# KhaoulaAguech/pl-fem-vectoriel

Hardware: AMD Instinct MI355X
Metric: eigenmodes/sec (assembly+solve), 7-core P2 mesh, 10 modes; |Δn_eff| vs ref (higher is better)
Workload: dtype f64

## Files before the change

include/plfem.h:

```cpp
#ifndef PLFEM_H
#define PLFEM_H

#include <stdint.h>

#ifdef __cplusplus
extern "C" {
#endif

#define PLFEM_OK 0
#define PLFEM_EINVAL (-1)
#define PLFEM_EMESH (-2)
#define PLFEM_EHIP (-3)
#define PLFEM_ENOCONV (-4)
#define PLFEM_ESTATE (-5)
#define PLFEM_ESINGULAR (-6)
#define PLFEM_ERESIDUAL (-7)
#define PLFEM_EHOST (-8)

typedef struct plfem_symbolic plfem_symbolic;
typedef struct plfem_ctx plfem_ctx;

int plfem_symbolic_create(int32_t nv, int32_t ne, const double* p_host, const int32_t* t_host,
                          int32_t leaf_elems, int32_t nthreads, plfem_symbolic** out,
                          char* err, int32_t errlen);
// ... 79 lines not shown
int plfem_modes_dev(plfem_ctx* ctx, const double** evecs_dev, int32_t* k);

int plfem_set_option(plfem_ctx* ctx, const char* name, double value);

int plfem_timings(plfem_ctx* ctx, double* out_host );

enum { PLFEM_PROF_KFWD = 0, PLFEM_PROF_FWD_SWEEP, PLFEM_PROF_BWD_SWEEP, PLFEM_PROF_SPMV_B, PLFEM_PROF_COUNT };
int plfem_profile_begin(plfem_ctx* ctx, int32_t max_ranges);
int plfem_profile_end(plfem_ctx* ctx, double* out_host );

#define PLFEM_LOC_TOL 1e-10
#define PLFEM_LOC_EPS4 8.881784197001252e-16
typedef struct plfem_locator plfem_locator;
int plfem_locator_bytes(const plfem_symbolic* sym, int64_t* bytes);
int plfem_locator_create(const plfem_symbolic* sym, int32_t device, void* hip_stream, void* mem_dev, int64_t mem_bytes,
                         plfem_locator** out, char* err, int32_t errlen);
void plfem_locator_destroy(plfem_locator* loc);
const char* plfem_locator_last_error(const plfem_locator* loc);
int plfem_stage_modes(plfem_locator* loc, int32_t ncomp, int32_t k, int32_t nrows, const double* src_dev, double* dst_dev);
int plfem_sample_fields(plfem_locator* loc, int32_t ncomp, int32_t k, const double* modes_dev, int32_t indexed,
                        const double* beta_dev, int32_t npts, const double* points_dev, double* out_dev, int32_t* elem_dev);
int plfem_overlap_work_bytes(int32_t ka, int32_t kb, int64_t* bytes);
int plfem_field_overlap(plfem_locator* loc_a, const double* modes_a_dev, int32_t ka, int32_t indexed_a,
                        plfem_locator* loc_b, const double* modes_b_dev, int32_t kb, int32_t indexed_b, int32_t ncomp,
                        const double* cores_host, int32_t ncore, double eps_core, double eps_clad,
                        void* work_dev, int64_t work_bytes, double* out_host);
int plfem_overlap_posed_work_bytes(const plfem_locator* loc_b, int32_t ka, int32_t kb, int32_t nposes, int64_t* bytes);
int plfem_field_overlap_posed(plfem_locator* loc_a, const double* modes_a_dev, int32_t ka, int32_t indexed_a,
                              plfem_locator* loc_b, const double* modes_b_dev, int32_t kb, int32_t indexed_b, int32_t ncomp,
                              const double* cores_host, int32_t ncore, double eps_core, double eps_clad,
                              int32_t nposes, const double* poses_host ,
                              void* work_dev, int64_t work_bytes, double* out_host );
int plfem_gram_work_bytes(int32_t ncomp, int32_t k, int64_t* bytes);
int plfem_mode_grams(plfem_locator* loc, int32_t ncomp, int32_t k, const double* modes_dev, int32_t indexed,
                     const double* cores_host, int32_t ncore, void* work_dev, int64_t work_bytes, double* out_host);

int plfem_profile_gram_work_bytes(int32_t ncomp, int32_t k, int64_t* bytes);
int plfem_profile_grams(plfem_locator* loc, int32_t ncomp, int32_t k, const double* modes_dev, int32_t indexed,
                        const double* layers_host, int32_t nlayer, double eps_bg, void* work_dev, int64_t work_bytes,
                        double* out_host);

int plfem_locator_set_index_map(plfem_locator* loc, const double* eps_host, int32_t nx, int32_t ny, double x0, double y0,
                                double dx, double dy);

int plfem_core_gram_work_bytes(const plfem_locator* loc, int32_t ncomp, int32_t k, int32_t ncore, int64_t* bytes);
int plfem_core_grams(plfem_locator* loc, int32_t ncomp, int32_t k, const double* modes_dev, int32_t indexed,
                     const double* cores_host, int32_t ncore, void* work_dev, int64_t work_bytes,
                     double* out_host   ,
                     int64_t* count_host );

int plfem_velocity_gram_work_bytes(const plfem_locator* loc, int32_t ncomp, int32_t k, int32_t nvel, int64_t* bytes);
int plfem_velocity_grams(plfem_locator* loc, int32_t ncomp, int32_t k, const double* modes_dev, int32_t indexed,
                         const double* cores_host, int32_t ncore, double eps_core, double eps_clad,
                         const double* layers_host, int32_t nlayer, double eps_bg, int32_t use_profile,
                         const double* velocities_host , int32_t nvel,
                         void* work_dev, int64_t work_bytes,
                         double* out_host    ,
                         int64_t* count_host );

int plfem_moment_gram_work_bytes(int32_t ncomp, int32_t k, int64_t* bytes);
int plfem_moment_grams(plfem_locator* loc, int32_t ncomp, int32_t k, const double* modes_dev, int32_t indexed,
                       const double* cores_host, int32_t ncore, const double origin_host[2], void* work_dev,
                       int64_t work_bytes, double* out_host);

int plfem_profile_tangent_gram_work_bytes(const plfem_locator* loc, int32_t ncomp, int32_t k, int32_t ntan, int32_t nmap,
                                          int32_t moments, int64_t* bytes);
int plfem_profile_tangent_grams(plfem_locator* loc, int32_t ncomp, int32_t k, const double* modes_dev, int32_t indexed,
                                const double* layers_host, int32_t nlayer, double eps_bg,
                                const double* tangents_host , int32_t ntan,
                                const double* tangent_maps_host , int32_t nmap,
                                const int32_t* tangent_map_host ,
                                int32_t moments, const double origin_host[2],
                                void* work_dev, int64_t work_bytes, double* out_host);

int plfem_index_map_gradient_work_bytes(const plfem_locator* loc, int32_t ncomp, int32_t k, int64_t* bytes);
int plfem_index_map_gradients(plfem_locator* loc, int32_t ncomp, int32_t k, const double* modes_dev, int32_t indexed,
                              const double* layers_host, int32_t nlayer, double eps_bg,
                              void* work_dev, int64_t work_bytes,
                              double* out_host ,
                              int32_t* support_host );

int plfem_quartic_work_bytes(int32_t ncomp, int32_t k, int64_t* bytes);
int plfem_mode_quartic(plfem_locator* loc, int32_t ncomp, int32_t k, const double* modes_dev, int32_t indexed,
                       const double* cores_host, int32_t ncore, double w_core, double w_clad,
                       void* work_dev, int64_t work_bytes, double* out_host);

int plfem_project_work_bytes(int32_t ncomp, int32_t k, int32_t la, int32_t lb, int64_t* bytes);
int plfem_mode_project(plfem_locator* loc, int32_t ncomp, int32_t k, const double* modes_dev, int32_t indexed,
                       int32_t la, const double* xfac_host ,
                       int32_t lb, const double* yfac_host ,
                       void* work_dev, int64_t work_bytes, double* out_host );

int plfem_project_sampled_work_bytes(int32_t ncomp, int32_t k, int32_t nf, int64_t* bytes);
int plfem_mode_project_sampled(plfem_locator* loc, int32_t ncomp, int32_t k, const double* modes_dev, int32_t indexed,
                               int32_t nx, int32_t ny, double x0, double y0, double dx, double dy,
                               int32_t nf, const double* frames_dev ,
                               void* work_dev, int64_t work_bytes, double* out_host );

int plfem_indicator_work_bytes(const plfem_locator* loc, int32_t ncomp, int32_t k, int64_t* bytes);
int plfem_mode_indicators(plfem_locator* loc, int32_t ncomp, int32_t k, const double* modes_dev, int32_t indexed,
                          const double* lambda_host , double k0, double alpha_p,
                          const double* cores_host, int32_t ncore, double eps_core, double eps_clad,
                          const double* layers_host, int32_t nlayer, double eps_bg,
                          void* work_dev, int64_t work_bytes, double* out_host );

int plfem_flux_gram_work_bytes(int32_t k, int64_t* bytes);
int plfem_flux_grams(plfem_locator* loc, int32_t ncomp, int32_t k, const double* modes_dev, int32_t indexed,
                     const double* cores_host, int32_t ncore, double eps_core, double eps_clad,
                     const double* layers_host, int32_t nlayer, double eps_bg, int32_t use_profile,
                     void* work_dev, int64_t work_bytes, double* out_host );
int plfem_sample_efields(plfem_locator* loc, int32_t ncomp, int32_t k, const double* modes_dev, int32_t indexed,
                         const double* beta_dev , double k0,
                         const double* cores_host, int32_t ncore, double eps_core, double eps_clad,
                         const double* layers_host, int32_t nlayer, double eps_bg, int32_t use_profile,
                         int32_t npts, const double* points_dev, double* out_dev ,
                         double* eps_dev , int32_t* elem_dev);
int plfem_flux_overlap_posed_work_bytes(const plfem_locator* loc_b, int32_t ka, int32_t kb, int32_t nposes, int64_t* bytes);
int plfem_flux_overlap_posed(plfem_locator* loc_a, const double* modes_a_dev, int32_t ka, int32_t indexed_a,
                             const double* cores_a_host, int32_t ncore_a, double eps_core_a, double eps_clad_a,
                             const double* layers_a_host, int32_t nlayer_a, double eps_bg_a, int32_t use_profile_a,
                             plfem_locator* loc_b, const double* modes_b_dev, int32_t kb, int32_t indexed_b,
                             const double* cores_b_host, int32_t ncore_b, double eps_core_b, double eps_clad_b,
                             const double* layers_b_host, int32_t nlayer_b, double eps_bg_b, int32_t use_profile_b,
                             int32_t nposes, const double* poses_host ,
                             void* work_dev, int64_t work_bytes, double* out_host );

#ifdef PLFEM_TEST_HOOKS
int plfem_debug_factor_until(plfem_ctx* ctx, double sigma, int32_t level, int32_t step, int32_t stage);
int plfem_debug_copy(plfem_ctx* ctx, const char* name, int64_t offset, int64_t count, double* out_host);
int plfem_debug_symeig(int32_t n, const double* a_host, int32_t last_rows, double* w_out, double* v_out);
int plfem_debug_symeig_band(int32_t n, int32_t b, const double* a_host, int32_t nsel, double* w_out, double* v_out);
int plfem_debug_set_perturb(plfem_ctx* ctx, double value);
int plfem_debug_set_elements(plfem_ctx* ctx, const double* elem_host );
#define PLFEM_DEBUG_PLAN_FIELDS 10
int plfem_debug_solve_block(plfem_ctx* ctx, const double* rhs_dev, int64_t ldx, double* x_dev, int32_t refine_steps);
int plfem_debug_level_plan(plfem_ctx* ctx, int64_t* out, int64_t cap);
enum { PLFEM_DEBUG_PANEL_DOT = 0, PLFEM_DEBUG_PANEL_AXPY, PLFEM_DEBUG_PANEL_DOT_BLOCK, PLFEM_DEBUG_PANEL_AXPY_BLOCK };
enum { PLFEM_DEBUG_SPMV_B_BLOCK = 0, PLFEM_DEBUG_SPMV_B_BLOCK_IL, PLFEM_DEBUG_SPMV_B_BLOCK_IL_GRAM, PLFEM_DEBUG_SPMV_A_BLOCK };
int plfem_debug_panel(plfem_ctx* ctx, int32_t form, int32_t ncols, const double* Pm, double* W, int64_t ldw, double* H,
                      int32_t ldh, double* hacc, int32_t ldacc, double* wil);
int plfem_debug_scale_store(plfem_ctx* ctx, const double* w, const double* bw, const double* beta2, double* v, double* bv,
                            double* beta_out);
int plfem_debug_first_pass(plfem_ctx* ctx, const double* xl_front, const double* BVm, const double* Vm, int32_t ncols,
                           double* W, int64_t ldw, double* Hout, int32_t ldh);
int plfem_debug_spmv_block(plfem_ctx* ctx, int32_t form, const double* x, double* y, int64_t ld, double* gram_out,
                           int32_t* nparts);
int plfem_debug_chol(plfem_ctx* ctx, const double* G, int32_t ldg, int32_t use_partials, int32_t nchunks, double* Tblk,
                     int32_t ldT, double* Rinv, int32_t* rank_flag);
int plfem_debug_block_scale(plfem_ctx* ctx, const double* W, const double* BW, int64_t ldw, const double* Rinv, double* Vn,
                            double* BVn, int64_t ldv, const double* exp_src, int32_t exp_n, double* exp_dst, int32_t* cnt_dst,
                            int32_t want_front);
int plfem_debug_rotate(plfem_ctx* ctx, const double* V, int32_t m, const double* S, int32_t ldS, int32_t p, double* out);
int plfem_debug_start_field(plfem_ctx* ctx, int32_t nvec, double* out);
#endif

#ifdef __cplusplus
}
#endif
#endif
```

pl_fem_vectoriel_amd/_native.py:

```python
from __future__ import annotations

import ctypes
import time
import os
from typing import Optional

import numpy as np

_HERE = os.path.dirname(os.path.abspath(__file__))
LIB_PATH = os.path.join(_HERE, "libplfem_hip.so")
HOOKS_PATH = os.path.join(_HERE, "libplfem_testhooks.so")

PLFEM_OK = 0
PLFEM_EINVAL, PLFEM_EMESH, PLFEM_EHIP, PLFEM_ENOCONV, PLFEM_ESTATE, PLFEM_ESINGULAR, PLFEM_ERESIDUAL = -1, -2, -3, -4, -5, -6, -7
PLFEM_EHOST = -8
BLOCKS = ("Axx", "Axy", "Ayx", "Ayy", "Minv", "Dxx", "Dxy", "Dyy")
INFO_NAMES = ("nv", "ne", "nedges", "N", "nsolve", "nnz", "levels", "nfronts", "front_doubles", "max_front",
              "solve_entries", "factor_flops", "t_numbering_us", "t_pattern_us", "t_tree_us", "t_fronts_us", "dofs_per_node",
              "arena_doubles")
POST_NAMES = ("norm", "div_energy", "core_x", "core_y", "all_x", "all_y")

EXPORTS = (
    "plfem_symbolic_create", "plfem_symbolic_destroy", "plfem_symbolic_info", "plfem_symbolic_array_bytes",
    "plfem_symbolic_get", "plfem_workspace_bytes", "plfem_create", "plfem_destroy", "plfem_last_error", "plfem_synchronize",
    "plfem_assemble_hfield", "plfem_block_values_dev", "plfem_block_values_host", "plfem_spmv", "plfem_factor",
    "plfem_solve", "plfem_lanczos_shift_invert", "plfem_postprocess", "plfem_timings",
    "plfem_profile_begin", "plfem_profile_end",
    "plfem_mesh_edge_count", "plfem_mesh_refine",
    "plfem_residuals", "plfem_set_option", "plfem_symbolic_create_ex", "plfem_assemble_scalar", "plfem_cmt_coupling",
    "plfem_solve_modes", "plfem_modes_dev",
    "plfem_locator_bytes", "plfem_locator_create", "plfem_locator_destroy", "plfem_locator_last_error", "plfem_stage_modes",
    "plfem_sample_fields", "plfem_overlap_work_bytes", "plfem_field_overlap", "plfem_gram_work_bytes", "plfem_mode_grams",
    "plfem_overlap_posed_work_bytes", "plfem_field_overlap_posed",
    "plfem_quartic_work_bytes", "plfem_mode_quartic", "plfem_project_work_bytes", "plfem_mode_project",
    "plfem_core_gram_work_bytes", "plfem_core_grams", "plfem_moment_gram_work_bytes", "plfem_moment_grams",
    "plfem_set_index_profile", "plfem_profile_gram_work_bytes", "plfem_profile_grams",
    "plfem_project_sampled_work_bytes", "plfem_mode_project_sampled",
    "plfem_indicator_work_bytes", "plfem_mode_indicators", "plfem_mesh_refine_marked_count", "plfem_mesh_refine_marked",
    "plfem_set_index_map", "plfem_locator_set_index_map",
    "plfem_flux_gram_work_bytes", "plfem_flux_grams", "plfem_sample_efields",
    "plfem_flux_overlap_posed_work_bytes", "plfem_flux_overlap_posed",
    "plfem_profile_tangent_gram_work_bytes", "plfem_profile_tangent_grams",
    "plfem_velocity_gram_work_bytes", "plfem_velocity_grams",
    "plfem_index_map_gradient_work_bytes", "plfem_index_map_gradients",
)
SOLVE_STATS = ("nconv", "n_opinv", "restarts", "max_rel_res", "n_block_solves", "true_residual_first", "true_residual", "refined",
               "pivot_perturbations", "assemble_us", "factor_us", "lanczos_us", "post_us", "upload_us", "residual_us", "call_us")
TEST_HOOK_EXPORTS = ("plfem_debug_factor_until", "plfem_debug_copy", "plfem_debug_symeig", "plfem_debug_symeig_band",
                     "plfem_debug_set_perturb", "plfem_debug_solve_block", "plfem_debug_level_plan", "plfem_debug_panel",
                     "plfem_debug_scale_store", "plfem_debug_first_pass", "plfem_debug_spmv_block", "plfem_debug_chol",
                     "plfem_debug_block_scale", "plfem_debug_rotate", "plfem_debug_start_field", "plfem_debug_set_elements")
PANEL_FORMS = ("dot", "axpy", "dot_block", "axpy_block")
SPMV_BLOCK_FORMS = ("b_block", "b_block_il", "b_block_il_gram", "a_block")
BLOCK_P = 4
PLAN_FIELDS = ("count", "fwd_rows", "bwd_rows", "fwd_mixed", "max_s2", "max_m", "fwd_n", "bwd_n", "steps", "max_block_p")
MAX_NCV = 320
PROF_SLOTS = ("k_fwd", "fwd_sweep", "bwd_sweep", "spmv_b")

_ARRAY_DTYPES = {
    "edof": np.int32, "tsorted": np.int32, "edges": np.int32, "doflocs": np.float64, "bmask": np.uint8,
    "interior": np.int32, "int_index": np.int32, "rowptr": np.int32, "colind": np.int32, "slot_row": np.int32,
    "nptr": np.int32, "nadj": np.int32, "nloc": np.uint8, "leaf_of_elem": np.int32, "leaf_elem_ptr": np.int32, "leaf_elems": np.int32, "epos": np.int32, "epos_leaf": np.int32,
    "owner": np.int32, "fs": np.int32, "fb": np.int32, "fs_true": np.int32, "fb_true": np.int32,
    "fnode_ptr": np.int64, "fnodes": np.int32, "cinv0": np.int32, "cinv1": np.int32, "foff": np.int64, "soff": np.int64, "prow": np.int32, "npos": np.int32,
    "loc_grid": np.float64, "loc_cell_ptr": np.int32, "loc_cell_elems": np.int32, "loc_stats": np.float64,
    "elem_nbr": np.int32,
}


from scipy.sparse.linalg import ArpackNoConvergence as _ArpackNoConvergence


def set_index_map_call(entry, handle, index_map):
    if index_map is None:
        return entry(handle, None, 0, 0, 0.0, 0.0, 0.0, 0.0)
    eps, x0, y0, dx, dy = index_map
    eps = np.ascontiguousarray(eps, dtype=np.float64)
    if eps.ndim != 2:
        raise ValueError("the index map must be a (ny, nx) array")
    return entry(handle, eps.ctypes.data_as(ctypes.c_void_p), eps.shape[1], eps.shape[0], float(x0), float(y0), float(dx),
                 float(dy))


class ArpackLikeNoConvergence(_ArpackNoConvergence, RuntimeError):

    def __init__(self, msg, eigenvalues=None, eigenvectors=None, stats=None):
        _ArpackNoConvergence.__init__(self, msg, eigenvalues, eigenvectors)
        self.stats = stats


_lib = None
_hooks = None

SCRATCH_FILL = None


def device_scratch(nbytes: int, tdev):
    import torch
    if SCRATCH_FILL is None:
        return torch.empty(int(nbytes), dtype=torch.uint8, device=tdev)
    buf = torch.empty((int(nbytes) + 7) & ~7, dtype=torch.uint8, device=tdev)
    buf.view(torch.float64).fill_(float(SCRATCH_FILL))
    torch.cuda.current_stream(tdev).synchronize()
    return buf


def device_output(shape, dtype, tdev):
    import torch
    if SCRATCH_FILL is None:
        return torch.empty(shape, dtype=dtype, device=tdev)
    shape = tuple(int(v) for v in (shape if isinstance(shape, (tuple, list)) else (shape,)))
    nbytes = int(np.prod(shape, dtype=np.int64)) * torch.empty((), dtype=dtype).element_size()
    return device_scratch(nbytes, tdev)[:nbytes].view(dtype).view(shape)


def _tune_host_allocator(_force: bool = False) -> None:
    if os.environ.get("PLFEM_MALLOC_TUNE", "0") != "1" and not _force:
        return
    try:
        libc = ctypes.CDLL("libc.so.6")
        libc.mallopt(-3, 32 << 20)
        libc.mallopt(-1, 512 << 20)
    except (OSError, AttributeError):
        pass


def load_library() -> ctypes.CDLL:
    global _lib
    if _lib is not None:
        return _lib
    if not os.path.exists(LIB_PATH):
        raise RuntimeError(
            f"libplfem_hip.so requis: {LIB_PATH} not found — build it with "
            "`python -c 'import __graft_entry__ as g; g.build()'` (hipcc --offload-arch=gfx950). "
            "There is no CPU fallback for the eigenmode path.")
    import torch
    lib = ctypes.CDLL(LIB_PATH)
    _tune_host_allocator()
    c_void_pp = ctypes.POINTER(ctypes.c_void_p)
    lib.plfem_symbolic_create.argtypes = [ctypes.c_int32, ctypes.c_int32, ctypes.c_void_p, ctypes.c_void_p,
                                          ctypes.c_int32, ctypes.c_int32, c_void_pp, ctypes.c_char_p, ctypes.c_int32]
    lib.plfem_symbolic_create_ex.argtypes = [ctypes.c_int32, ctypes.c_int32, ctypes.c_void_p, ctypes.c_void_p, ctypes.c_int32,
                                             ctypes.c_int32, ctypes.c_int32, ctypes.c_int32, c_void_pp, ctypes.c_char_p, ctypes.c_int32]
    lib.plfem_symbolic_destroy.argtypes = [ctypes.c_void_p]
    lib.plfem_symbolic_destroy.restype = None
    lib.plfem_symbolic_info.argtypes = [ctypes.c_void_p, ctypes.c_void_p]
    lib.plfem_symbolic_array_bytes.argtypes = [ctypes.c_void_p, ctypes.c_char_p]
    lib.plfem_symbolic_array_bytes.restype = ctypes.c_int64
    lib.plfem_symbolic_get.argtypes = [ctypes.c_void_p, ctypes.c_char_p, ctypes.c_void_p, ctypes.c_int64]
    lib.plfem_workspace_bytes.argtypes = [ctypes.c_void_p, ctypes.c_int32, ctypes.POINTER(ctypes.c_int64)]
    lib.plfem_create.argtypes = [ctypes.c_void_p, ctypes.c_int32, ctypes.c_void_p, ctypes.c_int32, ctypes.c_void_p,
                                 ctypes.c_int64, c_void_pp, ctypes.c_char_p, ctypes.c_int32]
    lib.plfem_destroy.argtypes = [ctypes.c_void_p]
    lib.plfem_destroy.restype = None
    lib.plfem_last_error.argtypes = [ctypes.c_void_p]
    lib.plfem_last_error.restype = ctypes.c_char_p
    lib.plfem_synchronize.argtypes = [ctypes.c_void_p]
    lib.plfem_assemble_hfield.argtypes = [ctypes.c_void_p, ctypes.c_void_p, ctypes.c_int32, ctypes.c_double,
                                          ctypes.c_double, ctypes.c_double, ctypes.c_double]
    lib.plfem_assemble_scalar.argtypes = [ctypes.c_void_p, ctypes.c_void_p, ctypes.c_int32, ctypes.c_double,
                                          ctypes.c_double, ctypes.c_double]
    lib.plfem_cmt_coupling.argtypes = [ctypes.c_void_p, ctypes.c_int32, ctypes.c_void_p, ctypes.c_void_p, ctypes.c_void_p,
                                       ctypes.c_int32, ctypes.c_double, ctypes.c_double, ctypes.c_void_p, ctypes.c_void_p,
                                       ctypes.c_void_p, ctypes.POINTER(ctypes.c_double)]
    lib.plfem_block_values_dev.argtypes = [ctypes.c_void_p, ctypes.c_int32, c_void_pp]
    lib.plfem_block_values_host.argtypes = [ctypes.c_void_p, ctypes.c_int32, ctypes.c_void_p]
    lib.plfem_spmv.argtypes = [ctypes.c_void_p, ctypes.c_int32, ctypes.c_void_p, ctypes.c_void_p]
    lib.plfem_factor.argtypes = [ctypes.c_void_p, ctypes.c_double]
    lib.plfem_solve.argtypes = [ctypes.c_void_p, ctypes.c_void_p, ctypes.c_void_p, ctypes.c_int32]
    lib.plfem_lanczos_shift_invert.argtypes = [ctypes.c_void_p, ctypes.c_int32, ctypes.c_int32, ctypes.c_double,
                                               ctypes.c_int32, ctypes.c_double, ctypes.c_void_p, ctypes.c_void_p,
                                               ctypes.c_void_p]
    lib.plfem_postprocess.argtypes = [ctypes.c_void_p, ctypes.c_int32, ctypes.c_void_p, ctypes.c_void_p,
                                      ctypes.c_int32, ctypes.c_void_p, ctypes.c_void_p, ctypes.c_void_p]
    lib.plfem_timings.argtypes = [ctypes.c_void_p, ctypes.c_void_p]
    lib.plfem_mesh_edge_count.argtypes = [ctypes.c_int32, ctypes.c_int32, ctypes.c_void_p, ctypes.c_void_p,
                                          ctypes.POINTER(ctypes.c_int32), ctypes.c_char_p, ctypes.c_int32]
    lib.plfem_mesh_refine.argtypes = [ctypes.c_int32, ctypes.c_int32, ctypes.c_void_p, ctypes.c_void_p,
                                      ctypes.c_void_p, ctypes.c_void_p, ctypes.c_char_p, ctypes.c_int32]
    lib.plfem_profile_begin.argtypes = [ctypes.c_void_p, ctypes.c_int32]
    lib.plfem_profile_end.argtypes = [ctypes.c_void_p, ctypes.c_void_p]
    lib.plfem_residuals.argtypes = [ctypes.c_void_p, ctypes.c_int32, ctypes.c_void_p, ctypes.c_void_p, ctypes.c_void_p]
    lib.plfem_set_option.argtypes = [ctypes.c_void_p, ctypes.c_char_p, ctypes.c_double]
    lib.plfem_solve_modes.argtypes = ([ctypes.c_void_p, ctypes.c_void_p, ctypes.c_int32] + [ctypes.c_double] * 5 +
                                      [ctypes.c_int32, ctypes.c_int32, ctypes.c_double, ctypes.c_int32, ctypes.c_double,
                                       ctypes.c_double] + [ctypes.c_void_p] * 6)
    lib.plfem_modes_dev.argtypes = [ctypes.c_void_p, c_void_pp, ctypes.POINTER(ctypes.c_int32)]
    lib.plfem_locator_bytes.argtypes = [ctypes.c_void_p, ctypes.POINTER(ctypes.c_int64)]
    lib.plfem_locator_create.argtypes = [ctypes.c_void_p, ctypes.c_int32, ctypes.c_void_p, ctypes.c_void_p, ctypes.c_int64,
                                         c_void_pp, ctypes.c_char_p, ctypes.c_int32]
    lib.plfem_locator_destroy.argtypes = [ctypes.c_void_p]
    lib.plfem_locator_destroy.restype = None
    lib.plfem_locator_last_error.argtypes = [ctypes.c_void_p]
    lib.plfem_locator_last_error.restype = ctypes.c_char_p
    vp, i32, i64, f64 = ctypes.c_void_p, ctypes.c_int32, ctypes.c_int64, ctypes.c_double
    head, tail, size = [vp, i32, i32, vp, i32], [vp, i64, vp], [ctypes.POINTER(i64)]
    pair = [vp, vp, i32, i32] * 2 + [i32, vp, i32, f64, f64]
    lib.plfem_stage_modes.argtypes = [vp, i32, i32, i32, vp, vp]
    lib.plfem_sample_fields.argtypes = head + [vp, i32, vp, vp, vp]
    lib.plfem_overlap_work_bytes.argtypes = [i32, i32] + size
    lib.plfem_field_overlap.argtypes = pair + tail
    lib.plfem_overlap_posed_work_bytes.argtypes = [vp, i32, i32, i32] + size
    lib.plfem_field_overlap_posed.argtypes = pair + [i32, vp] + tail
    lib.plfem_gram_work_bytes.argtypes = [i32, i32] + size
    lib.plfem_mode_grams.argtypes = head + [vp, i32] + tail
    lib.plfem_core_gram_work_bytes.argtypes = [vp, i32, i32, i32] + size
    lib.plfem_core_grams.argtypes = head + [vp, i32] + tail + [vp]
    lib.plfem_moment_gram_work_bytes.argtypes = [i32, i32] + size
    lib.plfem_moment_grams.argtypes = head + [vp, i32, vp] + tail
    lib.plfem_set_index_profile.argtypes = [vp, vp, i32, f64]
    lib.plfem_set_index_map.argtypes = [vp, vp, i32, i32] + [f64] * 4
    lib.plfem_locator_set_index_map.argtypes = lib.plfem_set_index_map.argtypes
    lib.plfem_profile_gram_work_bytes.argtypes = [i32, i32] + size
    lib.plfem_profile_grams.argtypes = head + [vp, i32, f64] + tail
    lib.plfem_profile_tangent_gram_work_bytes.argtypes = [vp, i32, i32, i32, i32, i32] + size
    lib.plfem_profile_tangent_grams.argtypes = head + [vp, i32, f64, vp, i32, vp, i32, vp, i32, vp] + tail
    lib.plfem_quartic_work_bytes.argtypes = [i32, i32] + size
    lib.plfem_mode_quartic.argtypes = head + [vp, i32, f64, f64] + tail
    lib.plfem_project_work_bytes.argtypes = [i32] * 4 + size
    lib.plfem_mode_project.argtypes = head + [i32, vp, i32, vp] + tail
    lib.plfem_project_sampled_work_bytes.argtypes = [i32] * 3 + size
    lib.plfem_mode_project_sampled.argtypes = head + [i32, i32, f64, f64, f64, f64, i32, vp] + tail
    lib.plfem_indicator_work_bytes.argtypes = [vp, i32, i32] + size
    lib.plfem_mode_indicators.argtypes = head + [vp, f64, f64, vp, i32, f64, f64, vp, i32, f64] + tail
    material = [vp, i32, f64, f64, vp, i32, f64, i32]
    lib.plfem_flux_gram_work_bytes.argtypes = [i32] + size
    lib.plfem_flux_grams.argtypes = head + material + tail
    lib.plfem_sample_efields.argtypes = head + [vp, f64] + material + [i32, vp, vp, vp, vp]
    lib.plfem_flux_overlap_posed_work_bytes.argtypes = [vp, i32, i32, i32] + size
    lib.plfem_flux_overlap_posed.argtypes = ([vp, vp, i32, i32] + material) * 2 + [i32, vp] + tail
    lib.plfem_velocity_gram_work_bytes.argtypes = [vp, i32, i32, i32] + size
    lib.plfem_velocity_grams.argtypes = head + material + [vp, i32] + tail + [vp]
    lib.plfem_index_map_gradient_work_bytes.argtypes = [vp, i32, i32] + size
    lib.plfem_index_map_gradients.argtypes = head + [vp, i32, f64] + tail + [vp]
    lib.plfem_mesh_refine_marked_count.argtypes = [ctypes.c_int32, ctypes.c_int32, ctypes.c_void_p, ctypes.c_void_p,
                                                   ctypes.c_void_p, ctypes.POINTER(ctypes.c_int32),
                                                   ctypes.POINTER(ctypes.c_int32), ctypes.c_char_p, ctypes.c_int32]
    lib.plfem_mesh_refine_marked.argtypes = [ctypes.c_int32, ctypes.c_int32, ctypes.c_void_p, ctypes.c_void_p, ctypes.c_void_p,
                                             ctypes.c_void_p, ctypes.c_void_p, ctypes.c_void_p, ctypes.c_char_p, ctypes.c_int32]
    _lib = lib
    return lib


def _ptr(a: np.ndarray):
    return a.ctypes.data_as(ctypes.c_void_p)


def mesh_refine(p, t):
    lib = load_library()
    p = np.ascontiguousarray(np.asarray(p, dtype=np.float64))
    t = np.ascontiguousarray(np.asarray(t, dtype=np.int32))
    if p.ndim != 2 or p.shape[0] != 2 or t.ndim != 2 or t.shape[0] != 3:
        raise ValueError("mesh.p must be (2, nv) and mesh.t (3, ne)")
    err = ctypes.create_string_buffer(512)
    nedges = ctypes.c_int32(0)
    rc = lib.plfem_mesh_edge_count(p.shape[1], t.shape[1], _ptr(p), _ptr(t), ctypes.byref(nedges), err, 512)
    if rc != PLFEM_OK:
        raise ValueError(f"plfem_mesh_edge_count failed ({rc}): {err.value.decode()}")
    p2 = np.empty((2, p.shape[1] + nedges.value), dtype=np.float64)
    t2 = np.empty((3, 4 * t.shape[1]), dtype=np.int32)
    rc = lib.plfem_mesh_refine(p.shape[1], t.shape[1], _ptr(p), _ptr(t), _ptr(p2), _ptr(t2), err, 512)
    if rc != PLFEM_OK:
        raise ValueError(f"plfem_mesh_refine failed ({rc}): {err.value.decode()}")
    return p2, t2


def mesh_refine_marked(p, t, marked):
    lib = load_library()
    p = np.ascontiguousarray(np.asarray(p, dtype=np.float64))
    t = np.ascontiguousarray(np.asarray(t, dtype=np.int32))
    if p.ndim != 2 or p.shape[0] != 2 or t.ndim != 2 or t.shape[0] != 3:
        raise ValueError("mesh.p must be (2, nv) and mesh.t (3, ne)")
    try:
        mk = np.asarray(marked)
        if mk.dtype.kind not in "biu":
            raise TypeError
    except (TypeError, ValueError):
        raise ValueError("marked must be an array of one flag (bool or integer) per element") from None
    if mk.shape != (t.shape[1],):
        raise ValueError(f"marked must have one flag per element ({t.shape[1]}), got shape {mk.shape}")
    mk = np.ascontiguousarray(mk != 0, dtype=np.uint8)
    err = ctypes.create_string_buffer(512)
    nv2, ne2 = ctypes.c_int32(0), ctypes.c_int32(0)
    rc = lib.plfem_mesh_refine_marked_count(p.shape[1], t.shape[1], _ptr(p), _ptr(t), _ptr(mk), ctypes.byref(nv2),
                                            ctypes.byref(ne2), err, 512)
    if rc != PLFEM_OK:
        raise ValueError(f"plfem_mesh_refine_marked_count failed ({rc}): {err.value.decode()}")
    p2 = np.empty((2, nv2.value), dtype=np.float64)
    t2 = np.empty((3, ne2.value), dtype=np.int32)
    parent = np.empty(ne2.value, dtype=np.int32)
    rc = lib.plfem_mesh_refine_marked(p.shape[1], t.shape[1], _ptr(p), _ptr(t), _ptr(mk), _ptr(p2), _ptr(t2), _ptr(parent),
                                      err, 512)
    if rc != PLFEM_OK:
        raise ValueError(f"plfem_mesh_refine_marked failed ({rc}): {err.value.decode()}")
    return p2, t2, parent


def load_test_hooks() -> ctypes.CDLL:
    global _hooks
    if _hooks is not None:
        return _hooks
    load_library()
    if not os.path.exists(HOOKS_PATH):
        raise RuntimeError(f"{HOOKS_PATH} not found -- build it with `python -c 'import __graft_entry__ as g; g.build()'`")
    h = ctypes.CDLL(HOOKS_PATH)
    h.plfem_debug_factor_until.argtypes = [ctypes.c_void_p, ctypes.c_double, ctypes.c_int32, ctypes.c_int32, ctypes.c_int32]
    h.plfem_debug_copy.argtypes = [ctypes.c_void_p, ctypes.c_char_p, ctypes.c_int64, ctypes.c_int64, ctypes.c_void_p]
    h.plfem_debug_set_perturb.argtypes = [ctypes.c_void_p, ctypes.c_double]
    h.plfem_debug_set_elements.argtypes = [ctypes.c_void_p, ctypes.c_void_p]
    h.plfem_debug_solve_block.argtypes = [ctypes.c_void_p, ctypes.c_void_p, ctypes.c_int64, ctypes.c_void_p, ctypes.c_int32]
    h.plfem_debug_level_plan.argtypes = [ctypes.c_void_p, ctypes.c_void_p, ctypes.c_int64]
    h.plfem_debug_symeig.argtypes = [ctypes.c_int32, ctypes.c_void_p, ctypes.c_int32, ctypes.c_void_p, ctypes.c_void_p]
    h.plfem_debug_symeig_band.argtypes = [ctypes.c_int32, ctypes.c_int32, ctypes.c_void_p, ctypes.c_int32,
                                          ctypes.c_void_p, ctypes.c_void_p]
    vp, i32, i64 = ctypes.c_void_p, ctypes.c_int32, ctypes.c_int64
    h.plfem_debug_panel.argtypes = [vp, i32, i32, vp, vp, i64, vp, i32, vp, i32, vp]
    h.plfem_debug_scale_store.argtypes = [vp, vp, vp, vp, vp, vp, vp]
    h.plfem_debug_first_pass.argtypes = [vp, vp, vp, vp, i32, vp, i64, vp, i32]
    h.plfem_debug_spmv_block.argtypes = [vp, i32, vp, vp, i64, vp, vp]
    h.plfem_debug_chol.argtypes = [vp, vp, i32, i32, i32, vp, i32, vp, vp]
    h.plfem_debug_block_scale.argtypes = [vp, vp, vp, i64, vp, vp, vp, i64, vp, i32, vp, vp, i32]
    h.plfem_debug_rotate.argtypes = [vp, vp, i32, vp, i32, i32, vp]
    h.plfem_debug_start_field.argtypes = [vp, i32, vp]
    _hooks = h
    return h


def debug_symeig(a, last_rows: int = -1):
    lib = load_test_hooks()
    a = np.ascontiguousarray(np.asarray(a, dtype=np.float64))
    n = a.shape[0]
    if a.shape != (n, n):
        raise ValueError("square matrix expected")
    w = np.empty(n, dtype=np.float64)
    v = np.empty((n, n if last_rows < 0 else last_rows), dtype=np.float64)
    rc = lib.plfem_debug_symeig(n, _ptr(a), int(last_rows), _ptr(w), _ptr(v))
    if rc != PLFEM_OK:
        raise ValueError(f"plfem_debug_symeig failed ({rc})")
    return w, v


def debug_symeig_band(a, b: int, nsel: int):
    lib = load_test_hooks()
    a = np.ascontiguousarray(np.asarray(a, dtype=np.float64))
    n = a.shape[0]
    if a.shape != (n, n):
        raise ValueError("square matrix expected")
    w = np.empty(n, dtype=np.float64)
    v = np.empty((n, n), dtype=np.float64)
    rc = lib.plfem_debug_symeig_band(n, int(b), _ptr(a), int(nsel), _ptr(w), _ptr(v))
    if rc != PLFEM_OK:
        raise ValueError(f"plfem_debug_symeig_band failed ({rc})")
    return w, v


def default_host_threads() -> int:
    ncpu = os.cpu_count() or 1
    if ncpu < 64:
        return max(1, min(ncpu, 8))
    try:
        local_world = max(1, int(os.environ.get("LOCAL_WORLD_SIZE", "1")))
    except ValueError:
        local_world = 1
    return max(2, min(24, (ncpu // 2) // local_world))


class Symbolic:

    def __init__(self, p, t, leaf_elems: int = 0, nthreads: int = 0, dofs_per_node: int = 2, dirichlet: bool = True):
        lib = load_library()
        p = np.ascontiguousarray(np.asarray(p, dtype=np.float64))
        t = np.ascontiguousarray(np.asarray(t, dtype=np.int32))
        if p.ndim != 2 or p.shape[0] != 2 or t.ndim != 2 or t.shape[0] != 3:
            raise ValueError("mesh.p must be (2, nv) and mesh.t (3, ne)")
        h = ctypes.c_void_p()
        err = ctypes.create_string_buffer(512)
        if nthreads <= 0:
            nthreads = int(os.environ.get("PLFEM_HOST_THREADS", default_host_threads()))
        if leaf_elems <= 0:
            leaf_elems = int(os.environ.get("PLFEM_LEAF_ELEMS", 0))
        rc = lib.plfem_symbolic_create_ex(p.shape[1], t.shape[1], _ptr(p), _ptr(t), int(leaf_elems), int(nthreads),
                                          int(dofs_per_node), 1 if dirichlet else 0, ctypes.byref(h), err, 512)
        if rc != PLFEM_OK:
            raise ValueError(f"plfem_symbolic_create failed ({rc}): {err.value.decode()}")
        self._h = h
        self._lib = lib
        info = np.zeros(32, dtype=np.int64)
        lib.plfem_symbolic_info(h, _ptr(info))
        self.info = {k: int(info[i]) for i, k in enumerate(INFO_NAMES)}
        for k in ("nv", "ne", "nedges", "N", "nsolve", "nnz"):
            setattr(self, k, self.info[k])
        self.dofs_per_node = self.info["dofs_per_node"]

    def array(self, name: str) -> np.ndarray:
        nb = self._lib.plfem_symbolic_array_bytes(self._h, name.encode())
        if nb < 0:
            raise KeyError(name)
        out = np.empty(nb // np.dtype(_ARRAY_DTYPES[name]).itemsize, dtype=_ARRAY_DTYPES[name])
        rc = self._lib.plfem_symbolic_get(self._h, name.encode(), _ptr(out), ctypes.c_int64(nb))
        if rc != PLFEM_OK:
            raise RuntimeError(f"plfem_symbolic_get({name}) failed: {rc}")
        return out

    def close(self):
        if getattr(self, "_h", None):
            self._lib.plfem_symbolic_destroy(self._h)
            self._h = None

    def __del__(self):
        try:
            self.close()
        except Exception:
            pass


class Context:

    def __init__(self, sym: Symbolic, device: Optional[int] = None, max_ncv: int = 65, use_torch_stream: bool = True):
        import torch

        lib = load_library()
        if not torch.cuda.is_available():
            raise RuntimeError("no HIP device visible: the eigenmode path has no CPU fallback")
        if device is None:
            device = torch.cuda.current_device()
        self.torch = torch
        self.device = int(device)
        self.tdev = torch.device("cuda", self.device)
        self.sym = sym
        self._lib = lib
        stream = torch.cuda.current_stream(self.tdev).cuda_stream if use_torch_stream else 0
        h = ctypes.c_void_p()
        err = ctypes.create_string_buffer(512)
        need = ctypes.c_int64(0)
        rc = lib.plfem_workspace_bytes(sym._h, int(max_ncv), ctypes.byref(need))
        if rc != PLFEM_OK:
            raise ValueError(f"plfem_workspace_bytes failed ({rc})")
        t0 = time.perf_counter()
        self.workspace = device_scratch(int(need.value) + 256, self.tdev)
        self.t_workspace = time.perf_counter() - t0
        base = self.workspace.data_ptr()
        aligned = (base + 255) & ~255
        rc = lib.plfem_create(sym._h, self.device, ctypes.c_void_p(stream), int(max_ncv), ctypes.c_void_p(aligned),
                              ctypes.c_int64(int(need.value)), ctypes.byref(h), err, 512)
        if rc in (PLFEM_EINVAL, PLFEM_EMESH):
            raise ValueError(f"plfem_create: {err.value.decode()}")
        if rc != PLFEM_OK:
            raise RuntimeError(f"plfem_create failed ({rc}): {err.value.decode()}")
        self._h = h
        self.max_ncv = int(max_ncv)
        self.N = sym.N
        self.dpn = sym.dofs_per_node
        self.n2 = self.dpn * sym.N

    def _check(self, rc, what):
        if rc == PLFEM_OK:
            return
        msg = self._lib.plfem_last_error(self._h).decode()
        if rc in (PLFEM_EINVAL, PLFEM_EMESH):
            raise ValueError(f"{what}: {msg}")
        raise RuntimeError(f"{what} failed ({rc}): {msg}")

    def _cores(self, cores):
        c = np.ascontiguousarray(np.asarray(cores, dtype=np.float64).reshape(-1, 3))
        return c, c.shape[0]

    def empty(self, *shape):
        return device_output(shape, self.torch.float64, self.tdev)

    def set_index_profile(self, profile=None):
        if profile is None:
            self._check(self._lib.plfem_set_index_profile(self._h, None, 0, 0.0), "plfem_set_index_profile")
            self.set_index_map(None)
            return
        t = np.ascontiguousarray(np.asarray(profile.table(), dtype=np.float64).reshape(-1, 8))
        index_map = getattr(profile, "index_map", None)
# ... 36 lines not shown

    def spmv(self, which: str, x):
        y = self.empty(self.n2)
        self._check(self._lib.plfem_spmv(self._h, 0 if which == "A" else 1, ctypes.c_void_p(x.data_ptr()),
                                         ctypes.c_void_p(y.data_ptr())), "plfem_spmv")
        return y

    def factor(self, sigma: float):
        self._check(self._lib.plfem_factor(self._h, float(sigma)), "plfem_factor")

    def solve(self, rhs, refine_steps: int = 0):
        x = self.empty(self.n2)
        self._check(self._lib.plfem_solve(self._h, ctypes.c_void_p(rhs.data_ptr()), ctypes.c_void_p(x.data_ptr()),
                                          int(refine_steps)), "plfem_solve")
        return x

    def lanczos(self, k, ncv, tol, maxiter, sigma):
        evals = np.empty(k, dtype=np.float64)
        evecs = self.empty(k, self.n2)
        stats = np.zeros(8, dtype=np.float64)
        rc = self._lib.plfem_lanczos_shift_invert(self._h, int(k), int(ncv), float(tol), int(maxiter), float(sigma),
                                                  _ptr(evals), ctypes.c_void_p(evecs.data_ptr()), _ptr(stats))
        st = {"nconv": int(stats[0]), "n_opinv": int(stats[1]), "restarts": int(stats[2]), "max_rel_res": float(stats[3]),
              "n_block_solves": int(stats[4])}
        if rc == PLFEM_ENOCONV:
            raise ArpackLikeNoConvergence(self._lib.plfem_last_error(self._h).decode(), evals, evecs, st)
        self._check(rc, "plfem_lanczos_shift_invert")
        return evals, evecs, st

    def solve_modes(self, cores, eps_core, eps_clad, k0, alpha_p, sigma, k, ncv, tol, maxiter, residual_tol, tol_refined,
                    modes_host=None):
        c, n = self._cores(cores)
        evals = np.empty(k, dtype=np.float64)
        post = np.zeros((k, len(POST_NAMES)), dtype=np.float64)
        resid = np.zeros(k, dtype=np.float64)
        stats = np.zeros(len(SOLVE_STATS), dtype=np.float64)
        frac = ctypes.c_double(0.0)
        if modes_host is not None and (tuple(modes_host.shape) != (k, self.dpn * self.sym.nsolve) or not modes_host.is_contiguous()
                                       or modes_host.dtype != self.torch.float64 or modes_host.device.type != "cpu"):
            raise ValueError("modes_host must be a contiguous float64 CPU tensor of shape (k, dofs_per_node * nsolve)")
        rc = self._lib.plfem_solve_modes(self._h, _ptr(c), n, float(eps_core), float(eps_clad), float(k0), float(alpha_p),
                                         float(sigma), int(k), int(ncv), float(tol), int(maxiter), float(residual_tol),
                                         float(tol_refined), _ptr(evals), _ptr(post), ctypes.cast(ctypes.byref(frac), ctypes.c_void_p),
                                         _ptr(resid), ctypes.c_void_p(modes_host.data_ptr()) if modes_host is not None else None,
                                         _ptr(stats))
        st = {name: (float(stats[i]) if name.endswith("_us") or "res" in name else int(stats[i])) for i, name in enumerate(SOLVE_STATS)}
        st["refined"] = bool(st["refined"])
        if rc == PLFEM_ENOCONV:
            raise ArpackLikeNoConvergence(self._lib.plfem_last_error(self._h).decode(), evals, self.modes_dev(), st)
        self._check(rc, "plfem_solve_modes")
        return evals, post, float(frac.value), resid, st

    def modes_dev(self):
        ptr = ctypes.c_void_p()
        k = ctypes.c_int32(0)
        self._check(self._lib.plfem_modes_dev(self._h, ctypes.byref(ptr), ctypes.byref(k)), "plfem_modes_dev")

        class _View:
            __cuda_array_interface__ = {"shape": (int(k.value), int(self.n2)), "typestr": "<f8", "data": (int(ptr.value), False),
                                        "version": 2, "strides": None}
        return self.torch.as_tensor(_View(), device=self.tdev).clone()

    def postprocess(self, evecs, cores, want_interior: bool = True):
        k = evecs.shape[0]
        c, n = self._cores(cores)
        out = np.zeros((k, len(POST_NAMES)), dtype=np.float64)
        frac = ctypes.c_double(0.0)
        modes_int = self.empty(k, self.dpn * self.sym.nsolve) if want_interior else None
        self._check(self._lib.plfem_postprocess(self._h, int(k), ctypes.c_void_p(evecs.data_ptr()), _ptr(c), n,
                                                _ptr(out), ctypes.byref(frac),
                                                ctypes.c_void_p(modes_int.data_ptr()) if want_interior else None),
                    "plfem_postprocess")
        return out, float(frac.value), modes_int

    def timings(self):
        t = np.zeros(8, dtype=np.float64)
        self._check(self._lib.plfem_timings(self._h, _ptr(t)), "plfem_timings")
        return {"assemble_us": t[0], "factor_us": t[1], "lanczos_us": t[2], "post_us": t[3], "upload_us": t[4],
                "pivot_perturbations": int(t[5])}

    def debug_factor_until(self, sigma, level, step, stage):
        self._check(load_test_hooks().plfem_debug_factor_until(self._h, float(sigma), int(level), int(step), int(stage)),
                    "plfem_debug_factor_until")

    def debug_copy(self, name: str, offset: int, count: int) -> np.ndarray:
        out = np.empty(int(count), dtype=np.float64)
        self._check(load_test_hooks().plfem_debug_copy(self._h, name.encode(), ctypes.c_int64(int(offset)),
                                                       ctypes.c_int64(int(count)), _ptr(out)), "plfem_debug_copy")
        return out

    def debug_set_perturb(self, value: float):
        self._check(load_test_hooks().plfem_debug_set_perturb(self._h, float(value)), "plfem_debug_set_perturb")

    def debug_set_elements(self, elem: np.ndarray):
        elem = np.ascontiguousarray(elem, dtype=np.float64)
        if elem.size != self.sym.ne * 8 * 36:
            raise ValueError("debug_set_elements: need ne x 8 x 36 doubles")
        self._check(load_test_hooks().plfem_debug_set_elements(self._h, _ptr(elem)), "plfem_debug_set_elements")

    def debug_solve_block(self, rhs, x, ldx: int, refine_steps: int = 0):
        self._check(load_test_hooks().plfem_debug_solve_block(self._h, ctypes.c_void_p(rhs.data_ptr()), ctypes.c_int64(int(ldx)),
                                                              ctypes.c_void_p(x.data_ptr()), int(refine_steps)),
                    "plfem_debug_solve_block")

    @staticmethod
    def _dev(t, offset: int = 0):
        return None if t is None else ctypes.c_void_p(t.data_ptr() + 8 * int(offset))

    def debug_panel(self, form: str, ncols: int, Pm, W, ldw: int, H, ldh: int, hacc=None, ldacc: int = 0, wil=None):
        d = self._dev
        self._check(load_test_hooks().plfem_debug_panel(self._h, PANEL_FORMS.index(form), int(ncols), d(Pm), d(W), int(ldw), d(H),
                                                        int(ldh), d(hacc), int(ldacc), d(wil)), "plfem_debug_panel")

    def debug_scale_store(self, w, bw, beta2, v, bv, beta_out=None):
        d = self._dev
        self._check(load_test_hooks().plfem_debug_scale_store(self._h, d(w), d(bw), d(beta2), d(v), d(bv), d(beta_out)),
                    "plfem_debug_scale_store")

    def debug_first_pass(self, xl_front, BVm, Vm, ncols: int, W, ldw: int, Hout, ldh: int):
        d = self._dev
        self._check(load_test_hooks().plfem_debug_first_pass(self._h, d(xl_front), d(BVm), d(Vm), int(ncols), d(W), int(ldw),
                                                             d(Hout), int(ldh)), "plfem_debug_first_pass")

    def debug_spmv_block(self, form: str, x, y, ld: int, gram_out=None) -> int:
        nparts = ctypes.c_int32(0)
        d = self._dev
        self._check(load_test_hooks().plfem_debug_spmv_block(self._h, SPMV_BLOCK_FORMS.index(form), d(x), d(y), int(ld),
                                                             d(gram_out), ctypes.byref(nparts)), "plfem_debug_spmv_block")
        return int(nparts.value)

    def debug_chol(self, G, ldg: int, use_partials: bool, nchunks: int, Tblk, ldT: int, Rinv, Tblk_offset: int = 0) -> int:
        flag = ctypes.c_int32(0)
        d = self._dev
        self._check(load_test_hooks().plfem_debug_chol(self._h, d(G), int(ldg), 1 if use_partials else 0, int(nchunks),
                                                       d(Tblk, Tblk_offset), int(ldT), d(Rinv), ctypes.byref(flag)),
                    "plfem_debug_chol")
        return int(flag.value)

    def debug_block_scale(self, W, BW, ldw: int, Rinv, Vn, BVn, ldv: int, exp_src=None, exp_n: int = 0, exp_dst=None,
                          cnt_dst=None, want_front: bool = False):
        d = self._dev
        self._check(load_test_hooks().plfem_debug_block_scale(self._h, d(W), d(BW), int(ldw), d(Rinv), d(Vn), d(BVn), int(ldv),
                                                              d(exp_src), int(exp_n), d(exp_dst), d(cnt_dst),
                                                              1 if want_front else 0), "plfem_debug_block_scale")

    def debug_rotate(self, V, m: int, S, ldS: int, p: int, out):
        d = self._dev
        self._check(load_test_hooks().plfem_debug_rotate(self._h, d(V), int(m), d(S), int(ldS), int(p), d(out)),
                    "plfem_debug_rotate")

    def debug_start_field(self, nvec: int, out):
        self._check(load_test_hooks().plfem_debug_start_field(self._h, int(nvec), self._dev(out)), "plfem_debug_start_field")

    def debug_level_plan(self):
        nl = self.sym.info["levels"] + 1
        out = np.zeros(len(PLAN_FIELDS) * nl, dtype=np.int64)
        self._check(load_test_hooks().plfem_debug_level_plan(self._h, _ptr(out), ctypes.c_int64(out.size)),
                    "plfem_debug_level_plan")
        return [dict(zip(PLAN_FIELDS, (int(v) for v in row))) for row in out.reshape(nl, len(PLAN_FIELDS))]

    def profile_begin(self, max_launches: int = 4096):
        self._check(self._lib.plfem_profile_begin(self._h, int(max_launches)), "plfem_profile_begin")

    def profile_end(self):
        out = np.zeros((len(PROF_SLOTS), 3), dtype=np.float64)
        self._check(self._lib.plfem_profile_end(self._h, _ptr(out)), "plfem_profile_end")
        res = {"launches": int(out[0, 0]), "total_us": float(out[0, 1]), "bytes": float(out[0, 2])}
        res["slots"] = {name: {"ranges": int(out[i, 0]), "total_us": float(out[i, 1]), "bytes": float(out[i, 2])}
                        for i, name in enumerate(PROF_SLOTS)}
        return res

    def residuals(self, evals, evecs) -> np.ndarray:
        lam = np.ascontiguousarray(np.asarray(evals, dtype=np.float64))
        out = np.zeros(len(lam), dtype=np.float64)
        self._check(self._lib.plfem_residuals(self._h, len(lam), _ptr(lam), ctypes.c_void_p(evecs.data_ptr()), _ptr(out)),
                    "plfem_residuals")
        return out

    def set_option(self, name: str, value: float):
        self._check(self._lib.plfem_set_option(self._h, name.encode(), float(value)), "plfem_set_option")

    def synchronize(self):
        self._check(self._lib.plfem_synchronize(self._h), "plfem_synchronize")

    def close(self):
        if getattr(self, "_h", None):
            self._lib.plfem_destroy(self._h)
            self._h = None
            self.workspace = None

    def __del__(self):
        try:
            self.close()
        except Exception:
            pass
```

pl_fem_vectoriel_amd/csrc/api_debug.hip:

```cpp
#include <algorithm>
#include <cmath>
#include <cstring>
#include <numeric>
#include <string>
#include <vector>

#ifndef PLFEM_TEST_HOOKS
#define PLFEM_TEST_HOOKS 1
#endif
#include "device.h"

namespace {
void perturb_root_pivots(plfem_ctx* c) {
  if (c->test_perturb != 0.0)
    plfem::launch_axpby(c, (int64_t)2 * c->dpn * c->S->fs[0], 1.0 + c->test_perturb, c->d_delta, 0.0, c->d_delta,
                        c->d_delta);
}
}

extern "C" int plfem_debug_set_perturb(plfem_ctx* c, double value) try {
  if (!c) return PLFEM_EINVAL;
  c->test_perturb = value;
  c->test_post_factor = value != 0.0 ? perturb_root_pivots : nullptr;
  c->factored = false;
  return PLFEM_OK;
} catch (...) { return host_failure(c); }

extern "C" int plfem_debug_factor_until(plfem_ctx* c, double sigma, int32_t level, int32_t step, int32_t stage) try {
  if (!c) return PLFEM_EINVAL;
  if (!c->assembled) { c->err = "debug factor before assemble"; return PLFEM_ESTATE; }
  TRY(wait_for_upload(c));
  plfem::launch_factor(c, sigma, level, step, stage);
  HIP_TRY(c, hipStreamSynchronize(c->stream));
  return check_launch(c, "debug factor");
} catch (...) { return host_failure(c); }

extern "C" int plfem_debug_copy(plfem_ctx* c, const char* name, int64_t offset, int64_t count, double* out_host) try {
  if (!c || !name || !out_host || offset < 0 || count < 0) return PLFEM_EINVAL;
  std::string n(name);
  const double* src = nullptr;
  if (n == "front") src = c->d_front;
  else if (n == "schur") src = c->d_schur;
  else if (n == "fvec") src = c->d_fvec;
  else if (n == "wbuf") src = c->d_wbuf;
  else if (n == "rbuf") src = c->d_rbuf;
  else if (n == "dinv") src = c->d_dinv;
  else if (n == "delta") src = c->d_delta;
  else if (n == "fvec2") src = c->d_fvec2;
  else if (n == "xl") src = c->d_xl;
  else if (n == "elem") src = c->d_elem;
  else if (n == "V") src = c->d_V;
  else if (n == "BV") src = c->d_BV;
  else if (n == "Hcols") src = c->d_Hcols;
  else if (n == "counters") {
    if (offset + count > 4) return PLFEM_EINVAL;
    int32_t tmp[4];
    HIP_TRY(c, hipStreamSynchronize(c->stream));
    HIP_TRY(c, hipMemcpy(tmp, c->d_counters, sizeof(tmp), hipMemcpyDeviceToHost));
    for (int64_t q = 0; q < count; ++q) out_host[q] = (double)tmp[offset + q];
    return PLFEM_OK;
  }
  else if (n == "colind" || n == "slot_row") {
    if (offset + count > c->nnz) return PLFEM_EINVAL;
    std::vector<int32_t> tmp((size_t)count);
    HIP_TRY(c, hipStreamSynchronize(c->stream));
    HIP_TRY(c, hipMemcpy(tmp.data(), (n == "colind" ? c->d_colind : c->d_slot_row) + offset, sizeof(int32_t) * count, hipMemcpyDeviceToHost));
    for (int64_t q = 0; q < count; ++q) out_host[q] = (double)tmp[q];
    return PLFEM_OK;
  }
  else return PLFEM_EINVAL;
  HIP_TRY(c, hipStreamSynchronize(c->stream));
  HIP_TRY(c, hipMemcpy(out_host, src + offset, sizeof(double) * count, hipMemcpyDeviceToHost));
  return PLFEM_OK;
} catch (...) { return host_failure(c); }

extern "C" int plfem_debug_set_elements(plfem_ctx* c, const double* elem_host) try {
  if (!c || !elem_host) return PLFEM_EINVAL;
  HIP_TRY(c, hipSetDevice(c->device));
  TRY(wait_for_upload(c));
  HIP_TRY(c, hipStreamSynchronize(c->stream));
  HIP_TRY(c, hipMemcpy(c->d_elem, elem_host, sizeof(double) * (size_t)c->ne * plfem::ELEM_STRIDE, hipMemcpyHostToDevice));
  plfem::launch_csr_gather(c);
  HIP_TRY(c, hipStreamSynchronize(c->stream));
  TRY(check_launch(c, "debug set elements"));
  c->assembled = true;
  c->factored = false;
  return PLFEM_OK;
} catch (...) { return host_failure(c); }

extern "C" int plfem_debug_solve_block(plfem_ctx* c, const double* rhs_dev, int64_t ldx, double* x_dev, int32_t refine_steps) try {
  constexpr int P = plfem::BLOCK_P;
  if (!c || !rhs_dev || !x_dev || refine_steps < 0) return PLFEM_EINVAL;
  if (!c->factored) { c->err = "debug block solve before plfem_factor"; return PLFEM_ESTATE; }
  if (c->max_block_p < P) { c->err = "debug block solve: the LDS budget of this tree allows one right-hand side per sweep"; return PLFEM_EINVAL; }
  if (ldx < c->n2) { c->err = "debug block solve: ldx < n2"; return PLFEM_EINVAL; }
  const int64_t scratch = (int64_t)c->n2 * plfem::basis_cols(c->max_ncv);
  if (refine_steps > 0 && 3 * P * ldx > scratch) { c->err = "debug block solve: ldx too large for the refinement scratch"; return PLFEM_EINVAL; }
  HIP_TRY(c, hipSetDevice(c->device));
  plfem::solve_refined(c, P, rhs_dev, x_dev, ldx, false, refine_steps, c->d_V2, c->d_V2 + (size_t)P * ldx,
                       c->d_V2 + (size_t)2 * P * ldx);
  HIP_TRY(c, hipStreamSynchronize(c->stream));
  return check_launch(c, "debug block solve");
} catch (...) { return host_failure(c); }

extern "C" int plfem_debug_level_plan(plfem_ctx* c, int64_t* out, int64_t cap) try {
  if (!c || !out) return PLFEM_EINVAL;
  const plfem::LaunchPlan& plan = *c->plan;
  const int nl = (int)plan.levels.size();
  if (cap < (int64_t)PLFEM_DEBUG_PLAN_FIELDS * nl) { c->err = "debug level plan: cap too small"; return PLFEM_EINVAL; }
  for (int l = 0; l < nl; ++l) {
    const plfem::LevelInfo& li = plan.levels[l];
    const int next = l + 1 < nl ? plan.levels[l + 1].step0 : (int)plan.upd_n.size();
    const int64_t rec[PLFEM_DEBUG_PLAN_FIELDS] = {li.count, li.fwd_rows, li.bwd_rows, li.fwd_mixed ? 1 : 0, li.max_s2, li.max_m,
                                                  li.fwd_n, li.bwd_n, next - li.step0, c->max_block_p};
    std::copy(rec, rec + PLFEM_DEBUG_PLAN_FIELDS, out + (int64_t)PLFEM_DEBUG_PLAN_FIELDS * l);
  }
  return PLFEM_OK;
} catch (...) { return host_failure(c); }

namespace {
int lanczos_hook_done(plfem_ctx* c, const char* what) {
  HIP_TRY(c, hipStreamSynchronize(c->stream));
  return check_launch(c, what);
}
}

extern "C" int plfem_debug_panel(plfem_ctx* c, int32_t form, int32_t ncols, const double* Pm, double* W, int64_t ldw, double* H,
                                 int32_t ldh, double* hacc, int32_t ldacc, double* wil) try {
  constexpr int P = plfem::BLOCK_P;
  if (!c || !H || !Pm || !W || form < PLFEM_DEBUG_PANEL_DOT || form > PLFEM_DEBUG_PANEL_AXPY_BLOCK) return PLFEM_EINVAL;
  if (ncols < 1 || ncols > c->max_ncv + P) { c->err = "debug panel: need 1 <= ncols <= max_ncv + BLOCK_P"; return PLFEM_EINVAL; }
  const bool block = form == PLFEM_DEBUG_PANEL_DOT_BLOCK || form == PLFEM_DEBUG_PANEL_AXPY_BLOCK;
  if (block && (ldw < c->n2 || ldh < ncols || (hacc && ldacc < ncols))) { c->err = "debug panel: leading dimension too small"; return PLFEM_EINVAL; }
  HIP_TRY(c, hipSetDevice(c->device));
  switch (form) {
    case PLFEM_DEBUG_PANEL_DOT: plfem::launch_panel_dot(c, 1, Pm, ncols, W, ldw, H, ldh, hacc, ldacc); break;
    case PLFEM_DEBUG_PANEL_AXPY: plfem::launch_panel_axpy(c, 1, Pm, ncols, H, ldh, W, ldw); break;
    case PLFEM_DEBUG_PANEL_DOT_BLOCK: plfem::launch_panel_dot(c, P, Pm, ncols, W, ldw, H, ldh, hacc, ldacc); break;
    default: plfem::launch_panel_axpy(c, P, Pm, ncols, H, ldh, W, ldw, wil); break;
  }
  return lanczos_hook_done(c, "debug panel");
} catch (...) { return host_failure(c); }

extern "C" int plfem_debug_scale_store(plfem_ctx* c, const double* w, const double* bw, const double* beta2, double* v, double* bv,
                                       double* beta_out) try {
  if (!c || !w || !bw || !beta2 || !v || !bv) return PLFEM_EINVAL;
  HIP_TRY(c, hipSetDevice(c->device));
  plfem::launch_scale_store(c, w, bw, beta2, v, bv, beta_out);
  return lanczos_hook_done(c, "debug scale store");
} catch (...) { return host_failure(c); }

extern "C" int plfem_debug_first_pass(plfem_ctx* c, const double* xl_front, const double* BVm, const double* Vm, int32_t ncols,
                                      double* W, int64_t ldw, double* Hout, int32_t ldh) try {
  if (!c || !xl_front || !BVm || !Vm || !W || !Hout) return PLFEM_EINVAL;
  if (ncols < 1 || ncols > plfem::FIRST_COLS || ldw < c->n2 || ldh < ncols) { c->err = "debug first pass: need 1 <= ncols <= FIRST_COLS, ldw >= n2, ldh >= ncols"; return PLFEM_EINVAL; }
  HIP_TRY(c, hipSetDevice(c->device));
  HIP_TRY(c, hipMemcpyAsync(c->d_xl, xl_front, sizeof(double) * 2 * c->fnodes_total * plfem::BLOCK_P, hipMemcpyDeviceToDevice, c->stream));
  plfem::launch_first_pass_block(c, BVm, Vm, ncols, W, ldw, Hout, ldh);
  return lanczos_hook_done(c, "debug first pass");
} catch (...) { return host_failure(c); }

extern "C" int plfem_debug_spmv_block(plfem_ctx* c, int32_t form, const double* x, double* y, int64_t ld, double* gram_out,
                                      int32_t* nparts) try {
  constexpr int P = plfem::BLOCK_P;
  if (!c || !x || !y || form < PLFEM_DEBUG_SPMV_B_BLOCK || form > PLFEM_DEBUG_SPMV_A_BLOCK) return PLFEM_EINVAL;
  if (!c->assembled) { c->err = "debug block spmv before assemble"; return PLFEM_ESTATE; }
  if (ld < c->n2) { c->err = "debug block spmv: ld < n2"; return PLFEM_EINVAL; }
  HIP_TRY(c, hipSetDevice(c->device));
  int np = 0;
  switch (form) {
    case PLFEM_DEBUG_SPMV_B_BLOCK: plfem::launch_spmv(c, 1, P, x, y, ld); break;
    case PLFEM_DEBUG_SPMV_B_BLOCK_IL: plfem::launch_spmv_b_block_il(c, x, y, ld); break;
    case PLFEM_DEBUG_SPMV_B_BLOCK_IL_GRAM:
      np = plfem::launch_spmv_b_block_il(c, x, y, ld, c->d_partial);
      if (gram_out) HIP_TRY(c, hipMemcpyAsync(gram_out, c->d_partial, sizeof(double) * P * P * np, hipMemcpyDeviceToDevice, c->stream));
      break;
    default: plfem::launch_spmv(c, 0, P, x, y, ld); break;
  }
  if (nparts) *nparts = np;
  return lanczos_hook_done(c, "debug block spmv");
} catch (...) { return host_failure(c); }

extern "C" int plfem_debug_chol(plfem_ctx* c, const double* G, int32_t ldg, int32_t use_partials, int32_t nchunks, double* Tblk,
                                int32_t ldT, double* Rinv, int32_t* rank_flag) try {
  constexpr int P = plfem::BLOCK_P;
  if (!c || !Tblk || !Rinv || ldT < P) return PLFEM_EINVAL;
  HIP_TRY(c, hipSetDevice(c->device));
  if (use_partials) {
    if (nchunks < 1 || (size_t)P * P * nchunks > c->partial_doubles) { c->err = "debug chol: nchunks out of range"; return PLFEM_EINVAL; }
    if (G) HIP_TRY(c, hipMemcpyAsync(c->d_partial, G, sizeof(double) * P * P * nchunks, hipMemcpyDeviceToDevice, c->stream));
  } else if (!G || ldg < P) {
    return PLFEM_EINVAL;
  }
  HIP_TRY(c, hipMemsetAsync(c->d_counters + 2, 0, sizeof(int32_t), c->stream));
  if (use_partials) plfem::launch_chol_from_partials(c, nchunks, Tblk, ldT, Rinv);
  else plfem::launch_chol_block(c, G, ldg, Tblk, ldT, Rinv);
  int32_t flag = 0;
  HIP_TRY(c, hipMemcpyAsync(&flag, c->d_counters + 2, sizeof(int32_t), hipMemcpyDeviceToHost, c->stream));
  HIP_TRY(c, hipMemsetAsync(c->d_counters + 2, 0, sizeof(int32_t), c->stream));
  TRY(lanczos_hook_done(c, "debug chol"));
  if (rank_flag) *rank_flag = flag;
  return PLFEM_OK;
} catch (...) { return host_failure(c); }

extern "C" int plfem_debug_block_scale(plfem_ctx* c, const double* W, const double* BW, int64_t ldw, const double* Rinv, double* Vn,
                                       double* BVn, int64_t ldv, const double* exp_src, int32_t exp_n, double* exp_dst,
                                       int32_t* cnt_dst, int32_t want_front) try {
  if (!c || !W || !BW || !Rinv || !Vn || !BVn || exp_n < 0) return PLFEM_EINVAL;
  if (ldw < c->n2 || ldv < c->n2) { c->err = "debug block scale: leading dimension < n2"; return PLFEM_EINVAL; }
  if (exp_dst && (!exp_src || !cnt_dst)) { c->err = "debug block scale: an export needs exp_src and cnt_dst"; return PLFEM_EINVAL; }
  HIP_TRY(c, hipSetDevice(c->device));
  plfem::launch_block_scale(c, W, BW, ldw, Rinv, Vn, BVn, ldv, exp_src, exp_dst ? exp_n : 0, exp_dst, cnt_dst,
                            want_front ? c->d_fvec : nullptr);
  return lanczos_hook_done(c, "debug block scale");
} catch (...) { return host_failure(c); }

extern "C" int plfem_debug_rotate(plfem_ctx* c, const double* V, int32_t m, const double* S, int32_t ldS, int32_t p, double* out) try {
  if (!c || !V || !S || !out) return PLFEM_EINVAL;
  if (m < 1 || m > PLFEM_MAX_NCV + plfem::BLOCK_P || p < 1 || ldS < m) { c->err = "debug rotate: need 1 <= m <= PLFEM_MAX_NCV + BLOCK_P, p >= 1, ldS >= m"; return PLFEM_EINVAL; }
  HIP_TRY(c, hipSetDevice(c->device));
  plfem::launch_rotate(c, V, m, S, ldS, p, out);
  return lanczos_hook_done(c, "debug rotate");
} catch (...) { return host_failure(c); }

extern "C" int plfem_debug_start_field(plfem_ctx* c, int32_t nvec, double* out) try {
  if (!c || !out || nvec < 1 || nvec > plfem::BLOCK_P) return PLFEM_EINVAL;
  HIP_TRY(c, hipSetDevice(c->device));
  plfem::launch_start_field(c, nvec, out);
  return lanczos_hook_done(c, "debug start field");
} catch (...) { return host_failure(c); }
```

pl_fem_vectoriel_amd/csrc/device.h:

```cpp
#pragma once
#include <hip/hip_runtime.h>

#include <cmath>
#include <cstdint>
#include <functional>
#include <string>
#include <type_traits>
#include <vector>

#include "../../include/plfem.h"
#include "internal.h"
#include "plan.h"

namespace plfem {

constexpr size_t PIN_POST = 0;
constexpr size_t PIN_RESID = 2048;
constexpr size_t PIN_CORE_QP = 4000;
constexpr size_t PIN_COUNTERS = 4096;
constexpr int PIN_COUNTERS_N = 2 * 4;
constexpr size_t PIN_CORES = 6144;
constexpr size_t PIN_LAYERS = 6400;
constexpr size_t PIN_PROJ = 8192;
static_assert(PIN_POST + 5 * PLFEM_MAX_NCV <= PIN_RESID, "pinned layout: post-processing sums");
// ... 28 lines not shown
  double* d = nullptr;
  size_t cap = 0;
  int nx = 0, ny = 0;
  double x0 = 0, y0 = 0, inv_dx = 0, inv_dy = 0;
  bool set() const { return nx > 0; }
};
struct IndexMapHeader {
  double x0, y0, inv_dx, inv_dy;
  int nx, ny;
};
static_assert(sizeof(IndexMapHeader) <= MAP_HEADER * sizeof(double), "the grid fits the map buffer's header");
}

struct plfem_ctx {
  const plfem::Symbolic* S = nullptr;
  const plfem::LaunchPlan* plan = nullptr;
  int device = 0;
  hipStream_t stream = nullptr;
  std::string err;
  int nv = 0, ne = 0, N = 0, nnz = 0, nsolve = 0, L = 0, nfronts = 0, max_ncv = 0;
  int dpn = 2, sh = 1;
  int64_t fnodes_total = 0;
  int64_t n2 = 0;
  int32_t* d_forder = nullptr;
  plfem::FrontRec* d_frec = nullptr;
  int2* d_tiles = nullptr;
  plfem::SweepJob* d_blk = nullptr;
  int32_t *d_tsorted = nullptr, *d_edof = nullptr, *d_rowptr = nullptr, *d_colind = nullptr;
  int32_t *d_slot_row = nullptr, *d_nptr = nullptr, *d_nadj = nullptr, *d_interior = nullptr;
  uint8_t* d_nloc = nullptr;
  uint8_t* d_bmask = nullptr;
  double* d_doflocs = nullptr;
  int32_t *d_fs2 = nullptr, *d_fm = nullptr;
  int64_t *d_fnode_ptr = nullptr, *d_foff = nullptr;
  int32_t *d_fnodes = nullptr, *d_cinv0 = nullptr, *d_cinv1 = nullptr;
  int32_t *d_epos = nullptr, *d_leaf_elem_ptr = nullptr, *d_leaf_elems = nullptr;
  double* d_cores = nullptr;
  double* d_layers = nullptr;
  int nlayer = 0;
  double eps_bg = 0.0;
  plfem::IndexMap map;
  double* d_elem = nullptr;
  double* d_vals[PLFEM_BLK_COUNT] = {nullptr};
  double* d_front = nullptr;
  double* d_schur = nullptr;
  int64_t arena_doubles = 0;
  int64_t* d_soff = nullptr;
  double* d_fvec = nullptr;
  double *d_u0 = nullptr, *d_u1 = nullptr;
  double* d_xl = nullptr;
  int32_t* d_npos = nullptr;
  int32_t* d_prow = nullptr;
  double *d_wbuf = nullptr, *d_rbuf = nullptr;
  double* d_dinv = nullptr;
  double* d_delta = nullptr;
  double* d_fvec2 = nullptr;
  int32_t* d_counters = nullptr;
  double *d_V = nullptr, *d_BV = nullptr, *d_V2 = nullptr, *d_BV2 = nullptr;
  double *d_w = nullptr, *d_bw = nullptr, *d_t1 = nullptr, *d_t2 = nullptr;
  double *d_hblk = nullptr, *d_G = nullptr, *d_Rinv = nullptr;
  double *d_h = nullptr, *d_hacc = nullptr, *d_partial = nullptr, *d_scal = nullptr, *d_S = nullptr;
  double* d_Hcols = nullptr;
  uint8_t* d_coremask = nullptr;
  double* d_post = nullptr;
  size_t post_doubles = 0;
  size_t partial_doubles = 0;
  double* h_pinned = nullptr;
  size_t h_pinned_bytes = 0;
  double* h_staging = nullptr;
  size_t h_staging_bytes = 0;
  double* h_slots = nullptr;
  char* slab = nullptr;
  size_t slab_off = 0, slab_bytes = 0;
  bool own_slab = false;
  int64_t workspace_need = 0;
  bool assembled = false, factored = false;
  hipEvent_t ev_step[2] = {nullptr, nullptr};
  bool defer_sync = false;
  hipStream_t copy_stream = nullptr;
  hipEvent_t ev_copy = nullptr;
  hipEvent_t ev_upload = nullptr;
  bool upload_pending = false;
  bool prof_on = false;
  unsigned prof_toggle = 0;
  int prof_n = 0, prof_max = 0;
  std::vector<hipEvent_t> prof_ev;
  std::vector<int> prof_slot;
  std::vector<double> prof_rbytes;
  int refine_steps = 0;
  void (*test_post_factor)(plfem_ctx*) = nullptr;
  double test_perturb = 0.0;
  int max_block_p = plfem::BLOCK_P;
  double sigma = 0.0;
  hipEvent_t ev[plfem::PH_COUNT][2] = {};
  bool ev_used[plfem::PH_COUNT] = {};
  double* modes_dev = nullptr;
  int modes_k = 0;
};

namespace {
template <class Owner>
int check_launch(Owner* owner, const char* what) {
  const hipError_t e = hipGetLastError();
  if (e == hipSuccess) return PLFEM_OK;
  owner->err = std::string(what) + ": " + hipGetErrorString(e);
  return PLFEM_EHIP;
}

int wait_for_upload(plfem_ctx* c) {
  if (!c->upload_pending) return PLFEM_OK;
  HIP_TRY(c, hipStreamWaitEvent(c->stream, c->ev_upload, 0));
  c->upload_pending = false;
  return PLFEM_OK;
}

hipError_t phase_begin(plfem_ctx* c, plfem::Phase ph) { return hipEventRecord(c->ev[ph][0], c->stream); }
hipError_t phase_end(plfem_ctx* c, plfem::Phase ph) {
  const hipError_t e = hipEventRecord(c->ev[ph][1], c->stream);
  if (e == hipSuccess) c->ev_used[ph] = true;
  return e;
}
double phase_us(const plfem_ctx* c, plfem::Phase ph) {
  float ms = 0;
  return (c->ev_used[ph] && hipEventElapsedTime(&ms, c->ev[ph][0], c->ev[ph][1]) == hipSuccess) ? ms * 1e3 : 0.0;
}
}

namespace plfem {

inline int prof_open(plfem_ctx* c, int slot, double bytes) {
  if (!c->prof_on || c->prof_n >= c->prof_max) return -1;
  while ((int)c->prof_ev.size() < 2 * (c->prof_n + 1)) {
    hipEvent_t e;
    if (hipEventCreate(&e) != hipSuccess) return -1;
    c->prof_ev.push_back(e);
  }
  const int id = c->prof_n++;
  c->prof_slot.push_back(slot);
  c->prof_rbytes.push_back(bytes);
  (void)hipEventRecord(c->prof_ev[2 * id], c->stream);
  return id;
}
inline void prof_close(plfem_ctx* c, int id) {
  if (id >= 0) (void)hipEventRecord(c->prof_ev[2 * id + 1], c->stream);
}

template <int V, int... Rest, class F>
inline void with_constant(int v, F&& f) {
  if constexpr (sizeof...(Rest) == 0) f(std::integral_constant<int, V>());
  else if (v == V) f(std::integral_constant<int, V>());
  else with_constant<Rest...>(v, f);
}

template <int V, bool DESC = false>
__device__ __forceinline__ int multi_reduce_index(int lane) {
  int idx = 0;
#pragma unroll
  for (int h = V / 2, s = 0; h >= 1; h >>= 1, ++s) idx += ((DESC ? lane >> (5 - s) : lane >> s) & 1) ? h : 0;
  return idx;
}

template <int H, int BIT, bool DESC, int V>
__device__ __forceinline__ void multi_reduce_step(double (&a)[V], int lane) {
  if constexpr (H >= 1) {
    const bool up = (lane & BIT) != 0;
#pragma unroll
    for (int k = 0; k < H; ++k) {
      const double send = up ? a[k] : a[k + H];
      const double keep = up ? a[k + H] : a[k];
      a[k] = keep + __shfl_xor(send, BIT);
    }
    multi_reduce_step<H / 2, DESC ? BIT / 2 : 2 * BIT, DESC>(a, lane);
  }
}

template <int V, bool DESC = false>
__device__ __forceinline__ void multi_reduce(double (&a)[V], int lane) {
  multi_reduce_step<V / 2, DESC ? 32 : 1, DESC>(a, lane);
  if constexpr (DESC) {
#pragma unroll
    for (int off = 32 / V; off >= 1; off >>= 1) a[0] += __shfl_xor(a[0], off);
  } else {
#pragma unroll
    for (int off = V; off < 64; off <<= 1) a[0] += __shfl_xor(a[0], off);
  }
}

inline int ceil_div(int64_t a, int64_t b) { return (int)((a + b - 1) / b); }
inline int basis_cols(int max_ncv) { return max_ncv + 1 + BLOCK_P; }
inline int proj_cols(int max_ncv) { return basis_cols(max_ncv) + 8; }

inline const char* profile_table_error(const double* layers, int nlayer, double eps_bg) {
  if (nlayer < 0 || nlayer > MAX_LAYERS) return "nlayer must be in [0, 64]";
  if (nlayer > 0 && !layers) return "null layer table";
  if (!std::isfinite(eps_bg) || !(eps_bg > 0.0)) return "the background permittivity must be finite and positive";
  for (int l = 0; l < nlayer; ++l) {
    const double* p = layers + LAYER_DOUBLES * l;
    for (int j = 0; j < LAYER_DOUBLES; ++j)
      if (!std::isfinite(p[j])) return "every layer entry must be finite";
    if (p[2] < 0.0) return "r_in must be >= 0";
    if (!(p[3] > p[2])) return "r_out must be > r_in";
    if (!(p[4] > 0.0) || !(p[5] > 0.0)) return "permittivities must be positive";
    if (p[6] < 0.0) return "g must be >= 0";
  }
  return nullptr;
}

inline const char* index_map_error(const double* eps, int nx, int ny, double x0, double y0, double dx, double dy) {
  if (nx < 2 || ny < 2 || nx > MAP_NMAX || ny > MAP_NMAX || (int64_t)nx * ny > MAP_SAMPLES)
    return "nx and ny must be in [2, 8192] with nx ny <= 2^24 (a null map with nx = ny = 0 clears)";
  if (!eps) return "null map";
  if (!std::isfinite(x0) || !std::isfinite(y0)) return "the origin must be finite";
  if (!std::isfinite(dx) || !std::isfinite(dy) || !(dx > 0.0) || !(dy > 0.0) || !std::isfinite(1.0 / dx) ||
      !std::isfinite(1.0 / dy))
    return "the steps must be finite and positive, with finite inverses";
  for (int64_t i = 0, n = (int64_t)nx * ny; i < n; ++i)
    if (!std::isfinite(eps[i]) || !(eps[i] > 0.0)) return "every permittivity must be finite and positive";
  return nullptr;
}

template <class Owner>
int set_index_map(Owner* o, const char* entry, const double* eps, int nx, int ny, double x0, double y0, double dx, double dy) {
  IndexMap& m = o->map;
  const bool clear = !eps && nx == 0 && ny == 0;
  if (!clear) {
    if (const char* bad = index_map_error(eps, nx, ny, x0, y0, dx, dy)) {
      o->err = std::string(entry) + ": " + bad;
      return PLFEM_EINVAL;
    }
  }
  if (clear && !m.d) return PLFEM_OK;
  HIP_TRY(o, hipSetDevice(o->device));
  const size_t n = clear ? 0 : (size_t)nx * ny;
  if (clear || m.cap < n) {
    HIP_TRY(o, hipStreamSynchronize(o->stream));
    double* old = m.d;
    m = IndexMap();
    if (old) HIP_TRY(o, hipFree(old));
    if (clear) return PLFEM_OK;
    HIP_TRY(o, hipMalloc((void**)&m.d, sizeof(double) * (MAP_HEADER + n)));
    m.cap = n;
  }
  m.nx = 0;
  const IndexMapHeader head{x0, y0, 1.0 / dx, 1.0 / dy, nx, ny};
  HIP_TRY(o, hipMemcpyAsync(m.d, &head, sizeof(head), hipMemcpyHostToDevice, o->stream));
  HIP_TRY(o, hipMemcpyAsync(m.d + MAP_HEADER, eps, sizeof(double) * n, hipMemcpyHostToDevice, o->stream));
  HIP_TRY(o, hipStreamSynchronize(o->stream));
  m.x0 = head.x0; m.y0 = head.y0; m.inv_dx = head.inv_dx; m.inv_dy = head.inv_dy;
  m.nx = nx; m.ny = ny;
  return PLFEM_OK;
}
inline void free_index_map(IndexMap& m) {
  if (m.d) (void)hipFree(m.d);
  m = IndexMap();
}

void launch_element_matrices(plfem_ctx* c, int ncore, double eps_core, double eps_clad, double k0, double alpha_p);
void launch_element_matrices_scalar(plfem_ctx* c, int ncore, double eps_core, double eps_clad, double k0);
double launch_delta_eps_mass(plfem_ctx* c, int ncore, double eps_core, double eps_clad);
void launch_csr_gather(plfem_ctx* c);
void launch_pattern_fill(plfem_ctx* c);
void launch_spmv(plfem_ctx* c, int which, int P, const double* x, double* y, int64_t ld);
int launch_spmv_b_block_il(plfem_ctx* c, const double* x_interleaved, double* y, int64_t ld, double* gram = nullptr);
inline int spmv_workgroups(int N) { return ceil_div(N, SPMV_WG_ROWS); }
inline size_t gram_partial_doubles(int N) { return (size_t)BLOCK_P * BLOCK_P * spmv_workgroups(N); }
void launch_residuals(plfem_ctx* c, int k, const double* lam_host, const double* evecs, double* out_host);
void launch_factor(plfem_ctx* c, double sigma, int stop_level = -1, int stop_step = 0, int stop_stage = 0);
void launch_solve(plfem_ctx* c, int P, const double* rhs, double* x, int64_t ldx, bool rhs_in_front_order = false);
inline int sweep_ldv(int m) { return (m + 2) & ~1; }
inline size_t sweep_dynamic_lds(int P, int m) { return sizeof(double) * P * sweep_ldv(m); }
inline size_t sweep_lds(int P, int m) { return sweep_dynamic_lds(P, m) + sizeof(double) * 8 * P * 64; }
void solve_refined(plfem_ctx* c, int P, const double* b, double* y, int64_t ld, bool b_in_front_order, int steps, double* ta,
                   double* tb, double* dy);
void launch_panel_dot(plfem_ctx* c, int P, const double* Pm, int ncols, const double* W, int64_t ldw, double* h, int ldh,
                      double* hacc = nullptr, int ldacc = 0);
inline int panel_chunks(int64_t n2) { return ceil_div(n2, PANEL_CHUNK); }
inline size_t panel_dot_partial_doubles(int64_t n2, int ncols) { return (size_t)panel_chunks(n2) * ncols * BLOCK_P; }
void launch_panel_axpy(plfem_ctx* c, int P, const double* Pm, int ncols, const double* H, int ldh, double* W, int64_t ldw,
                       double* w_interleaved = nullptr);
void launch_dot(plfem_ctx* c, const double* a, const double* b, double* out);
void launch_scale_store(plfem_ctx* c, const double* w, const double* bw, const double* beta2, double* v, double* bv,
                        double* beta_out);
void launch_axpby(plfem_ctx* c, int64_t n, double a, const double* x, double b, const double* y, double* z);
void launch_rotate(plfem_ctx* c, const double* V, int m, const double* Smat, int ldS, int p, double* out);
void launch_first_pass_block(plfem_ctx* c, const double* BVm, const double* Vm, int ncols, double* W, int64_t ldw, double* Hout, int ldh);
inline int first_pass_segments(int64_t n2) { return ceil_div(n2, FIRST_ROWS); }
inline size_t first_pass_partial_doubles(int64_t n2) { return (size_t)FIRST_COLS * BLOCK_P * first_pass_segments(n2); }
void launch_chol_from_partials(plfem_ctx* c, int nchunks, double* Tblk, int ldT, double* Rinv);
void launch_chol_block(plfem_ctx* c, const double* G, int ldg, double* Tblk, int ldT, double* Rinv);
void launch_block_scale(plfem_ctx* c, const double* W, const double* BW, int64_t ldw, const double* Rinv, double* Vn,
                        double* BVn, int64_t ldv, const double* exp_src = nullptr, int exp_n = 0, double* exp_dst = nullptr,
                        int32_t* cnt_dst = nullptr, double* bv_front = nullptr);
void launch_start_field(plfem_ctx* c, int nvec, double* out);
void launch_post(plfem_ctx* c, int k, double* evecs, int ncore, double* out_host, double* frac_core, double* modes_int);
void post_enqueue(plfem_ctx* c, int k, double* evecs, int ncore, double* modes_int, const std::function<void(int, int)>* group_done);
void post_finish(plfem_ctx* c, int k, double* out_host, double* frac_core);
void resid_enqueue(plfem_ctx* c, int k, const double* lam_host, const double* evecs);
void resid_finish(plfem_ctx* c, int k, double* out_host);
inline int post_blocks(int N) { return ceil_div(N, POST_ROWS); }
inline size_t post_sum_doubles(int N, int modes) { return (size_t)POST_SUMS * modes * (post_blocks(N) + 1); }
inline size_t resid_sum_doubles(int N, int modes) { return (size_t)RESID_SUMS * modes * (post_blocks(N) + 1); }

}
```

pl_fem_vectoriel_amd/csrc/kernels_assembly.hip:

```cpp
#include "device.h"
#include "p2_element.h"

namespace plfem {
namespace {

constexpr int EPB = 7;

template <bool PROFILE, typename... Map>
__global__ __launch_bounds__(256) void k_element_matrices(
    int ne, int N, const int32_t* __restrict__ tsorted, const double* __restrict__ doflocs,
    const double* __restrict__ cores, int ncore, double inv_eps_core, double inv_eps_clad, double k0sq,
    double alpha_p, int scalar, double* __restrict__ elem, Map... map) {
  static_assert(PROFILE || sizeof...(Map) == 0, "a map belongs to the profile instance");
  __shared__ double s_phi[6][6];
  __shared__ double s_gx[EPB][6][6];
  __shared__ double s_gy[EPB][6][6];
  __shared__ double s_w1[EPB][6];
  __shared__ double s_we[EPB][6];
  const int tid = threadIdx.x;
  const int e0 = blockIdx.x * EPB;
  if (tid < 36) {
    int i = tid / 6, q = tid % 6;
    s_phi[i][q] = p2_phi(i, c_qx[q], c_qy[q]);
  }
// ... 76 lines not shown
    double X, Y;
    P2Map(tsorted, (size_t)ne, doflocs, doflocs + N, e).point(c_qx[q], c_qy[q], X, Y);
    in_core = in_any_core(X, Y, cores, ncore);
  }
  const unsigned long long b = __ballot(in_core);
  if ((threadIdx.x & 63) == 0 && b) atomicAdd(count, (unsigned long long)__popcll(b));
}

constexpr int PATTERN_CAP = 64, PATTERN_OUT = 4096, PATTERN_BIG = 1536;
__global__ __launch_bounds__(128) void k_pattern_fill(int N, int ne, const int32_t* __restrict__ nptr,
                                                      const int32_t* __restrict__ nadj, const int32_t* __restrict__ edof,
                                                      const int32_t* __restrict__ rowptr, int32_t* __restrict__ colind,
                                                      int32_t* __restrict__ slot_row) {
  __shared__ int32_t cand[128][PATTERN_CAP + 1];
  __shared__ int32_t outbuf[PATTERN_OUT];
  __shared__ uint8_t outrow[PATTERN_OUT];
  __shared__ int32_t big[PATTERN_BIG];
  __shared__ uint8_t bigfirst[PATTERN_BIG];
  __shared__ int32_t biglist[128];
  __shared__ int nbig;
  const int i0 = blockIdx.x * 128;
  const int i = i0 + threadIdx.x;
  const int base = rowptr[i0], end = rowptr[min(i0 + 128, N)];
  const bool buffered = end - base <= PATTERN_OUT;
  if (threadIdx.x == 0) nbig = 0;
  __syncthreads();
  auto put = [&](int k, int col, int local_row) {
    if (buffered) { outbuf[k - base] = col; outrow[k - base] = (uint8_t)local_row; }
    else { colind[k] = col; slot_row[k] = i0 + local_row; }
  };
  if (i < N) {
    const int q0 = nptr[i], q1 = nptr[i + 1];
    const int nc = 6 * (q1 - q0);
    int32_t* mine = cand[threadIdx.x];
    if (nc > PATTERN_CAP && nc <= PATTERN_BIG) {
      biglist[atomicAdd(&nbig, 1)] = threadIdx.x;
    } else {
      const bool staged = nc <= PATTERN_CAP;
      if (staged) {
        for (int q = q0; q < q1; ++q) {
          const int e = nadj[q];
#pragma unroll
          for (int a = 0; a < 6; ++a) mine[6 * (q - q0) + a] = edof[(size_t)a * ne + e];
        }
      }
      int prev = -1;
      for (int k = rowptr[i]; k < rowptr[i + 1]; ++k) {
        int best = 0x7fffffff;
        if (staged) {
          for (int j = 0; j < nc; ++j) {
            const int v = mine[j];
            best = (v > prev && v < best) ? v : best;
          }
        } else {
          for (int q = q0; q < q1; ++q) {
            const int e = nadj[q];
#pragma unroll
            for (int a = 0; a < 6; ++a) {
              const int v = edof[(size_t)a * ne + e];
              best = (v > prev && v < best) ? v : best;
            }
          }
        }
        put(k, best, threadIdx.x);
        prev = best;
      }
    }
  }
  __syncthreads();
  const int nb = nbig;
  for (int b = 0; b < nb; ++b) {
    const int lr = biglist[b], r = i0 + lr;
    const int q0 = nptr[r], nc = 6 * (nptr[r + 1] - q0);
    for (int j = threadIdx.x; j < nc; j += 128) big[j] = edof[(size_t)(j % 6) * ne + nadj[q0 + j / 6]];
    __syncthreads();
    for (int j = threadIdx.x; j < nc; j += 128) {
      const int v = big[j];
      bool first = true;
      for (int m = 0; m < j; ++m) first = first && big[m] != v;
      bigfirst[j] = first;
    }
    __syncthreads();
    for (int j = threadIdx.x; j < nc; j += 128) {
      if (!bigfirst[j]) continue;
      const int v = big[j];
      int rank = 0;
      for (int m = 0; m < nc; ++m) rank += (bigfirst[m] && big[m] < v) ? 1 : 0;
      const int k = rowptr[r] + rank;
      if (k < rowptr[r + 1]) put(k, v, lr);
    }
    __syncthreads();
  }
  if (buffered) {
    for (int k = base + threadIdx.x; k < end; k += 128) {
      colind[k] = outbuf[k - base];
      slot_row[k] = i0 + outrow[k - base];
    }
  }
}

__global__ __launch_bounds__(256) void k_csr_gather(int nnz, int ne, const int32_t* __restrict__ slot_row,
                                                    const int32_t* __restrict__ colind, const int32_t* __restrict__ nptr,
                                                    const int32_t* __restrict__ nadj, const uint8_t* __restrict__ nloc,
                                                    const int32_t* __restrict__ edof, const double* __restrict__ elem,
                                                    double* __restrict__ v0, double* __restrict__ v1,
                                                    double* __restrict__ v2, double* __restrict__ v3,
                                                    double* __restrict__ v4, double* __restrict__ v5,
                                                    double* __restrict__ v6, double* __restrict__ v7) {
  int k = blockIdx.x * blockDim.x + threadIdx.x;
  if (k >= nnz) return;
  const int i = slot_row[k], col = colind[k];
  double acc[ELEM_FORMS] = {0, 0, 0, 0, 0, 0, 0, 0};
  const int q1 = nptr[i + 1];
  for (int q = nptr[i]; q < q1; ++q) {
    const int e = nadj[q];
    int b = -1;
#pragma unroll
    for (int bb = 0; bb < 6; ++bb)
      if (edof[(size_t)bb * ne + e] == col) b = bb;
    if (b < 0) continue;
    const double* p = elem + (size_t)e * ELEM_STRIDE + (int)nloc[q] * 6 + b;
#pragma unroll
    for (int f = 0; f < ELEM_FORMS; ++f) acc[f] += p[f * 36];
  }
  v0[k] = acc[0]; v1[k] = acc[1]; v2[k] = acc[2]; v3[k] = acc[3];
  v4[k] = acc[4]; v5[k] = acc[5]; v6[k] = acc[6]; v7[k] = acc[7];
}


template <int P, int DPN>
__global__ __launch_bounds__(256) void k_spmv_b_block(int N, int64_t ld, const int32_t* __restrict__ rowptr,
                                                      const int32_t* __restrict__ colind,
                                                      const uint8_t* __restrict__ bmask, const double* __restrict__ vm,
                                                      const double* __restrict__ x, double* __restrict__ y) {
  int gt = blockIdx.x * blockDim.x + threadIdx.x;
  int row = gt >> 3, sub = gt & 7;
  double sx[P], sy[P];
#pragma unroll
  for (int q = 0; q < P; ++q) { sx[q] = 0.0; sy[q] = 0.0; }
  if (row < N && !bmask[row]) {
    int q0 = rowptr[row], q1 = rowptr[row + 1];
    for (int k = q0 + sub; k < q1; k += 8) {
      const int c = colind[k];
      const double mv = vm[k];
#pragma unroll
      for (int q = 0; q < P; ++q) {
        sx[q] += mv * x[(int64_t)q * ld + c];
        if (DPN == 2) sy[q] += mv * x[(int64_t)q * ld + N + c];
      }
    }
  }
#pragma unroll
  for (int q = 0; q < P; ++q) {
#pragma unroll
    for (int off = 4; off >= 1; off >>= 1) {
      sx[q] += __shfl_xor(sx[q], off, 8);
      sy[q] += __shfl_xor(sy[q], off, 8);
    }
  }
  if (row < N && sub == 0) {
#pragma unroll
    for (int q = 0; q < P; ++q) {
      y[(int64_t)q * ld + row] = sx[q];
      if (DPN == 2) y[(int64_t)q * ld + N + row] = sy[q];
    }
  }
}

template <int P, int DPN, bool GRAM>
__global__ __launch_bounds__(256) void k_spmv_b_block_il(int N, int64_t ld, const int32_t* __restrict__ rowptr,
                                                         const int32_t* __restrict__ colind,
                                                         const uint8_t* __restrict__ bmask, const double* __restrict__ vm,
                                                         const double* __restrict__ xi, double* __restrict__ y,
                                                         double* __restrict__ gram) {
  int gt = blockIdx.x * blockDim.x + threadIdx.x;
  int row = gt >> 3, sub = gt & 7;
  double s[DPN * P];
#pragma unroll
  for (int q = 0; q < DPN * P; ++q) s[q] = 0.0;
  if (row < N && !bmask[row]) {
    int q0 = rowptr[row], q1 = rowptr[row + 1];
    for (int k = q0 + sub; k < q1; k += 8) {
      const int c = colind[k];
      const double mv = vm[k];
      const double* xc = xi + (int64_t)c * (DPN * P);
#pragma unroll
      for (int q = 0; q < DPN * P; ++q) s[q] += mv * xc[q];
    }
  }
#pragma unroll
  for (int q = 0; q < DPN * P; ++q) {
#pragma unroll
    for (int off = 4; off >= 1; off >>= 1) s[q] += __shfl_xor(s[q], off, 8);
  }
  if (row < N && sub == 0) {
#pragma unroll
    for (int comp = 0; comp < DPN; ++comp)
#pragma unroll
      for (int q = 0; q < P; ++q) y[(int64_t)q * ld + (int64_t)comp * N + row] = s[comp * P + q];
  }
  if (GRAM) {
    constexpr int GE = P * P / 8;
    static_assert(!GRAM || GE * 8 == P * P, "the 8 lanes of a row share the P x P entries");
    __shared__ double red[4][P * P];
    double g[GE];
#pragma unroll
    for (int t = 0; t < GE; ++t) g[t] = 0.0;
    if (row < N) {
      const double* xr = xi + (int64_t)row * (DPN * P);
#pragma unroll
      for (int t = 0; t < GE; ++t) {
        const int idx = GE * sub + t, p = idx / P, q = idx % P;
#pragma unroll
        for (int comp = 0; comp < DPN; ++comp) {
          double sq = s[comp * P];
#pragma unroll
          for (int qq = 1; qq < P; ++qq) sq = (q == qq) ? s[comp * P + qq] : sq;
          g[t] = fma(xr[comp * P + p], sq, g[t]);
        }
      }
    }
#pragma unroll
    for (int t = 0; t < GE; ++t) {
      g[t] += __shfl_xor(g[t], 8);
      g[t] += __shfl_xor(g[t], 16);
      g[t] += __shfl_xor(g[t], 32);
    }
    const int wave = threadIdx.x >> 6, lane = threadIdx.x & 63;
    if (lane < 8) {
#pragma unroll
      for (int t = 0; t < GE; ++t) red[wave][GE * lane + t] = g[t];
    }
    __syncthreads();
    if ((int)threadIdx.x < P * P)
      gram[(int64_t)threadIdx.x * gridDim.x + blockIdx.x] = (red[0][threadIdx.x] + red[1][threadIdx.x]) + (red[2][threadIdx.x] + red[3][threadIdx.x]);
  }
}

template <int P>
__global__ __launch_bounds__(256) void k_spmv_a_block(int N, int64_t ld, const int32_t* __restrict__ rowptr,
                                                      const int32_t* __restrict__ colind, const uint8_t* __restrict__ bmask,
                                                      const double* __restrict__ vxx, const double* __restrict__ vxy,
                                                      const double* __restrict__ vyx, const double* __restrict__ vyy,
                                                      const double* __restrict__ x, double* __restrict__ y) {
  int gt = blockIdx.x * blockDim.x + threadIdx.x;
  int row = gt >> 3, sub = gt & 7;
  double sx[P], sy[P];
#pragma unroll
  for (int q = 0; q < P; ++q) { sx[q] = 0.0; sy[q] = 0.0; }
  if (row < N && !bmask[row]) {
    int q0 = rowptr[row], q1 = rowptr[row + 1];
    for (int k = q0 + sub; k < q1; k += 8) {
      const int c = colind[k];
      const double axx = vxx[k], axy = vxy[k], ayx = vyx[k], ayy = vyy[k];
#pragma unroll
      for (int q = 0; q < P; ++q) {
        const double xx = x[(int64_t)q * ld + c], xy = x[(int64_t)q * ld + N + c];
        sx[q] += axx * xx + axy * xy;
        sy[q] += ayx * xx + ayy * xy;
      }
    }
  }
#pragma unroll
  for (int q = 0; q < P; ++q) {
#pragma unroll
    for (int off = 4; off >= 1; off >>= 1) {
      sx[q] += __shfl_xor(sx[q], off, 8);
      sy[q] += __shfl_xor(sy[q], off, 8);
    }
  }
  if (row < N && sub == 0) {
#pragma unroll
    for (int q = 0; q < P; ++q) {
      y[(int64_t)q * ld + row] = sx[q];
      y[(int64_t)q * ld + N + row] = sy[q];
    }
  }
}

}

namespace {
EpsMap eps_map(const IndexMap& m) { return {m.d}; }
}

void launch_element_matrices(plfem_ctx* c, int ncore, double eps_core, double eps_clad, double k0, double alpha_p) {
  int grid = (c->ne + EPB - 1) / EPB;
  if (c->map.set()) {
    hipLaunchKernelGGL((k_element_matrices<true, EpsMap>), dim3(grid), dim3(256), 0, c->stream, c->ne, c->N, c->d_tsorted,
                       c->d_doflocs, c->d_layers, c->nlayer, 0.0, c->eps_bg, k0 * k0, alpha_p, 0, c->d_elem, eps_map(c->map));
    return;
  }
  if (c->nlayer > 0) {
    hipLaunchKernelGGL(k_element_matrices<true>, dim3(grid), dim3(256), 0, c->stream, c->ne, c->N, c->d_tsorted,
                       c->d_doflocs, c->d_layers, c->nlayer, 0.0, c->eps_bg, k0 * k0, alpha_p, 0, c->d_elem);
    return;
  }
  hipLaunchKernelGGL(k_element_matrices<false>, dim3(grid), dim3(256), 0, c->stream, c->ne, c->N, c->d_tsorted,
                     c->d_doflocs, c->d_cores, ncore, 1.0 / eps_core, 1.0 / eps_clad, k0 * k0, alpha_p, 0, c->d_elem);
}

void launch_element_matrices_scalar(plfem_ctx* c, int ncore, double eps_core, double eps_clad, double k0) {
  int grid = (c->ne + EPB - 1) / EPB;
  if (c->map.set()) {
    hipLaunchKernelGGL((k_element_matrices<true, EpsMap>), dim3(grid), dim3(256), 0, c->stream, c->ne, c->N, c->d_tsorted,
                       c->d_doflocs, c->d_layers, c->nlayer, 0.0, c->eps_bg, k0 * k0, 0.0, 1, c->d_elem, eps_map(c->map));
    return;
  }
  if (c->nlayer > 0) {
    hipLaunchKernelGGL(k_element_matrices<true>, dim3(grid), dim3(256), 0, c->stream, c->ne, c->N, c->d_tsorted,
                       c->d_doflocs, c->d_layers, c->nlayer, 0.0, c->eps_bg, k0 * k0, 0.0, 1, c->d_elem);
    return;
  }
  hipLaunchKernelGGL(k_element_matrices<false>, dim3(grid), dim3(256), 0, c->stream, c->ne, c->N, c->d_tsorted,
                     c->d_doflocs, c->d_cores, ncore, eps_core, eps_clad, k0 * k0, 0.0, 1, c->d_elem);
}

double launch_delta_eps_mass(plfem_ctx* c, int ncore, double eps_core, double eps_clad) {
  unsigned long long* cnt = reinterpret_cast<unsigned long long*>(c->d_counters + 2);
  (void)hipMemsetAsync(cnt, 0, sizeof(unsigned long long), c->stream);
  const int64_t nq = (int64_t)c->ne * 6;
  hipLaunchKernelGGL(k_count_core_qp, dim3((unsigned)((nq + 255) / 256)), dim3(256), 0, c->stream, c->ne, c->N, c->d_tsorted,
                     c->d_doflocs, c->d_cores, ncore, cnt);
  unsigned long long* h = reinterpret_cast<unsigned long long*>(c->h_pinned + PIN_CORE_QP);
  (void)hipMemcpyAsync(h, cnt, sizeof(unsigned long long), hipMemcpyDeviceToHost, c->stream);
  (void)hipStreamSynchronize(c->stream);
  const double frac = (double)*h / (double)nq;
  const double mean = eps_clad + (eps_core - eps_clad) * frac;
  int grid = (c->ne + EPB - 1) / EPB;
  hipLaunchKernelGGL(k_element_matrices<false>, dim3(grid), dim3(256), 0, c->stream, c->ne, c->N, c->d_tsorted,
                     c->d_doflocs, c->d_cores, ncore, eps_core - mean, eps_clad - mean, 0.0, 0.0, 2, c->d_elem);
  launch_csr_gather(c);
  (void)hipMemsetAsync(cnt, 0, sizeof(unsigned long long), c->stream);
  return mean;
}

void launch_pattern_fill(plfem_ctx* c) {
  hipLaunchKernelGGL(k_pattern_fill, dim3((c->N + 127) / 128), dim3(128), 0, c->stream, c->N, c->ne, c->d_nptr, c->d_nadj,
                     c->d_edof, c->d_rowptr, c->d_colind, c->d_slot_row);
}

void launch_csr_gather(plfem_ctx* c) {
  int grid = (c->nnz + 255) / 256;
  hipLaunchKernelGGL(k_csr_gather, dim3(grid), dim3(256), 0, c->stream, c->nnz, c->ne, c->d_slot_row, c->d_colind,
                     c->d_nptr, c->d_nadj, c->d_nloc, c->d_edof, c->d_elem,
                     c->d_vals[0], c->d_vals[1], c->d_vals[2], c->d_vals[3], c->d_vals[4], c->d_vals[5],
                     c->d_vals[6], c->d_vals[7]);
}

void launch_spmv(plfem_ctx* c, int which, int P, const double* x, double* y, int64_t ld) {
  const int grid = spmv_workgroups(c->N);
  if (c->dpn == 2 && which == 0) {
    with_constant<1, BLOCK_P>(P, [&](auto p) {
      hipLaunchKernelGGL(k_spmv_a_block<decltype(p)::value>, dim3(grid), dim3(256), 0, c->stream, c->N, ld, c->d_rowptr,
                         c->d_colind, c->d_bmask, c->d_vals[PLFEM_BLK_AXX], c->d_vals[PLFEM_BLK_AXY], c->d_vals[PLFEM_BLK_AYX],
                         c->d_vals[PLFEM_BLK_AYY], x, y);
    });
    return;
  }
  const double* v = c->d_vals[which == 0 ? PLFEM_BLK_AXX : PLFEM_BLK_MINV];
  with_constant<1, BLOCK_P>(P, [&](auto p) {
    with_constant<1, 2>(c->dpn, [&](auto dpn) {
      hipLaunchKernelGGL((k_spmv_b_block<decltype(p)::value, decltype(dpn)::value>), dim3(grid), dim3(256), 0, c->stream, c->N, ld,
                         c->d_rowptr, c->d_colind, c->d_bmask, v, x, y);
    });
  });
}

int launch_spmv_b_block_il(plfem_ctx* c, const double* xi, double* y, int64_t ld, double* gram) {
  const int grid = spmv_workgroups(c->N);
  with_constant<1, 2>(c->dpn, [&](auto dpn) {
    with_constant<1, 0>(gram != nullptr, [&](auto with_gram) {
      hipLaunchKernelGGL((k_spmv_b_block_il<BLOCK_P, decltype(dpn)::value, decltype(with_gram)::value != 0>), dim3(grid), dim3(256), 0,
                         c->stream, c->N, ld, c->d_rowptr, c->d_colind, c->d_bmask, c->d_vals[PLFEM_BLK_MINV], xi, y, gram);
    });
  });
  return grid;
}

}
```

pl_fem_vectoriel_amd/csrc/kernels_front.hip:

```cpp
#include <algorithm>

#include <type_traits>

#include "device.h"

namespace plfem {
namespace {

typedef double v4d __attribute__((ext_vector_type(4)));

__device__ __forceinline__ double* schur_of(int f, const int64_t* __restrict__ soff, double* __restrict__ schur, int64_t arena) {
  const int level = 31 - __clz(f + 1);
  return schur + (level & 1) * arena + soff[f];
}

template <int sh>
__global__ __launch_bounds__(256) void k_leaf_assemble(
    int first_front, int ne, double sigma, const int32_t* __restrict__ fs2, const int32_t* __restrict__ fm,
    const int64_t* __restrict__ foff, const int64_t* __restrict__ soff,
    const int64_t* __restrict__ fnode_ptr, const int32_t* __restrict__ fnodes,
    const int32_t* __restrict__ leaf_elem_ptr, const int32_t* __restrict__ leaf_elems,
    const int32_t* __restrict__ epos, const double* __restrict__ elem, double* __restrict__ front,
    double* __restrict__ schur, int64_t arena) {
  const int lf = blockIdx.x;
  const int f = first_front + lf;
  const int m = fm[f], s2 = fs2[f], b2 = m - s2;
  constexpr int dpn = sh + 1;
  double* F = front + foff[f];
  double* S = schur_of(f, soff, schur, arena);
  auto at = [&](int i, int j) -> int64_t { return j < s2 ? (int64_t)j * m + i : (i >= s2 ? -2 - ((int64_t)(j - s2) * b2 + (i - s2)) : -1); };
  const int tid = threadIdx.x;
  const int32_t* fn = fnodes + fnode_ptr[f];
  for (int q = tid; q < (m >> sh); q += 256)
    if (fn[q] < 0) {
      for (int cc = 0; cc < dpn; ++cc) {
        const int d = dpn * q + cc;
        if (d < s2) F[(int64_t)d * m + d] = 1.0;
        else S[(int64_t)(d - s2) * b2 + (d - s2)] = 1.0;
      }
    }
  __syncthreads();
  constexpr int nd = 6 * dpn;
  const int adof = tid / nd, bdof = tid % nd;
  const int a = adof >> sh, ca = adof & sh, b = bdof >> sh, cb = bdof & sh;
  const bool worker = tid < nd * nd;
  const int blk_a = (ca == 0 && cb == 0) ? PLFEM_BLK_AXX : (ca == 0) ? PLFEM_BLK_AXY : (cb == 0) ? PLFEM_BLK_AYX : PLFEM_BLK_AYY;
  const bool diag_blk = ca == cb;
  constexpr int EB = 8;
  for (int q0 = leaf_elem_ptr[lf]; q0 < leaf_elem_ptr[lf + 1]; q0 += EB) {
    const int nb = min(EB, leaf_elem_ptr[lf + 1] - q0);
    int64_t dst[EB];
    double val[EB];
#pragma unroll
    for (int t = 0; t < EB; ++t) {
      dst[t] = -1;
      val[t] = 0.0;
      if (worker && t < nb) {
        const int e = leaf_elems[q0 + t];
        const int pa = epos[(size_t)(q0 + t) * 6 + a], pb = epos[(size_t)(q0 + t) * 6 + b];
        const double* em = elem + (size_t)e * ELEM_STRIDE + a * 6 + b;
        double v = em[blk_a * 36];
        if (diag_blk) v -= sigma * em[PLFEM_BLK_MINV * 36];
        if (pa >= 0 && pb >= 0) { dst[t] = at(dpn * pa + ca, dpn * pb + cb); val[t] = v; }
      }
    }
#pragma unroll
    for (int t = 0; t < EB; ++t) {
      if (t < nb) {
        if (dst[t] >= 0) F[dst[t]] += val[t];
        else if (dst[t] <= -2) S[-2 - dst[t]] += val[t];
        __syncthreads();
      }
    }
  }
}

template <int sh>
__global__ __launch_bounds__(256) void k_front_gather(
    const int2* __restrict__ tiles, const int32_t* __restrict__ fs2, const int32_t* __restrict__ fm,
    const int64_t* __restrict__ foff, const int64_t* __restrict__ soff, const int64_t* __restrict__ fnode_ptr,
    const int32_t* __restrict__ fnodes, const int32_t* __restrict__ cinv0, const int32_t* __restrict__ cinv1,
    double* __restrict__ front, double* __restrict__ schur, int64_t arena) {
  const int2 job = tiles[blockIdx.x];
  const int f = job.x;
  const int m = fm[f], s2 = fs2[f], b2 = m - s2;
  constexpr int dpn = sh + 1;
  const int i = (job.y & 0xffff) * 64 + (threadIdx.x & 63);
  const int j0 = ((job.y >> 16) * 4 + (threadIdx.x >> 6)) * 16;
  if (i >= m || j0 >= m) return;
  if (j0 >= s2 && i < s2) return;
  const int64_t np = fnode_ptr[f];
  const int qi = i >> sh, ci = i & sh;
  const int c0i = cinv0[np + qi], c1i = cinv1[np + qi];
  const bool dummy_i = fnodes[np + qi] < 0;
  const int ch0 = 2 * f + 1, ch1 = 2 * f + 2;
  const int b0 = fm[ch0] - fs2[ch0], b1 = fm[ch1] - fs2[ch1];
  const double* S0 = schur_of(ch0, soff, schur, arena);
  const double* S1 = schur_of(ch1, soff, schur, arena);
  double* F = front + foff[f];
  double* S = schur_of(f, soff, schur, arena);
  int c0j[16 >> sh], c1j[16 >> sh];
#pragma unroll
  for (int q = 0; q < (16 >> sh); ++q) {
    c0j[q] = cinv0[np + (j0 >> sh) + q];
    c1j[q] = cinv1[np + (j0 >> sh) + q];
  }
  double v[16];
#pragma unroll
  for (int jj = 0; jj < 16; ++jj) {
    const int cj = jj & sh, q = jj >> sh;
    double a = 0.0, b = 0.0;
    if (c0i >= 0 && c0j[q] >= 0) {
      const int bi = dpn * c0i + ci, bj = dpn * c0j[q] + cj;
      a = S0[(int64_t)min(bi, bj) * b0 + max(bi, bj)];
    }
    if (c1i >= 0 && c1j[q] >= 0) {
      const int bi = dpn * c1i + ci, bj = dpn * c1j[q] + cj;
      b = S1[(int64_t)min(bi, bj) * b1 + max(bi, bj)];
    }
    v[jj] = a + b;
  }
#pragma unroll
  for (int jj = 0; jj < 16; ++jj) {
    const int j = j0 + jj;
    const double val = (dummy_i && i == j) ? 1.0 : v[jj];
    if (j0 < s2) F[(int64_t)j * m + i] = val;
    else S[(int64_t)(j - s2) * b2 + (i - s2)] = val;
  }
}

__device__ __forceinline__ double fast_rcp(double d) {
  double r = __builtin_amdgcn_rcp(d);
  r = fma(fma(-d, r, 1.0), r, r);
  return fma(fma(-d, r, 1.0), r, r);
}

__device__ __forceinline__ double lane_xor16(double v, bool odd_row) {
  const int lo = __double2loint(v), hi = __double2hiint(v);
  const auto a = __builtin_amdgcn_permlane16_swap(lo, lo, false, false);
  const auto b = __builtin_amdgcn_permlane16_swap(hi, hi, false, false);
  return __hiloint2double(odd_row ? b[0] : b[1], odd_row ? a[0] : a[1]);
}

__device__ __forceinline__ void pair_step(double a, double b, double c, double thr, double rep, bool past_first, bool past_second,
                                          double y0, double y1, const double (&ra)[4], const double (&rb)[4],
                                          double (&v)[4], double& d0, double& d1, double& od, int& nper) {
  const double p = b * b;
  const double det = fma(a, c, -p) - fma(b, b, -p);
  const double s = fmax(fmax(fabs(a), fabs(c)), fabs(b));
  if (p * fabs(det) <= (a * a) * (s * s)) {
    if (__builtin_expect(!(fabs(a) >= thr), 0)) {
      a = (a < 0.0) ? -rep : rep;
      nper += 1;
    }
    const double r1 = fast_rcp(a);
    const double g = b * r1;
    double d2 = fma(-g, b, c);
    if (__builtin_expect(!(fabs(d2) >= thr), 0)) {
      d2 = (d2 < 0.0) ? -rep : rep;
      nper += 1;
    }
    const double r2 = fast_rcp(d2);
    const double l0 = past_first ? y0 * r1 : 0.0;
    const double l1 = past_second ? fma(-l0, b, y1) * r2 : 0.0;
#pragma unroll
    for (int cc = 0; cc < 4; ++cc) v[cc] = fma(-l1, fma(-g, ra[cc], rb[cc]), fma(-l0, ra[cc], v[cc]));
    d0 = r1;
    d1 = r2;
    od = 0.0;
    asm volatile("" ::: "memory");
  } else {
    double dt = det;
    if (__builtin_expect(!(fabs(dt) >= thr * s), 0)) {
      dt = (dt < 0.0) ? -rep * s : rep * s;
      nper += 1;
    }
    const double rd = fast_rcp(dt);
    const double x11 = c * rd, x12 = -b * rd, x22 = a * rd;
    const double l0 = past_second ? fma(y0, x11, y1 * x12) : 0.0;
    const double l1 = past_second ? fma(y0, x12, y1 * x22) : 0.0;
#pragma unroll
    for (int cc = 0; cc < 4; ++cc) v[cc] = fma(-l1, rb[cc], fma(-l0, ra[cc], v[cc]));
    d0 = x11;
    d1 = x22;
    od = x12;
    asm volatile("" ::: "memory");
  }
}

struct PivotLds {
  double row[2][2][NB];
  double col[2][2][NB];
  double rmax[NB];
};

__device__ __forceinline__ void ldl_pivot_block(const double* src, int64_t ld, int nbk, int tid,
                                                double (*tile)[NB + 1], double* __restrict__ sDd, double* __restrict__ sDo,
                                                PivotLds& S, int32_t* __restrict__ counters) {
  static_assert(NB == 32, "thread map of ldl_pivot_block");
  const int i = tid & 31, cg = tid >> 5;
  double v[4];
  double rmax = 0.0;
#pragma unroll
  for (int cc = 0; cc < 4; ++cc) {
    const int c = 4 * cg + cc;
    v[cc] = (i < nbk && c < nbk) ? src[(int64_t)c * ld + i] : (i == c ? 1.0 : 0.0);
    rmax = fmax(rmax, fabs(v[cc]));
  }
  __syncthreads();
  tile[cg][i] = rmax;
  __syncthreads();
  if (tid < NB) {
    double r = 0.0;
#pragma unroll
    for (int g = 0; g < 8; ++g) r = fmax(r, fmax(tile[g][tid], tile[g][tid ^ 1]));
    S.rmax[tid] = r;
  }
  double dd = 1.0, od = 0.0;
  int nper = 0;
#pragma unroll
  for (int q = 0; q < NB / 2; ++q) {
    const int k = 2 * q, cgk = k >> 2, pc = k & 3, buf = q & 1;
    if (k >= nbk) break;
    if (cg == cgk) {
      S.col[buf][0][i] = v[pc];
      S.col[buf][1][i] = v[pc + 1];
      v[pc] = (i == k) ? 1.0 : 0.0;
      v[pc + 1] = (i == k + 1) ? 1.0 : 0.0;
    }
    if ((i | 1) == k + 1) {
#pragma unroll
      for (int cc = 0; cc < 4; ++cc) S.row[buf][i & 1][4 * cg + cc] = v[cc];
    }
    __syncthreads();
    const double a = S.col[buf][0][k], b = S.col[buf][0][k + 1], c = S.col[buf][1][k + 1];
    const double thr = fmax(1e-13 * S.rmax[k], 1e-300), rep = fmax(1e-8 * S.rmax[k], 1e-300);
    const double y0 = (i > k) ? S.col[buf][0][i] : 0.0, y1 = (i > k + 1) ? S.col[buf][1][i] : 0.0;
    double ra[4], rb[4];
#pragma unroll
    for (int cc = 0; cc < 4; ++cc) {
      const int cidx = 4 * cg + cc;
      const bool behind = cidx > k + 1;
      ra[cc] = behind ? S.col[buf][0][cidx] : S.row[buf][0][cidx];
      rb[cc] = behind ? S.col[buf][1][cidx] : S.row[buf][1][cidx];
    }
    double d0, d1, o01;
    pair_step(a, b, c, thr, rep, i > k, i > k + 1, y0, y1, ra, rb, v, d0, d1, o01, nper);
    if ((i | 1) == k + 1) {
      dd = (i == k) ? d0 : d1;
      od = o01;
    }
  }
  __syncthreads();
#pragma unroll
  for (int cc = 0; cc < 4; ++cc) {
    const int c = 4 * cg + cc;
    tile[i][c] = (c <= i) ? v[cc] : 0.0;
  }
  if (tid < NB) {
    sDd[i] = dd;
    sDo[i] = od;
  }
  if (tid == 0 && nper > 0 && counters) atomicAdd(&counters[0], nper);
}

__device__ __forceinline__ void store_pivot_results(int f, int k0, int nbk, int64_t np,
                                                    double* __restrict__ dinv, double* __restrict__ delta,
                                                    double (*tile)[NB + 1], const double* __restrict__ sDd,
                                                    const double* __restrict__ sDo) {
  double* D = dinv + (int64_t)f * NB * NB;
  for (int e = threadIdx.x; e < NB * NB; e += 256) D[e] = tile[e & (NB - 1)][e >> 5];
  if ((int)threadIdx.x < nbk)
    reinterpret_cast<double2*>(delta)[2 * np + k0 + threadIdx.x] = make_double2(sDd[threadIdx.x], sDo[threadIdx.x]);
}

struct PanelOperands {
  double xa0[NB / 4], xa1[NB / 4], rdd[2][4], rdo[2][4];
  __device__ __forceinline__ void load(const double (*tile)[NB + 1], const double* sDd, const double* sDo, int nbk, int lr, int lk) {
#pragma unroll
    for (int kk = 0; kk < NB / 4; ++kk) {
      xa0[kk] = tile[lr][4 * kk + lk];
      xa1[kk] = tile[16 + lr][4 * kk + lk];
    }
#pragma unroll
    for (int tc = 0; tc < 2; ++tc)
#pragma unroll
      for (int r = 0; r < 4; ++r) {
        const int c = 16 * tc + lk + 4 * r;
        rdd[tc][r] = (c < nbk) ? sDd[c] : 0.0;
        rdo[tc][r] = (c < nbk) ? sDo[c] : 0.0;
      }
  }
  __device__ __forceinline__ void rows(const double (&b)[NB / 4], int nbk, int kcol, int64_t m, int i, int lk,
                                       double* __restrict__ W, double* __restrict__ Y, double* __restrict__ F) const {
    v4d y0 = (v4d){0.0, 0.0, 0.0, 0.0}, y1 = (v4d){0.0, 0.0, 0.0, 0.0};
#pragma unroll
    for (int kk = 0; kk < NB / 4; ++kk) {
      y0 = __builtin_amdgcn_mfma_f64_16x16x4f64(xa0[kk], b[kk], y0, 0, 0, 0);
      y1 = __builtin_amdgcn_mfma_f64_16x16x4f64(xa1[kk], b[kk], y1, 0, 0, 0);
    }
#pragma unroll
    for (int tc = 0; tc < 2; ++tc)
#pragma unroll
      for (int r = 0; r < 4; ++r) {
        const int c = 16 * tc + lk + 4 * r;
        const double y = tc == 0 ? y0[r] : y1[r];
        const double w = fma(y, rdd[tc][r], lane_xor16(y, lk & 1) * rdo[tc][r]);
        W[(int64_t)c * m + i] = w;
        Y[(int64_t)c * m + i] = y;
        if (c < nbk) F[(int64_t)(kcol + c) * m + i] = w;
      }
  }
};

__global__ __launch_bounds__(256) void k_ldl_first_panel(const FrontRec* __restrict__ frec, double* __restrict__ front,
                                                         double* __restrict__ dinv, double* __restrict__ delta,
                                                         double* __restrict__ wbuf, double* __restrict__ rbuf,
                                                         int32_t* __restrict__ counters) {
  const FrontRec R = frec[blockIdx.x];
  const int f = R.f;
  const int s2 = R.s2;
  const int nbk = min(NB, s2);
  const int m = R.m;
  double* F = front + R.foff;
  const int wave = threadIdx.x >> 6, lane = threadIdx.x & 63;
  const int bx = blockIdx.y;
  const int n_pan = gridDim.y;
  const int t0 = nbk;
  if (bx > 0 && t0 + bx * 64 >= m) return;
  __shared__ __attribute__((aligned(16))) PivotLds piv;
  __shared__ double tile[NB][NB + 1];
  __shared__ double sDd[NB], sDo[NB];
  const int lr = lane & 15, lk = lane >> 4;
  double b[NB / 4];
  {
    const int ibase = t0 + bx * 64 + 16 * wave;
#pragma unroll
    for (int kk = 0; kk < NB / 4; ++kk) {
      const int jx = 4 * kk + lk;
      b[kk] = (ibase < m && jx < nbk) ? F[(int64_t)jx * m + ibase + lr] : 0.0;
    }
  }
  ldl_pivot_block(F, m, nbk, threadIdx.x, tile, sDd, sDo, piv, bx == 0 ? counters : nullptr);
  __syncthreads();
  if (bx == 0) store_pivot_results(f, 0, nbk, R.np, dinv, delta, tile, sDd, sDo);
  double* W = wbuf + 2 * R.np * NB;
  double* Y = rbuf + 2 * R.np * NB;
  PanelOperands po;
  po.load(tile, sDd, sDo, nbk, lr, lk);
  for (int ch = bx; t0 + ch * 64 < m; ch += n_pan) {
    const int ibase = t0 + ch * 64 + 16 * wave;
    if (ibase >= m) break;
    const int i = ibase + lr;
    if (ch != bx) {
#pragma unroll
      for (int kk = 0; kk < NB / 4; ++kk) {
        const int jx = 4 * kk + lk;
        b[kk] = (jx < nbk) ? F[(int64_t)jx * m + i] : 0.0;
      }
    }
    po.rows(b, nbk, 0, m, i, lk, W, Y, F);
  }
}

__device__ __forceinline__ void ldl_invrow_block(int f, int bx, int kb, const int32_t* __restrict__ fs2,
                                                 const int32_t* __restrict__ fm, const int64_t* __restrict__ foff,
                                                 double* __restrict__ front, const double* __restrict__ dinv,
                                                 double* __restrict__ part ) {
  const int s2 = fs2[f];
  const int k0 = kb * NB;
  if (k0 >= s2 || k0 == 0) return;
  const int wave = threadIdx.x >> 6, lane = threadIdx.x & 63;
  const int c0 = bx * 16;
  if (c0 >= k0) return;
  const int nbk = min(NB, s2 - k0);
  const int m = fm[f];
  double* F = front + foff[f];
  const double* D = dinv + (int64_t)f * NB * NB;
  const int lr = lane & 15, lk = lane >> 4;
  const int c = c0 + lr;
  v4d t0 = (v4d){0.0, 0.0, 0.0, 0.0}, t1 = (v4d){0.0, 0.0, 0.0, 0.0};
  auto groups = [&](int j0, auto G_) {
    constexpr int G = decltype(G_)::value;
    double a0[4 * G], a1[4 * G], b[4 * G];
#pragma unroll
    for (int t = 0; t < 4 * G; ++t) {
      const int j = j0 + 4 * t + lk;
      a0[t] = F[(int64_t)j * m + k0 + lr];
      a1[t] = (nbk > 16) ? F[(int64_t)j * m + k0 + 16 + lr] : 0.0;
      b[t] = (j >= c) ? F[(int64_t)j * m + c] : 0.0;
    }
#pragma unroll
    for (int t = 0; t < 4 * G; ++t) {
      t0 = __builtin_amdgcn_mfma_f64_16x16x4f64(a0[t], b[t], t0, 0, 0, 0);
      t1 = __builtin_amdgcn_mfma_f64_16x16x4f64(a1[t], b[t], t1, 0, 0, 0);
    }
  };
  const int ngroups = (k0 - c0) / 16;
  int j0 = c0 + 16 * (wave * ngroups / 4);
  const int j_end = c0 + 16 * ((wave + 1) * ngroups / 4);
  for (; j0 + 16 < j_end; j0 += 32) groups(j0, std::integral_constant<int, 2>());
  if (j0 < j_end) groups(j0, std::integral_constant<int, 1>());
  if (wave > 0) {
#pragma unroll
    for (int r = 0; r < 4; ++r) {
      part[((wave - 1) * 8 + r) * 64 + lane] = t0[r];
      part[((wave - 1) * 8 + 4 + r) * 64 + lane] = t1[r];
    }
  }
  __syncthreads();
  if (wave > 0) return;
#pragma unroll
  for (int w = 0; w < 3; ++w)
#pragma unroll
    for (int r = 0; r < 4; ++r) {
      t0[r] += part[(w * 8 + r) * 64 + lane];
      t1[r] += part[(w * 8 + 4 + r) * 64 + lane];
    }
  v4d x0 = (v4d){0.0, 0.0, 0.0, 0.0}, x1 = (v4d){0.0, 0.0, 0.0, 0.0};
#pragma unroll
  for (int kk = 0; kk < 8; ++kk) {
    const int q = 4 * kk + lk;
    const double a0 = -D[(int64_t)q * NB + lr];
    const double a1 = -D[(int64_t)q * NB + 16 + lr];
    const double b = kk < 4 ? t0[kk & 3] : t1[kk & 3];
    x0 = __builtin_amdgcn_mfma_f64_16x16x4f64(a0, b, x0, 0, 0, 0);
    x1 = __builtin_amdgcn_mfma_f64_16x16x4f64(a1, b, x1, 0, 0, 0);
  }
#pragma unroll
  for (int r = 0; r < 4; ++r) {
    const int r0 = lk + 4 * r, r1 = 16 + lk + 4 * r;
    if (r0 < nbk) F[(int64_t)(k0 + r0) * m + c] = x0[r];
    if (r1 < nbk) F[(int64_t)(k0 + r1) * m + c] = x1[r];
  }
}

template <int MODE>
__device__ __forceinline__ void ldl_update_tile(const int2 job, int kb, const int32_t* __restrict__ fs2,
                                                const int32_t* __restrict__ fm, const int64_t* __restrict__ foff,
                                                const int64_t* __restrict__ soff, const int64_t* __restrict__ fnode_ptr,
                                                double* __restrict__ front, double* __restrict__ schur, int64_t arena,
                                                const double* __restrict__ wbuf, const double* __restrict__ rbuf,
                                                const double* __restrict__ wbuf_prev, const double* __restrict__ rbuf_prev) {
  const int f = job.x;
  const int s2 = fs2[f];
  const int k0 = kb * NB;
  if (k0 >= s2) return;
  const int m = fm[f];
  const int nbk = min(NB, s2 - k0);
  const int t0 = k0 + nbk;
  const int wave = threadIdx.x >> 6, lane = threadIdx.x & 63;
  const int i0 = t0 + ((job.y & 0xffff) * 2 + (wave & 1)) * 32;
  const int j0 = t0 + ((job.y >> 16) * 2 + (wave >> 1)) * 32;
  if (i0 >= m || j0 >= m) return;
  if (i0 < j0) return;
  const int ncol = (t0 < s2 && j0 == t0) ? min(NB, s2 - t0) : 0;
  if ((MODE == 0 && t0 < s2) || ncol == NB) return;
  double* F = front + foff[f];
  double* S = schur_of(f, soff, schur, arena);
  const int b2 = m - s2;
// ... 374 lines not shown
```

pl_fem_vectoriel_amd/csrc/kernels_lanczos.hip:

```cpp
#include <algorithm>
#include <cmath>
#include <functional>

#include "device.h"
#include "p2_element.h"

namespace plfem {
namespace {

typedef double v4d __attribute__((ext_vector_type(4)));
constexpr int CHUNK = PANEL_CHUNK;

__global__ __launch_bounds__(256) void k_scale_store(int64_t n, const double* __restrict__ w,
                                                     const double* __restrict__ bw, const double* __restrict__ beta2,
                                                     double* __restrict__ v, double* __restrict__ bv,
                                                     double* __restrict__ beta_out) {
  const double b2 = *beta2;
  const double beta = sqrt(fmax(b2, 0.0));
  const double inv = beta > 0.0 ? 1.0 / beta : 0.0;
  const int64_t i = (int64_t)blockIdx.x * 256 + threadIdx.x;
  if (i == 0 && beta_out) *beta_out = beta;
  if (i >= n) return;
  v[i] = w[i] * inv;
  bv[i] = bw[i] * inv;
}

__global__ __launch_bounds__(256) void k_axpby(int64_t n, double a, const double* __restrict__ x, double b,
                                               const double* __restrict__ y, double* __restrict__ z) {
  const int64_t i = (int64_t)blockIdx.x * 256 + threadIdx.x;
  if (i < n) z[i] = a * x[i] + b * y[i];
}

template <int P, int CW>
__global__ __launch_bounds__(256) void k_panel_dot_p(int64_t n, int ncols, int nchunks, const double* __restrict__ Pm,
                                                     const double* __restrict__ W, int64_t ldw,
                                                     double* __restrict__ partial) {
  const int c0 = (blockIdx.y * 4 + (threadIdx.x >> 6)) * CW;
  if (c0 >= ncols) return;
  const int lane = threadIdx.x & 63;
  const int64_t i0 = (int64_t)blockIdx.x * CHUNK;
  const int64_t i1 = min(n, i0 + CHUNK);
  const double* col[CW];
#pragma unroll
  for (int t = 0; t < CW; ++t) col[t] = Pm + (int64_t)min(c0 + t, ncols - 1) * n;
  double acc[CW][P];
#pragma unroll
  for (int t = 0; t < CW; ++t)
#pragma unroll
    for (int q = 0; q < P; ++q) acc[t][q] = 0.0;
  int64_t i = i0 + lane;
  for (; i + 64 < i1; i += 128) {
    double a[2][CW], w[2][P];
#pragma unroll
    for (int h = 0; h < 2; ++h) {
#pragma unroll
      for (int t = 0; t < CW; ++t) a[h][t] = col[t][i + 64 * h];
#pragma unroll
      for (int q = 0; q < P; ++q) w[h][q] = W[(int64_t)q * ldw + i + 64 * h];
    }
#pragma unroll
    for (int h = 0; h < 2; ++h)
#pragma unroll
      for (int t = 0; t < CW; ++t)
#pragma unroll
        for (int q = 0; q < P; ++q) acc[t][q] += a[h][t] * w[h][q];
  }
  for (; i < i1; i += 64) {
    double w[P];
#pragma unroll
    for (int q = 0; q < P; ++q) w[q] = W[(int64_t)q * ldw + i];
#pragma unroll
    for (int t = 0; t < CW; ++t) {
      const double a = col[t][i];
#pragma unroll
      for (int q = 0; q < P; ++q) acc[t][q] += a * w[q];
    }
  }
#pragma unroll
  for (int t = 0; t < CW; ++t) {
#pragma unroll
    for (int q = 0; q < P; ++q) {
      double v = acc[t][q];
      for (int off = 32; off >= 1; off >>= 1) v += __shfl_xor(v, off);
      if (lane == 0 && c0 + t < ncols) partial[((int64_t)(c0 + t) * P + q) * nchunks + blockIdx.x] = v;
    }
  }
}

__global__ __launch_bounds__(64) void k_panel_dot_finish_p(int P, int nchunks, const double* __restrict__ partial,
                                                           double* __restrict__ h, int ldh, double* __restrict__ hacc,
                                                           int ldacc) {
  const int cq = blockIdx.x;
  const int c = cq / P, q = cq % P;
  double acc = 0.0;
  for (int t = threadIdx.x; t < nchunks; t += 64) acc += partial[(int64_t)cq * nchunks + t];
  for (int off = 32; off >= 1; off >>= 1) acc += __shfl_xor(acc, off);
  if (threadIdx.x == 0) {
    h[c + (int64_t)q * ldh] = acc;
    if (hacc) hacc[c + (int64_t)q * ldacc] += acc;
  }
}

template <int P>
__global__ __launch_bounds__(256) void k_panel_axpy_p(int64_t n, int ncols, const double* __restrict__ Pm,
                                                      const double* __restrict__ H, int ldh, double* __restrict__ W,
                                                      int64_t ldw, double* __restrict__ wil, int N, int dpn) {
  extern __shared__ double sh[];
  for (int k = threadIdx.x; k < ncols * P; k += 256) sh[k] = H[(k / P) + (int64_t)(k % P) * ldh];
  __syncthreads();
  const int64_t i = (int64_t)blockIdx.x * 256 + threadIdx.x;
  if (i >= n) return;
  double acc[P];
#pragma unroll
  for (int q = 0; q < P; ++q) acc[q] = 0.0;
  for (int c = 0; c < ncols; ++c) {
    const double a = Pm[(int64_t)c * n + i];
#pragma unroll
    for (int q = 0; q < P; ++q) acc[q] += a * sh[c * P + q];
  }
  double w[P];
#pragma unroll
  for (int q = 0; q < P; ++q) {
    w[q] = W[(int64_t)q * ldw + i] - acc[q];
    W[(int64_t)q * ldw + i] = w[q];
  }
  if (wil) {
    const int comp = (int)(i / N), node = (int)(i - (int64_t)comp * N);
    double* d = wil + ((int64_t)node * dpn + comp) * P;
#pragma unroll
    for (int q = 0; q < P; ++q) d[q] = w[q];
  }
}


template <int P>
__global__ __launch_bounds__(FIRST_THREADS) void k_permute_dot_first(int64_t n2, int N, int nseg, int ncols, const int32_t* __restrict__ npos,
                                                          const double* __restrict__ xl, double* __restrict__ W, int64_t ldw,
                                                          const double* __restrict__ Pm, double* __restrict__ partial) {
  constexpr int CW = FIRST_COLS, V = CW * P, NT = FIRST_THREADS, NW = NT / 64;
  static_assert(V <= 64 && (V & (V - 1)) == 0 && FIRST_ROWS % NT == 0 && NW == 4, "multi_reduce<V>; whole rows per thread; four waves meet");
  __shared__ double red[NW][V];
  const int seg = blockIdx.x, wave = threadIdx.x >> 6, lane = threadIdx.x & 63;
  double acc[V];
#pragma unroll
  for (int v = 0; v < V; ++v) acc[v] = 0.0;
  const double* col[CW];
#pragma unroll
  for (int t = 0; t < CW; ++t) col[t] = Pm + (int64_t)min(t, ncols - 1) * n2;
  constexpr int RPT = FIRST_ROWS / NT;
  int64_t g[RPT];
  int pos[RPT];
  double a[RPT][CW], w[RPT][P];
#pragma unroll
  for (int j = 0; j < RPT; ++j) {
    g[j] = (int64_t)seg * FIRST_ROWS + j * NT + threadIdx.x;
    const bool on = g[j] < n2;
    const int c = on && g[j] >= N;
    pos[j] = on ? npos[(int)(g[j] - (int64_t)c * N)] : -1;
#pragma unroll
    for (int t = 0; t < CW; ++t) a[j][t] = on ? col[t][g[j]] : 0.0;
  }
#pragma unroll
  for (int j = 0; j < RPT; ++j) {
    const int c = g[j] >= N;
#pragma unroll
    for (int q = 0; q < P; ++q) w[j][q] = pos[j] >= 0 ? xl[((int64_t)pos[j] + c) * P + q] : 0.0;
  }
#pragma unroll
  for (int j = 0; j < RPT; ++j) {
    if (g[j] < n2) {
#pragma unroll
      for (int q = 0; q < P; ++q) W[(int64_t)q * ldw + g[j]] = w[j][q];
    }
#pragma unroll
    for (int t = 0; t < CW; ++t)
#pragma unroll
      for (int q = 0; q < P; ++q) acc[t * P + q] = fma(a[j][t], w[j][q], acc[t * P + q]);
  }
  multi_reduce<V, true>(acc, lane);
  if ((lane & (64 / V - 1)) == 0) red[wave][multi_reduce_index<V, true>(lane)] = acc[0];
  __syncthreads();
  if ((int)threadIdx.x < V) {
    const int v = threadIdx.x, t = v / P;
    if (t < ncols) partial[(int64_t)v * nseg + seg] = (red[0][v] + red[1][v]) + (red[2][v] + red[3][v]);
  }
}

template <int P>
__global__ __launch_bounds__(256) void k_axpy_first(int64_t n, int ncols, int nseg, const double* __restrict__ Pm,
                                                    const double* __restrict__ partial, double* __restrict__ Hout, int ldh,
                                                    double* __restrict__ W, int64_t ldw) {
  constexpr int CW = 8;
  __shared__ double sh[CW * P];
  {
    const int v = threadIdx.x >> 3, part = threadIdx.x & 7;
    double x = 0.0;
    if (v / P < ncols) {
      const double* pp = partial + (int64_t)v * nseg;
      int k = part;
      for (; k + 7 * 8 < nseg; k += 8 * 8) {
        double t[8];
#pragma unroll
        for (int u = 0; u < 8; ++u) t[u] = pp[k + 8 * u];
#pragma unroll
        for (int u = 0; u < 8; ++u) x += t[u];
      }
      for (; k < nseg; k += 8) x += pp[k];
    }
    x += __shfl_xor(x, 1, 8);
    x += __shfl_xor(x, 2, 8);
    x += __shfl_xor(x, 4, 8);
    if (part == 0) {
      sh[v] = x;
      if (blockIdx.x == 0 && v / P < ncols) Hout[(v / P) + (int64_t)(v % P) * ldh] = x;
    }
  }
  __syncthreads();
  const int64_t i = (int64_t)blockIdx.x * 256 + threadIdx.x;
  if (i >= n) return;
  double a[CW];
#pragma unroll
  for (int t = 0; t < CW; ++t) a[t] = Pm[(int64_t)min(t, ncols - 1) * n + i];
  double acc[P];
#pragma unroll
  for (int q = 0; q < P; ++q) acc[q] = 0.0;
#pragma unroll
  for (int t = 0; t < CW; ++t)
    if (t < ncols) {
#pragma unroll
      for (int q = 0; q < P; ++q) acc[q] = fma(a[t], sh[t * P + q], acc[q]);
    }
#pragma unroll
  for (int q = 0; q < P; ++q) W[(int64_t)q * ldw + i] -= acc[q];
}

template <int P>
__global__ __launch_bounds__(64 * P * P > 1024 ? 1024 : 64 * P * P) void k_chol_small(const double* __restrict__ G, int ldg, const double* __restrict__ partial,
                                                           int nchunks, double* __restrict__ Tblk, int ldT,
                                                           double* __restrict__ Rinv, int32_t* __restrict__ counters) {
  __shared__ double sG[P * P];
  if (G) {
    if (threadIdx.x < P * P) sG[threadIdx.x] = G[(threadIdx.x % P) + (int64_t)(threadIdx.x / P) * ldg];
  } else {
    const int lane = threadIdx.x & 63;
    for (int cq = threadIdx.x >> 6; cq < P * P; cq += blockDim.x >> 6) {
      const double* pp = partial + (int64_t)cq * nchunks;
      double acc = 0.0;
      int t = lane;
      for (; t + 7 * 64 < nchunks; t += 8 * 64) {
        double v[8];
#pragma unroll
        for (int u = 0; u < 8; ++u) v[u] = pp[t + 64 * u];
#pragma unroll
        for (int u = 0; u < 8; ++u) acc += v[u];
      }
      for (; t < nchunks; t += 64) acc += pp[t];
      for (int off = 32; off >= 1; off >>= 1) acc += __shfl_xor(acc, off);
      if (lane == 0) sG[(cq / P) + (cq % P) * P] = acc;
    }
  }
  __syncthreads();
  if (threadIdx.x != 0) return;
  ldg = P;
  G = sG;
  double R[P][P], X[P][P];
  for (int i = 0; i < P; ++i)
    for (int j = 0; j < P; ++j) { R[i][j] = 0.0; X[i][j] = 0.0; }
  for (int j = 0; j < P; ++j) {
    for (int i = 0; i <= j; ++i) {
      double v = 0.5 * (G[i + (int64_t)j * ldg] + G[j + (int64_t)i * ldg]);
      for (int k = 0; k < i; ++k) v -= R[k][i] * R[k][j];
      if (i == j) {
        if (!(v > 0.0)) { atomicAdd(&counters[2], 1); v = 1.0; }
        R[j][j] = sqrt(v);
      } else {
        R[i][j] = v / R[i][i];
      }
    }
  }
  for (int j = 0; j < P; ++j) {
    X[j][j] = 1.0 / R[j][j];
    for (int i = j - 1; i >= 0; --i) {
      double v = 0.0;
      for (int k = i + 1; k <= j; ++k) v -= R[i][k] * X[k][j];
      X[i][j] = v / R[i][i];
    }
  }
  for (int i = 0; i < P; ++i)
    for (int j = 0; j < P; ++j) {
      Tblk[i + (int64_t)j * ldT] = R[i][j];
      Rinv[i + j * P] = X[i][j];
    }
}

template <int P>
__global__ __launch_bounds__(256) void k_block_scale(int64_t n, const double* __restrict__ W, const double* __restrict__ BW,
                                                     int64_t ldw, const double* __restrict__ Rinv,
                                                     double* __restrict__ Vn, double* __restrict__ BVn, int64_t ldv,
                                                     const double* __restrict__ exp_src, int exp_n, double* __restrict__ exp_dst,
                                                     const int32_t* __restrict__ cnt_src, int32_t* __restrict__ cnt_dst,
                                                     double* __restrict__ bv_front, const int32_t* __restrict__ npos, int N) {
  __shared__ double X[P * P];
  if (threadIdx.x < P * P) X[threadIdx.x] = Rinv[threadIdx.x];
  if (blockIdx.x == 0 && exp_dst) {
    for (int t = threadIdx.x; t < exp_n; t += 256) exp_dst[t] = exp_src[t];
    if (threadIdx.x < 4) cnt_dst[threadIdx.x] = cnt_src[threadIdx.x];
  }
  __syncthreads();
  const int64_t i = (int64_t)blockIdx.x * 256 + threadIdx.x;
  if (i >= n) return;
  double w[P], bw[P];
#pragma unroll
  for (int q = 0; q < P; ++q) { w[q] = W[(int64_t)q * ldw + i]; bw[q] = BW[(int64_t)q * ldw + i]; }
  int64_t fo = -1;
  if (bv_front) {
    const int c = i >= N;
    const int pos = npos[(int)(i - (int64_t)c * N)];
    if (pos >= 0) fo = ((int64_t)pos + c) * P;
  }
#pragma unroll
  for (int q = 0; q < P; ++q) {
    double a = 0.0, b = 0.0;
#pragma unroll
    for (int k = 0; k <= q; ++k) { a += w[k] * X[k + q * P]; b += bw[k] * X[k + q * P]; }
    Vn[(int64_t)q * ldv + i] = a;
    BVn[(int64_t)q * ldv + i] = b;
    if (fo >= 0) bv_front[fo + q] = b;
  }
}

__global__ __launch_bounds__(256) void k_rotate(int64_t n, int m, int p, const double* __restrict__ V,
                                                const double* __restrict__ Smat, int ldS, double* __restrict__ out) {
  extern __shared__ double sS[];
  const int mpad = (m + 3) & ~3, ppad = (p + 15) & ~15;
  for (int k = threadIdx.x; k < mpad * ppad; k += 256) {
    int r = k / ppad, c = k % ppad;
    sS[k] = (r < m && c < p) ? Smat[(int64_t)c * ldS + r] : 0.0;
  }
  __syncthreads();
  const int wave = threadIdx.x >> 6, lane = threadIdx.x & 63;
  const int64_t i0 = ((int64_t)blockIdx.x * 4 + wave) * 16;
  if (i0 >= n) return;
  const int lr = lane & 15, lk = lane >> 4;
  const int64_t row = i0 + lr;
  const bool rv = row < n;
  for (int c0 = 0; c0 < ppad; c0 += 16) {
    v4d acc = (v4d){0.0, 0.0, 0.0, 0.0};
    for (int kk = 0; kk < mpad; kk += 4) {
      int k = kk + lk;
      double a = sS[k * ppad + c0 + lr];
      double b = (rv && k < m) ? V[(int64_t)k * n + row] : 0.0;
      acc = __builtin_amdgcn_mfma_f64_16x16x4f64(a, b, acc, 0, 0, 0);
    }
#pragma unroll
    for (int r = 0; r < 4; ++r) {
      int oc = c0 + lk + 4 * r;
      if (rv && oc < p) out[(int64_t)oc * n + row] = acc[r];
    }
  }
}

__global__ __launch_bounds__(256) void k_core_mask(int N, const double* __restrict__ doflocs,
                                                   const double* __restrict__ cores, int ncore,
                                                   const uint8_t* __restrict__ bmask, uint8_t* __restrict__ mask,
                                                   int32_t* __restrict__ counters) {
  const int i = blockIdx.x * 256 + threadIdx.x;
  bool counted = false;
  if (i < N) {
    const bool in = in_any_core(doflocs[i], doflocs[N + i], cores, ncore);
    mask[i] = in ? 1 : 0;
    counted = in && !bmask[i];
  }
  unsigned long long b = __ballot(counted);
  if ((threadIdx.x & 63) == 0 && b) atomicAdd(&counters[1], (int)__popcll(b));
}

constexpr int POST_MB = 4;
template <int DPN>
__global__ __launch_bounds__(256) void k_post_sums(int N, int k, int nblocks, const int32_t* __restrict__ rowptr,
                                                   const int32_t* __restrict__ colind, const double* __restrict__ dxx,
                                                   const double* __restrict__ dxy, const double* __restrict__ dyy,
                                                   const uint8_t* __restrict__ mask, const double* __restrict__ evecs,
                                                   double* __restrict__ partial) {
  constexpr int MB = POST_MB;
  const int mode0 = blockIdx.y * MB;
  const int nm = min(MB, k - mode0);
  const double* vx[MB];
#pragma unroll
  for (int j = 0; j < MB; ++j) vx[j] = evecs + (int64_t)min(mode0 + j, k - 1) * DPN * N;
  const int64_t yoff = DPN == 2 ? N : 0;
  __shared__ double red[4][MB][5];
  double acc[MB][5];
#pragma unroll
  for (int j = 0; j < MB; ++j)
#pragma unroll
    for (int t = 0; t < 5; ++t) acc[j][t] = 0.0;
  const int sub = threadIdx.x & 7;
  for (int rr = threadIdx.x >> 3; rr < POST_ROWS; rr += 32) {
    int row = blockIdx.x * POST_ROWS + rr;
    if (row >= N) break;
    double px[MB], py[MB];
#pragma unroll
    for (int j = 0; j < MB; ++j) { px[j] = 0.0; py[j] = 0.0; }
    int q1 = rowptr[row + 1];
    for (int q = rowptr[row] + sub; q < q1; q += 8) {
      int c = colind[q];
      const double a = dxx[q];
      if (DPN == 1) {
#pragma unroll
        for (int j = 0; j < MB; ++j) px[j] += a * vx[j][c];
        continue;
      }
      const double b = dxy[q], d = dyy[q];
#pragma unroll
      for (int j = 0; j < MB; ++j) {
        double ux = vx[j][c], uy = vx[j][yoff + c];
        px[j] += a * ux + 2.0 * b * uy;
        py[j] += d * uy;
      }
    }
    const bool msk = mask[row] != 0;
#pragma unroll
    for (int j = 0; j < MB; ++j) {
      double x = vx[j][row], y = DPN == 2 ? vx[j][yoff + row] : 0.0;
      acc[j][4] += x * px[j] + y * py[j];
      if (sub == 0) {
        acc[j][0] += x * x;
        acc[j][1] += y * y;
        if (msk) { acc[j][2] += x * x; acc[j][3] += y * y; }
      }
    }
  }
#pragma unroll
  for (int j = 0; j < MB; ++j)
#pragma unroll
    for (int t = 0; t < 5; ++t) {
      double v = acc[j][t];
      for (int off = 32; off >= 1; off >>= 1) v += __shfl_xor(v, off);
      if ((threadIdx.x & 63) == 0) red[threadIdx.x >> 6][j][t] = v;
    }
  __syncthreads();
  if ((int)threadIdx.x < 5 * nm) {
    const int j = threadIdx.x / 5, t = threadIdx.x % 5;
    partial[((int64_t)(mode0 + j) * nblocks + blockIdx.x) * 5 + t] = red[0][j][t] + red[1][j][t] + red[2][j][t] + red[3][j][t];
  }
}

__global__ __launch_bounds__(64) void k_post_finish(int k, int nblocks, const double* __restrict__ partial,
                                                    double* __restrict__ out) {
  const int t = blockIdx.x;
  const int mode = t / 5, q = t % 5;
  double acc = 0.0;
  for (int b = threadIdx.x; b < nblocks; b += 64) acc += partial[((int64_t)mode * nblocks + b) * 5 + q];
  for (int off = 32; off >= 1; off >>= 1) acc += __shfl_xor(acc, off);
  if (threadIdx.x == 0) out[t] = acc;
}

__global__ __launch_bounds__(256) void k_post_scale(int N, int dpn, const double* __restrict__ sums, double* __restrict__ evecs) {
  const int mode = blockIdx.y;
  const double n2 = dpn == 2 ? sums[mode * 5 + 0] + sums[mode * 5 + 1] : sums[mode * 5 + 4];
  const double nrm = sqrt(n2) + 1e-30;
  const double inv = 1.0 / nrm;
  double* v = evecs + (int64_t)mode * dpn * N;
  const int64_t i = (int64_t)blockIdx.x * 256 + threadIdx.x;
  if (i < dpn * (int64_t)N) v[i] *= inv;
}

__global__ __launch_bounds__(256) void k_gather_interior(int N, int nsolve, int dpn, const int32_t* __restrict__ interior,
                                                         const double* __restrict__ evecs,
                                                         double* __restrict__ modes_int) {
  const int mode = blockIdx.y;
  const int64_t i = (int64_t)blockIdx.x * 256 + threadIdx.x;
  if (i >= dpn * (int64_t)nsolve) return;
  int comp = i >= nsolve ? 1 : 0;
  int q = (int)(i - (int64_t)comp * nsolve);
  modes_int[(int64_t)mode * dpn * nsolve + i] = evecs[(int64_t)mode * dpn * N + (int64_t)comp * N + interior[q]];
}

template <int DPN>
__global__ __launch_bounds__(256) void k_resid_sums(int N, int k, int nblocks, const int32_t* __restrict__ rowptr,
                                                    const int32_t* __restrict__ colind, const uint8_t* __restrict__ bmask,
                                                    const double* __restrict__ vxx, const double* __restrict__ vxy,
                                                    const double* __restrict__ vyx, const double* __restrict__ vyy,
                                                    const double* __restrict__ vm, const double* __restrict__ lam,
                                                    const double* __restrict__ evecs, double* __restrict__ partial) {
  constexpr int MB = POST_MB;
  const int mode0 = blockIdx.y * MB;
  const int nm = min(MB, k - mode0);
  const double* vx[MB];
  double l[MB];
#pragma unroll
  for (int j = 0; j < MB; ++j) {
    const int mode = min(mode0 + j, k - 1);
    vx[j] = evecs + (int64_t)mode * DPN * N;
    l[j] = lam[mode];
  }
  const int64_t yoff = DPN == 2 ? N : 0;
  __shared__ double red[4][MB][2];
  double r2[MB], a2[MB];
#pragma unroll
  for (int j = 0; j < MB; ++j) { r2[j] = 0.0; a2[j] = 0.0; }
  const int sub = threadIdx.x & 7;
  for (int rr = threadIdx.x >> 3; rr < POST_ROWS; rr += 32) {
    const int row = blockIdx.x * POST_ROWS + rr;
    if (row >= N) break;
    if (bmask[row]) continue;
    double ax[MB], ay[MB], bx[MB], by[MB];
#pragma unroll
    for (int j = 0; j < MB; ++j) { ax[j] = 0; ay[j] = 0; bx[j] = 0; by[j] = 0; }
    const int q1 = rowptr[row + 1];
    for (int q = rowptr[row] + sub; q < q1; q += 8) {
      const int c = colind[q];
      const double axx = vxx[q], m = vm[q];
      if (DPN == 1) {
#pragma unroll
        for (int j = 0; j < MB; ++j) { const double ux = vx[j][c]; ax[j] += axx * ux; bx[j] += m * ux; }
        continue;
      }
      const double axy = vxy[q], ayx = vyx[q], ayy = vyy[q];
#pragma unroll
      for (int j = 0; j < MB; ++j) {
        const double ux = vx[j][c], uy = vx[j][yoff + c];
        ax[j] += axx * ux + axy * uy;
        ay[j] += ayx * ux + ayy * uy;
        bx[j] += m * ux;
        by[j] += m * uy;
      }
    }
#pragma unroll
    for (int j = 0; j < MB; ++j) {
#pragma unroll
      for (int off = 4; off >= 1; off >>= 1) {
        ax[j] += __shfl_xor(ax[j], off, 8); ay[j] += __shfl_xor(ay[j], off, 8);
        bx[j] += __shfl_xor(bx[j], off, 8); by[j] += __shfl_xor(by[j], off, 8);
      }
      if (sub == 0) {
        const double rx = ax[j] - l[j] * bx[j], ry = ay[j] - l[j] * by[j];
        r2[j] += rx * rx + ry * ry;
        a2[j] += ax[j] * ax[j] + ay[j] * ay[j];
      }
    }
  }
#pragma unroll
  for (int j = 0; j < MB; ++j) {
    for (int off = 32; off >= 1; off >>= 1) { r2[j] += __shfl_xor(r2[j], off); a2[j] += __shfl_xor(a2[j], off); }
    if ((threadIdx.x & 63) == 0) { red[threadIdx.x >> 6][j][0] = r2[j]; red[threadIdx.x >> 6][j][1] = a2[j]; }
  }
  __syncthreads();
  if ((int)threadIdx.x < 2 * nm) {
    const int j = threadIdx.x >> 1, t = threadIdx.x & 1;
    partial[((int64_t)(mode0 + j) * nblocks + blockIdx.x) * 2 + t] = red[0][j][t] + red[1][j][t] + red[2][j][t] + red[3][j][t];
  }
}

__global__ __launch_bounds__(64) void k_resid_finish(int nblocks, const double* __restrict__ partial, double* __restrict__ out) {
  const int t = blockIdx.x;
  const int mode = t >> 1, q = t & 1;
  double acc = 0.0;
  for (int b = threadIdx.x; b < nblocks; b += 64) acc += partial[((int64_t)mode * nblocks + b) * 2 + q];
  for (int off = 32; off >= 1; off >>= 1) acc += __shfl_xor(acc, off);
  if (threadIdx.x == 0) out[t] = acc;
}

}


void resid_enqueue(plfem_ctx* c, int k, const double* lam_host, const double* evecs) {
  hipStream_t st = c->stream;
  const int N = c->N;
  const int nblocks = post_blocks(N);
  double* hs = c->h_pinned + PIN_RESID;
  for (int i = 0; i < k; ++i) hs[i] = lam_host[i];
  (void)hipMemcpyAsync(c->d_hacc, hs, sizeof(double) * k, hipMemcpyHostToDevice, st);
  double* partial = c->d_post + c->post_doubles;
  double* sums = partial + (int64_t)k * nblocks * RESID_SUMS;
  with_constant<1, 2>(c->dpn, [&](auto dpn) {
    hipLaunchKernelGGL(k_resid_sums<decltype(dpn)::value>, dim3(nblocks, (k + POST_MB - 1) / POST_MB), dim3(256), 0, st, N, k, nblocks,
                       c->d_rowptr, c->d_colind, c->d_bmask, c->d_vals[PLFEM_BLK_AXX], c->d_vals[PLFEM_BLK_AXY],
                       c->d_vals[PLFEM_BLK_AYX], c->d_vals[PLFEM_BLK_AYY], c->d_vals[PLFEM_BLK_MINV], c->d_hacc, evecs, partial);
  });
  hipLaunchKernelGGL(k_resid_finish, dim3(RESID_SUMS * k), dim3(64), 0, st, nblocks, partial, sums);
  (void)hipMemcpyAsync(hs + k, sums, sizeof(double) * RESID_SUMS * k, hipMemcpyDeviceToHost, st);
}

void resid_finish(plfem_ctx* c, int k, double* out_host) {
  const double* hs = c->h_pinned + PIN_RESID;
  for (int i = 0; i < k; ++i) {
    const double r2 = hs[k + 2 * i], a2 = hs[k + 2 * i + 1];
    out_host[i] = a2 > 0.0 ? std::sqrt(r2 / a2) : (r2 > 0.0 ? INFINITY : 0.0);
  }
}

void launch_residuals(plfem_ctx* c, int k, const double* lam_host, const double* evecs, double* out_host) {
  resid_enqueue(c, k, lam_host, evecs);
  (void)hipStreamSynchronize(c->stream);
  resid_finish(c, k, out_host);
}

void launch_axpby(plfem_ctx* c, int64_t n, double a, const double* x, double b, const double* y, double* z) {
  hipLaunchKernelGGL(k_axpby, dim3((unsigned)((n + 255) / 256)), dim3(256), 0, c->stream, n, a, x, b, y, z);
}

void launch_scale_store(plfem_ctx* c, const double* w, const double* bw, const double* beta2, double* v, double* bv,
                        double* beta_out) {
  hipLaunchKernelGGL(k_scale_store, dim3((unsigned)((c->n2 + 255) / 256)), dim3(256), 0, c->stream, c->n2, w, bw,
                     beta2, v, bv, beta_out);
}

void launch_panel_dot(plfem_ctx* c, int P, const double* Pm, int ncols, const double* W, int64_t ldw, double* h, int ldh,
                      double* hacc, int ldacc) {
  const int nchunks = panel_chunks(c->n2);
  with_constant<1, BLOCK_P>(P, [&](auto p) {
    constexpr int PT = decltype(p)::value, CW = PT == 1 ? 1 : 4;
    hipLaunchKernelGGL((k_panel_dot_p<PT, CW>), dim3(nchunks, (ncols + 4 * CW - 1) / (4 * CW)), dim3(256), 0, c->stream, c->n2,
                       ncols, nchunks, Pm, W, ldw, c->d_partial);
    hipLaunchKernelGGL(k_panel_dot_finish_p, dim3(ncols * PT), dim3(64), 0, c->stream, PT, nchunks, c->d_partial, h, ldh,
                       hacc, ldacc);
  });
}

void launch_panel_axpy(plfem_ctx* c, int P, const double* Pm, int ncols, const double* H, int ldh, double* W, int64_t ldw,
                       double* w_interleaved) {
  with_constant<1, BLOCK_P>(P, [&](auto p) {
    constexpr int PT = decltype(p)::value;
    hipLaunchKernelGGL(k_panel_axpy_p<PT>, dim3((unsigned)((c->n2 + 255) / 256)), dim3(256), sizeof(double) * ncols * PT,
                       c->stream, c->n2, ncols, Pm, H, ldh, W, ldw, w_interleaved, c->N, c->dpn);
  });
}

void launch_dot(plfem_ctx* c, const double* a, const double* b, double* out) { launch_panel_dot(c, 1, a, 1, b, c->n2, out, 1); }

void launch_first_pass_block(plfem_ctx* c, const double* BVm, const double* Vm, int ncols, double* W, int64_t ldw, double* Hout,
                             int ldh) {
  constexpr int P = BLOCK_P;
  const int nseg = first_pass_segments(c->n2);
  hipLaunchKernelGGL(k_permute_dot_first<P>, dim3(nseg), dim3(FIRST_THREADS), 0, c->stream, c->n2, c->N, nseg, ncols, c->d_npos, c->d_xl, W, ldw,
                     BVm, c->d_partial);
  hipLaunchKernelGGL(k_axpy_first<P>, dim3((unsigned)((c->n2 + 255) / 256)), dim3(256), 0, c->stream, c->n2, ncols, nseg, Vm,
                     c->d_partial, Hout, ldh, W, ldw);
}

void launch_chol_block(plfem_ctx* c, const double* G, int ldg, double* Tblk, int ldT, double* Rinv) {
  hipLaunchKernelGGL(k_chol_small<BLOCK_P>, dim3(1), dim3(64), 0, c->stream, G, ldg, (const double*)nullptr, 0, Tblk, ldT,
                     Rinv, c->d_counters);
}

void launch_chol_from_partials(plfem_ctx* c, int nchunks, double* Tblk, int ldT, double* Rinv) {
  constexpr int P = BLOCK_P;
  hipLaunchKernelGGL(k_chol_small<P>, dim3(1), dim3(std::min(1024, 64 * P * P)), 0, c->stream, (const double*)nullptr, 0, c->d_partial, nchunks,
                     Tblk, ldT, Rinv, c->d_counters);
}

void launch_block_scale(plfem_ctx* c, const double* W, const double* BW, int64_t ldw, const double* Rinv, double* Vn,
                        double* BVn, int64_t ldv, const double* exp_src, int exp_n, double* exp_dst, int32_t* cnt_dst,
                        double* bv_front) {
  hipLaunchKernelGGL(k_block_scale<BLOCK_P>, dim3((unsigned)((c->n2 + 255) / 256)), dim3(256), 0, c->stream, c->n2, W,
                     BW, ldw, Rinv, Vn, BVn, ldv, exp_src, exp_n, exp_dst, c->d_counters, cnt_dst, bv_front, c->d_npos, c->N);
}

__global__ __launch_bounds__(256) void k_start_field(int nsolve, int N, int dpn, int64_t ld, int nvec,
                                                     const int32_t* __restrict__ interior, double* __restrict__ out) {
  const int64_t e = (int64_t)blockIdx.x * 256 + threadIdx.x;
  if (e >= (int64_t)nvec * dpn * nsolve) return;
  uint64_t k = (uint64_t)e + 1, am = 1, ap = 0, cm = 6364136223846793005ull, cp = 1442695040888963407ull;
  while (k) {
    if (k & 1) { am *= cm; ap = ap * cm + cp; }
    cp = (cm + 1) * cp;
    cm *= cm;
    k >>= 1;
  }
  const uint64_t s = am * 0x9E3779B97F4A7C15ull + ap;
  const int q = (int)(e / (dpn * (int64_t)nsolve));
  const int r = (int)(e - (int64_t)q * dpn * nsolve);
  const int comp = r >= nsolve, i = r - comp * nsolve;
  out[(int64_t)q * ld + (int64_t)comp * N + interior[i]] = ((double)(s >> 11) / 9007199254740992.0) * 2.0 - 1.0;
}

void launch_start_field(plfem_ctx* c, int nvec, double* out) {
  (void)hipMemsetAsync(out, 0, sizeof(double) * c->n2 * nvec, c->stream);
  const int64_t total = (int64_t)nvec * c->dpn * c->nsolve;
  hipLaunchKernelGGL(k_start_field, dim3((unsigned)((total + 255) / 256)), dim3(256), 0, c->stream, c->nsolve, c->N, c->dpn,
                     c->n2, nvec, c->d_interior, out);
}

void launch_rotate(plfem_ctx* c, const double* V, int m, const double* Smat, int ldS, int p, double* out) {
  const int mpad = (m + 3) & ~3;
  const int chunk = std::max(16, ((64 * 1024) / (8 * mpad)) & ~15);
  unsigned grid = (unsigned)((c->n2 + 63) / 64);
  for (int p0 = 0; p0 < p; p0 += chunk) {
    const int pc = std::min(chunk, p - p0);
    const size_t lds = sizeof(double) * mpad * ((pc + 15) & ~15);
    hipLaunchKernelGGL(k_rotate, dim3(grid), dim3(256), lds, c->stream, c->n2, m, pc, V, Smat + (size_t)p0 * ldS, ldS,
                       out + (size_t)p0 * c->n2);
  }
}

constexpr int POST_GROUP = 8;
void post_enqueue(plfem_ctx* c, int k, double* evecs, int ncore, double* modes_int, const std::function<void(int, int)>* group_done) {
  hipStream_t st = c->stream;
  const int N = c->N;
  (void)hipMemsetAsync(c->d_counters + 1, 0, sizeof(int32_t), st);
  hipLaunchKernelGGL(k_core_mask, dim3((N + 255) / 256), dim3(256), 0, st, N, c->d_doflocs, c->d_cores, ncore,
                     c->d_bmask, c->d_coremask, c->d_counters);
  const int nblocks = post_blocks(N);
  const int group = group_done ? POST_GROUP : k;
  for (int g0 = 0; g0 < k; g0 += group) {
    const int kg = std::min(group, k - g0);
    double* ev = evecs + (int64_t)g0 * c->n2;
    double* partial = c->d_post + (int64_t)g0 * nblocks * POST_SUMS;
    double* sums = c->d_post + (int64_t)k * nblocks * POST_SUMS + (int64_t)g0 * POST_SUMS;
    const double* dxx = c->d_vals[c->dpn == 1 ? PLFEM_BLK_MINV : PLFEM_BLK_DXX];
    with_constant<1, 2>(c->dpn, [&](auto dpn) {
      hipLaunchKernelGGL(k_post_sums<decltype(dpn)::value>, dim3(nblocks, (kg + POST_MB - 1) / POST_MB), dim3(256), 0, st, N, kg, nblocks,
// ... 43 lines not shown
```

pl_fem_vectoriel_amd/csrc/kernels_sweep.hip:

```cpp
#include <algorithm>

#include "device.h"

namespace plfem {
namespace {

struct SweepArgs {
  int leaf_level;
  int ldv;
  int sh;
  const int32_t *cinv0, *cinv1, *prow;
  const double* front;
  const double2* dinv2;
  double *fr, *u0, *u1, *ys, *xl;
};

template <int P, bool SOA>
__device__ __forceinline__ int sidx(int i, int u, int ldv) { return SOA ? u * ldv + i : i * P + u; }

template <int P>
struct FwdStage {
  double a[P], b0[P], b1[P];
  int c0, c1;
  __device__ __forceinline__ void request(const SweepArgs& A, int64_t np, int i, bool on) {
    c0 = c1 = -1;
#pragma unroll
    for (int u = 0; u < P; ++u) { a[u] = 0.0; b0[u] = 0.0; b1[u] = 0.0; }
    if (!on) return;
    const int64_t e = (2 * np + i) * P;
#pragma unroll
    for (int u = 0; u < P; ++u) a[u] = A.fr[e + u];
    if (!A.leaf_level) {
      c0 = A.cinv0[np + (i >> A.sh)];
      c1 = A.cinv1[np + (i >> A.sh)];
#pragma unroll
      for (int u = 0; u < P; ++u) { b0[u] = A.u0[e + u]; b1[u] = A.u1[e + u]; }
    }
  }
  __device__ __forceinline__ double value(int u) const {
    return a[u] + (c0 >= 0 ? b0[u] : 0.0) + (c1 >= 0 ? b1[u] : 0.0);
  }
};

template <int P, bool SOA>
__device__ __forceinline__ void stage_fwd(const SweepArgs& A, double* sv, int64_t np, int need, int T, int tid,
                                          FwdStage<P>& first) {
  for (int i = tid + T; i < need; i += T) {
    FwdStage<P> s;
    s.request(A, np, i, true);
#pragma unroll
    for (int u = 0; u < P; ++u) sv[sidx<P, SOA>(i, u, A.ldv)] = s.value(u);
  }
  first.request(A, np, tid, tid < need);
}

template <int P>
struct FwdOut {
  double w0[P], w1[P];
  int c0, c1;
  int64_t dst;
  __device__ __forceinline__ void request(const SweepArgs& A, int64_t npp, int64_t np, int s2, int m, int r) {
    c0 = c1 = -1;
    dst = -1;
#pragma unroll
    for (int u = 0; u < P; ++u) { w0[u] = 0.0; w1[u] = 0.0; }
    if (r >= m || r < s2) return;
    const int pr = A.prow[np + (r >> A.sh)];
    if (!A.leaf_level) {
      c0 = A.cinv0[np + (r >> A.sh)];
      c1 = A.cinv1[np + (r >> A.sh)];
      const int64_t e = (2 * np + r) * P;
#pragma unroll
      for (int u = 0; u < P; ++u) { w0[u] = A.u0[e + u]; w1[u] = A.u1[e + u]; }
    }
    if (pr >= 0) dst = (2 * npp + (pr << A.sh) + (r & A.sh)) * P;
  }
  __device__ __forceinline__ double w(int u) const { return (c0 >= 0 ? w0[u] : 0.0) + (c1 >= 0 ? w1[u] : 0.0); }
};

template <int P, int NW, int TBF>
__device__ __forceinline__ void fwd_tile_body(const SweepArgs& A, const SweepJob& J, double* __restrict__ sv, double* __restrict__ red) {
  const int f = J.f, m = J.m, s2 = J.s2;
  const int r0 = (J.rb & ~SWEEP_ROW_JOB_FLAG) * 64;
  const int64_t np = J.np;
  const int tid = threadIdx.x, wave = tid >> 6, lane = tid & 63;
  const int need = (r0 + 64 <= s2) ? r0 + 64 : s2;
  const int r = r0 + lane;
  const bool valid = r < m;
  const int h = lane >> 5, ra = r0 + 2 * (lane & 31), rb = ra + 1;
  const bool pvalid = ra < m;
  const int cea = pvalid ? ((ra < s2) ? ra + 1 : s2) : 0;
  const int ceb = pvalid ? ((rb < s2) ? rb + 1 : s2) : 0;
  const double* p = A.front + J.foff + ra;
  FwdOut<P> out;
  if (wave == 0) out.request(A, J.npp, np, s2, m, r);
  FwdStage<P> st;
  stage_fwd<P, false>(A, sv, np, need, NW * 64, tid, st);
  double2 a0[TBF];
#pragma unroll
  for (int t = 0; t < TBF; ++t) {
    const int c = 2 * (wave + NW * t) + h;
    a0[t] = (c < ceb) ? *reinterpret_cast<const double2*>(p + (int64_t)c * m) : make_double2(0.0, 0.0);
  }
  if (tid < need) {
#pragma unroll
    for (int u = 0; u < P; ++u) sv[tid * P + u] = st.value(u);
  }
  __syncthreads();
  double acc[2][P];
#pragma unroll
  for (int u = 0; u < P; ++u) { acc[0][u] = 0.0; acc[1][u] = 0.0; }
#pragma unroll
  for (int t = 0; t < TBF; ++t) {
    const int c = 2 * (wave + NW * t) + h;
    if (c < ceb) {
      const double ax = (c < cea) ? a0[t].x : 0.0;
#pragma unroll
      for (int u = 0; u < P; ++u) {
        const double v = sv[c * P + u];
        acc[0][u] += ax * v;
        acc[1][u] += a0[t].y * v;
      }
    }
  }
  for (int c0 = 2 * NW * TBF; c0 < ceb; c0 += 2 * NW * TBF) {
    double2 a[TBF];
#pragma unroll
    for (int t = 0; t < TBF; ++t) {
      const int c = c0 + 2 * (wave + NW * t) + h;
      a[t] = (c < ceb) ? *reinterpret_cast<const double2*>(p + (int64_t)c * m) : make_double2(0.0, 0.0);
    }
#pragma unroll
    for (int t = 0; t < TBF; ++t) {
      const int c = c0 + 2 * (wave + NW * t) + h;
      if (c < ceb) {
        const double ax = (c < cea) ? a[t].x : 0.0;
#pragma unroll
        for (int u = 0; u < P; ++u) {
          const double v = sv[c * P + u];
          acc[0][u] += ax * v;
          acc[1][u] += a[t].y * v;
        }
      }
    }
  }
#pragma unroll
  for (int u = 0; u < P; ++u) {
    acc[0][u] += __shfl_xor(acc[0][u], 32);
    acc[1][u] += __shfl_xor(acc[1][u], 32);
  }
  if (h == 0) {
#pragma unroll
    for (int u = 0; u < P; ++u)
      *reinterpret_cast<double2*>(&red[(wave * P + u) * 64 + 2 * lane]) = make_double2(acc[0][u], acc[1][u]);
  }
  __syncthreads();
  if (wave == 0 && valid) {
    double tot[P];
#pragma unroll
    for (int u = 0; u < P; ++u) {
      double t = 0.0;
#pragma unroll
      for (int w = 0; w < NW; ++w) t += red[(w * P + u) * 64 + lane];
      tot[u] = t;
    }
    if (r < s2) {
#pragma unroll
      for (int u = 0; u < P; ++u) A.ys[(2 * np + r) * P + u] = tot[u];
    } else if (out.dst >= 0) {
      double* d = ((f & 1) ? A.u0 : A.u1) + out.dst;
#pragma unroll
      for (int u = 0; u < P; ++u) d[u] = out.w(u) - tot[u];
    }
  }
}

template <int P, int NW, int R, int LOADS>
__device__ __forceinline__ void fwd_rows_body(const SweepArgs& A, const SweepJob& J, double* __restrict__ sv) {
  constexpr int RB = NW * R, UNR = LOADS / R, V = R * P;
  const int f = J.f, m = J.m, s2 = J.s2;
  const int j0 = (J.rb & ~SWEEP_ROW_JOB_FLAG) * RB;
  const int64_t np = J.np;
  const int tid = threadIdx.x, wave = tid >> 6, lane = tid & 63;
  const int need = min(s2, j0 + RB);
  const double* F = A.front + J.foff;
  int ce[R], cmax = 0;
  const double* rowp[R];
#pragma unroll
  for (int q = 0; q < R; ++q) {
    const int r = j0 + wave + NW * q;
    ce[q] = r < m ? ((r < s2) ? r + 1 : s2) : 0;
    cmax = max(cmax, ce[q]);
    rowp[q] = r < s2 ? F + (int64_t)r * m : F + (int64_t)m * s2 + (int64_t)(r - s2) * s2;
  }
  const int oidx = multi_reduce_index<V>(lane & (V - 1));
  const int orow = j0 + wave + NW * (oidx / P);
  FwdOut<P> out;
  out.request(A, J.npp, np, s2, m, lane < V ? orow : m);
  FwdStage<P> st;
  stage_fwd<P, true>(A, sv, np, need, NW * 64, tid, st);
  double2 a0[UNR][R];
#pragma unroll
  for (int t = 0; t < UNR; ++t) {
    const int i = 128 * t + 2 * lane;
#pragma unroll
    for (int q = 0; q < R; ++q) a0[t][q] = (i < ce[q]) ? *reinterpret_cast<const double2*>(rowp[q] + i) : make_double2(0.0, 0.0);
  }
  if (tid < need) {
#pragma unroll
    for (int u = 0; u < P; ++u) sv[u * A.ldv + tid] = st.value(u);
  }
  __syncthreads();
  double acc[V];
#pragma unroll
  for (int v = 0; v < V; ++v) acc[v] = 0.0;
#define PLFEM_FWD_ROWS_CONSUME(a, c)                                                                   \
  _Pragma("unroll") for (int t = 0; t < UNR; ++t) {                                                    \
    const int i = (c) + 128 * t + 2 * lane;                                                            \
    if (i < cmax) {                                                                                    \
      _Pragma("unroll") for (int u = 0; u < P; ++u) {                                                  \
        const double2 vi = *reinterpret_cast<const double2*>(&sv[u * A.ldv + i]);                      \
        _Pragma("unroll") for (int q = 0; q < R; ++q) {                                                \
          const double ay = (i + 1 < ce[q]) ? a[t][q].y : 0.0;                                         \
          acc[q * P + u] = fma(ay, vi.y, fma(a[t][q].x, vi.x, acc[q * P + u]));                        \
        }                                                                                              \
      }                                                                                                \
    }                                                                                                  \
  }
  PLFEM_FWD_ROWS_CONSUME(a0, 0)
  for (int c = 128 * UNR; c < cmax; c += 128 * UNR) {
    double2 a[UNR][R];
#pragma unroll
    for (int t = 0; t < UNR; ++t) {
      const int i = c + 128 * t + 2 * lane;
#pragma unroll
      for (int q = 0; q < R; ++q) a[t][q] = (i < ce[q]) ? *reinterpret_cast<const double2*>(rowp[q] + i) : make_double2(0.0, 0.0);
    }
    PLFEM_FWD_ROWS_CONSUME(a, c)
  }
#undef PLFEM_FWD_ROWS_CONSUME
  multi_reduce<V>(acc, lane);
  if (lane < V && orow < m) {
    const int u = oidx % P;
    if (orow < s2) {
      A.ys[(2 * np + orow) * P + u] = acc[0];
    } else if (out.dst >= 0) {
      double wu = out.w(0);
#pragma unroll
      for (int q = 1; q < P; ++q) wu = (u == q) ? out.w(q) : wu;
      (((f & 1) ? A.u0 : A.u1) + out.dst)[u] = wu - acc[0];
    }
  }
}

template <int P>
struct BwdStage {
  double v[P];
  int pr, i;
  bool own, on;
  __device__ __forceinline__ void request_index(const SweepArgs& A, int64_t np, int s2, int i_, bool on_) {
    i = i_;
    on = on_;
    own = i < s2;
    pr = -1;
    if (on && !own) pr = A.prow[np + (i >> A.sh)];
    if (on && own) {
      const double2 d = A.dinv2[2 * np + i];
#pragma unroll
      for (int u = 0; u < P; ++u) v[u] = fma(d.x, A.ys[(2 * np + i) * P + u], d.y * A.ys[(2 * np + (i ^ 1)) * P + u]);
    }
  }
  __device__ __forceinline__ void request_value(const SweepArgs& A, int64_t npp) {
    if (on && !own) {
#pragma unroll
      for (int u = 0; u < P; ++u) v[u] = pr >= 0 ? -A.xl[(2 * npp + (pr << A.sh) + (i & A.sh)) * P + u] : 0.0;
    }
  }
  template <bool SOA>
  __device__ __forceinline__ void finish(const SweepArgs& A, double* sv, int64_t np, bool publish) const {
    if (!on) return;
#pragma unroll
    for (int u = 0; u < P; ++u) sv[sidx<P, SOA>(i, u, A.ldv)] = v[u];
    if (publish && !own) {
#pragma unroll
      for (int u = 0; u < P; ++u) A.xl[(2 * np + i) * P + u] = -v[u];
    }
  }
};

template <int P, bool SOA>
__device__ __forceinline__ void stage_bwd_rest(const SweepArgs& A, double* sv, int lo, int m, int s2, int64_t np,
                                               int64_t npp, int T, int tid, bool publish) {
  for (int i = lo + tid + T; i < m; i += T) {
    BwdStage<P> s;
    s.request_index(A, np, s2, i, true);
    s.request_value(A, npp);
    s.template finish<SOA>(A, sv, np, publish);
  }
}

template <int P, int NW, int TBB>
__device__ __forceinline__ void bwd_tile_body(const SweepArgs& A, const SweepJob& J, double* __restrict__ sv, double* __restrict__ red) {
  const int rb = J.rb, m = J.m, s2 = J.s2;
  const int r0 = rb * 64;
  const int64_t np = J.np;
  const int64_t npp = J.npp;
  const int tid = threadIdx.x, wave = tid >> 6, lane = tid & 63;
  const bool publish = rb == 0 && !A.leaf_level;
  BwdStage<P> st;
  st.request_index(A, np, s2, r0 + tid, r0 + tid < m);
  const int r = r0 + lane;
  const bool valid = r < s2;
  const int h = lane >> 5, ra = r0 + 2 * (lane & 31);
  const bool pvalid = ra < s2;
  const double* p = A.front + J.foff + ra;
  const double* pz = A.front + J.foff + (int64_t)m * s2 + ra - (int64_t)s2 * s2;
  auto entry = [&](int i) { return *reinterpret_cast<const double2*>(i < s2 ? p + (int64_t)i * m : pz + (int64_t)i * s2); };
  const int cb = pvalid ? ra : m, ce = m;
  const int slot = 2 * wave + h;
  const int cstart = cb + ((slot - cb) & (2 * NW - 1));
  double2 a0[TBB];
#pragma unroll
  for (int t = 0; t < TBB; ++t) a0[t] = (cstart + 2 * NW * t < ce) ? entry(cstart + 2 * NW * t) : make_double2(0.0, 0.0);
  st.request_value(A, npp);
  stage_bwd_rest<P, false>(A, sv, r0, m, s2, np, npp, NW * 64, tid, publish);
  st.template finish<false>(A, sv, np, publish);
  __syncthreads();
  double acc[2][P];
#pragma unroll
  for (int u = 0; u < P; ++u) { acc[0][u] = 0.0; acc[1][u] = 0.0; }
#pragma unroll
  for (int t = 0; t < TBB; ++t) {
    const int c = cstart + 2 * NW * t;
    if (c < ce) {
      const double ay = (c > ra) ? a0[t].y : 0.0;
#pragma unroll
      for (int u = 0; u < P; ++u) {
        const double v = sv[c * P + u];
        acc[0][u] += a0[t].x * v;
        acc[1][u] += ay * v;
      }
    }
  }
  for (int c0 = cstart + 2 * NW * TBB; c0 < ce; c0 += 2 * NW * TBB) {
    double2 a[TBB];
#pragma unroll
    for (int t = 0; t < TBB; ++t) a[t] = (c0 + 2 * NW * t < ce) ? entry(c0 + 2 * NW * t) : make_double2(0.0, 0.0);
#pragma unroll
    for (int t = 0; t < TBB; ++t) {
      const int c = c0 + 2 * NW * t;
      if (c < ce) {
#pragma unroll
        for (int u = 0; u < P; ++u) {
          const double v = sv[c * P + u];
          acc[0][u] += a[t].x * v;
          acc[1][u] += a[t].y * v;
        }
      }
    }
  }
#pragma unroll
  for (int u = 0; u < P; ++u) {
    acc[0][u] += __shfl_xor(acc[0][u], 32);
    acc[1][u] += __shfl_xor(acc[1][u], 32);
  }
  if (h == 0) {
#pragma unroll
    for (int u = 0; u < P; ++u)
      *reinterpret_cast<double2*>(&red[(wave * P + u) * 64 + 2 * lane]) = make_double2(acc[0][u], acc[1][u]);
  }
  __syncthreads();
  if (wave == 0 && valid) {
#pragma unroll
    for (int u = 0; u < P; ++u) {
      double t = 0.0;
#pragma unroll
      for (int w = 0; w < NW; ++w) t += red[(w * P + u) * 64 + lane];
      A.xl[(2 * np + r) * P + u] = t;
    }
  }
}

template <int P, int NW, int R, int LOADS>
__device__ __forceinline__ void bwd_rows_body(const SweepArgs& A, const SweepJob& J, double* __restrict__ sv) {
  constexpr int RB = NW * R, UNR = LOADS / R, V = R * P;
  const int rb = J.rb, m = J.m, s2 = J.s2;
  const int j0 = rb * RB;
  const int64_t np = J.np;
  const int64_t npp = J.npp;
  const int tid = threadIdx.x, wave = tid >> 6, lane = tid & 63;
  const bool publish = rb == 0 && !A.leaf_level;
  const int lo = j0 & ~63;
  BwdStage<P> st;
  st.request_index(A, np, s2, lo + tid, lo + tid < m);
  const double* F = A.front + J.foff;
  int jq[R];
#pragma unroll
  for (int q = 0; q < R; ++q) {
    const int j = j0 + wave + NW * q;
    jq[q] = j < s2 ? j : m;
  }
  const int c0 = (j0 + wave) & ~63;
  double2 a0[UNR][R];
#pragma unroll
  for (int t = 0; t < UNR; ++t) {
    const int i = c0 + 128 * t + 2 * lane;
#pragma unroll
    for (int q = 0; q < R; ++q) a0[t][q] = (i < m && i + 1 >= jq[q]) ? *reinterpret_cast<const double2*>(F + i + (int64_t)jq[q] * m) : make_double2(0.0, 0.0);
  }
  st.request_value(A, npp);
  stage_bwd_rest<P, true>(A, sv, lo, m, s2, np, npp, NW * 64, tid, publish);
  st.template finish<true>(A, sv, np, publish);
  __syncthreads();
  const int oidx = multi_reduce_index<V>(lane & (V - 1));
  const int oj = j0 + wave + NW * (oidx / P);
  double acc[V];
#pragma unroll
  for (int v = 0; v < V; ++v) acc[v] = 0.0;
#define PLFEM_BWD_ROWS_CONSUME(a, c)                                                                   \
  _Pragma("unroll") for (int t = 0; t < UNR; ++t) {                                                    \
    const int i = (c) + 128 * t + 2 * lane;                                                            \
    if (i < m) {                                                                                       \
      _Pragma("unroll") for (int u = 0; u < P; ++u) {                                                  \
        const double2 vi = *reinterpret_cast<const double2*>(&sv[u * A.ldv + i]);                      \
        _Pragma("unroll") for (int q = 0; q < R; ++q) {                                                \
          const double ax = (i >= jq[q]) ? a[t][q].x : 0.0;                                            \
          acc[q * P + u] = fma(a[t][q].y, vi.y, fma(ax, vi.x, acc[q * P + u]));                        \
        }                                                                                              \
      }                                                                                                \
    }                                                                                                  \
  }
  PLFEM_BWD_ROWS_CONSUME(a0, c0)
  for (int c = c0 + 128 * UNR; c < m; c += 128 * UNR) {
    double2 a[UNR][R];
#pragma unroll
    for (int t = 0; t < UNR; ++t) {
      const int i = c + 128 * t + 2 * lane;
#pragma unroll
      for (int q = 0; q < R; ++q) a[t][q] = (i < m && i + 1 >= jq[q]) ? *reinterpret_cast<const double2*>(F + i + (int64_t)jq[q] * m) : make_double2(0.0, 0.0);
    }
    PLFEM_BWD_ROWS_CONSUME(a, c)
  }
#undef PLFEM_BWD_ROWS_CONSUME
  multi_reduce<V>(acc, lane);
  if (lane < V && oj < s2) A.xl[(2 * np + oj) * P + oidx % P] = acc[0];
}

template <int P, int R, int LD>
__global__ __launch_bounds__(512) void k_fwd_rows(const SweepJob* __restrict__ blk, SweepArgs A) {
  extern __shared__ __attribute__((aligned(16))) double sv[];
  const SweepJob job = blk[blockIdx.x];
  fwd_rows_body<P, 8, R, LD>(A, job, sv);
}

template <int P, int R, int LD>
__global__ __launch_bounds__(512) void k_bwd_rows(const SweepJob* __restrict__ blk, SweepArgs A) {
  extern __shared__ __attribute__((aligned(16))) double sv[];
  const SweepJob job = blk[blockIdx.x];
  bwd_rows_body<P, 8, R, LD>(A, job, sv);
}

template <int P, int LD>
__global__ __launch_bounds__(256) void k_fwd(const SweepJob* __restrict__ blk, SweepArgs A) {
  extern __shared__ __attribute__((aligned(16))) double sv[];
  __shared__ __attribute__((aligned(16))) double red[4 * P * 64];
  const SweepJob job = blk[blockIdx.x];
  fwd_tile_body<P, 4, LD>(A, job, sv, red);
}

template <int P, int LD>
__global__ __launch_bounds__(256) void k_fwd_mix(const SweepJob* __restrict__ blk, SweepArgs A) {
  extern __shared__ __attribute__((aligned(16))) double sv[];
  __shared__ __attribute__((aligned(16))) double red[4 * P * 64];
  const SweepJob job = blk[blockIdx.x];
  if (job.rb & SWEEP_ROW_JOB_FLAG) fwd_rows_body<P, 4, 4, LD>(A, job, sv);
  else fwd_tile_body<P, 4, LD>(A, job, sv, red);
}

template <int P, int LD>
__global__ __launch_bounds__(512) void k_bwd(const SweepJob* __restrict__ blk, SweepArgs A) {
  extern __shared__ __attribute__((aligned(16))) double sv[];
  __shared__ __attribute__((aligned(16))) double red[8 * P * 64];
  const SweepJob job = blk[blockIdx.x];
  bwd_tile_body<P, 8, LD>(A, job, sv, red);
}

template <int P>
__global__ __launch_bounds__(256) void k_permute_in(int64_t n2, int N, const int32_t* __restrict__ npos,
                                                    const double* __restrict__ rhs, int64_t ldx, double* __restrict__ fr) {
  const int64_t g = (int64_t)blockIdx.x * 256 + threadIdx.x;
  if (g >= n2) return;
  const int c = g >= N, node = (int)(g - (int64_t)c * N);
  const int pos = npos[node];
  if (pos < 0) return;
#pragma unroll
  for (int u = 0; u < P; ++u) fr[((int64_t)pos + c) * P + u] = rhs[(int64_t)u * ldx + g];
}

template <int P>
__global__ __launch_bounds__(256) void k_permute_out(int64_t n2, int N, const int32_t* __restrict__ npos,
                                                     const double* __restrict__ xl, double* __restrict__ x, int64_t ldx) {
  const int64_t g = (int64_t)blockIdx.x * 256 + threadIdx.x;
  if (g >= n2) return;
  const int c = g >= N, node = (int)(g - (int64_t)c * N);
  const int pos = npos[node];
#pragma unroll
  for (int u = 0; u < P; ++u) x[(int64_t)u * ldx + g] = pos >= 0 ? xl[((int64_t)pos + c) * P + u] : 0.0;
}

template <int P>
void sweeps(plfem_ctx* c) {
  hipStream_t st = c->stream;
  SweepArgs A;
  A.sh = c->sh;
  A.cinv0 = c->d_cinv0; A.cinv1 = c->d_cinv1; A.prow = c->d_prow;
  A.front = c->d_front; A.dinv2 = reinterpret_cast<const double2*>(c->d_delta);
  A.fr = c->d_fvec; A.u0 = c->d_u0; A.u1 = c->d_u1; A.ys = c->d_fvec2; A.xl = c->d_xl;
// ... 76 lines not shown
```

Measured before the change: 542.0.

## Replace ds_bpermute wave shuffles with DPP and permlane swap reductions

Adds lane_xor helpers that implement butterfly exchanges with DPP row operations (offsets 1-8) and permlane16/32 swaps (offsets 16/32) instead of __shfl_xor, which goes through LDS bpermute. The helpers are applied to wave and group-of-8 reductions across the assembly, Lanczos panel/gram, residual, front and sweep kernels, and the panel dot kernel switches to a multi-value transpose reduction (multi_reduce) instead of one full wave reduction per accumulator. k_resid_sums is made branch-uniform so every lane joins the shuffles. A debug hook is added to test the new lane ops, and the risk is correctness of the DPP control encodings and lane-half selection.

```diff
diff --git a/include/plfem.h b/include/plfem.h
--- a/include/plfem.h
+++ b/include/plfem.h
@@ -255,6 +255,8 @@
                             int32_t want_front);
 int plfem_debug_rotate(plfem_ctx* ctx, const double* V, int32_t m, const double* S, int32_t ldS, int32_t p, double* out);
 int plfem_debug_start_field(plfem_ctx* ctx, int32_t nvec, double* out);
+enum { PLFEM_DEBUG_LANE_XOR = 0, PLFEM_DEBUG_LANE_SUM = 8, PLFEM_DEBUG_LANE_REDUCE = 16 };
+int plfem_debug_lane_ops(plfem_ctx* ctx, int32_t what, const double* in, double* out);
 #endif
 
 #ifdef __cplusplus
diff --git a/pl_fem_vectoriel_amd/_native.py b/pl_fem_vectoriel_amd/_native.py
--- a/pl_fem_vectoriel_amd/_native.py
+++ b/pl_fem_vectoriel_amd/_native.py
@@ -49,7 +49,9 @@
 TEST_HOOK_EXPORTS = ("plfem_debug_factor_until", "plfem_debug_copy", "plfem_debug_symeig", "plfem_debug_symeig_band",
                      "plfem_debug_set_perturb", "plfem_debug_solve_block", "plfem_debug_level_plan", "plfem_debug_panel",
                      "plfem_debug_scale_store", "plfem_debug_first_pass", "plfem_debug_spmv_block", "plfem_debug_chol",
-                     "plfem_debug_block_scale", "plfem_debug_rotate", "plfem_debug_start_field", "plfem_debug_set_elements")
+                     "plfem_debug_block_scale", "plfem_debug_rotate", "plfem_debug_start_field", "plfem_debug_set_elements",
+                     "plfem_debug_lane_ops")
+LANE_XOR, LANE_SUM, LANE_REDUCE = 0, 8, 16
 PANEL_FORMS = ("dot", "axpy", "dot_block", "axpy_block")
 SPMV_BLOCK_FORMS = ("b_block", "b_block_il", "b_block_il_gram", "a_block")
 BLOCK_P = 4
@@ -322,6 +324,7 @@
     h.plfem_debug_block_scale.argtypes = [vp, vp, vp, i64, vp, vp, vp, i64, vp, i32, vp, vp, i32]
     h.plfem_debug_rotate.argtypes = [vp, vp, i32, vp, i32, i32, vp]
     h.plfem_debug_start_field.argtypes = [vp, i32, vp]
+    h.plfem_debug_lane_ops.argtypes = [vp, i32, vp, vp]
     _hooks = h
     return h
 
@@ -664,6 +667,10 @@
     def debug_start_field(self, nvec: int, out):
         self._check(load_test_hooks().plfem_debug_start_field(self._h, int(nvec), self._dev(out)), "plfem_debug_start_field")
 
+    def debug_lane_ops(self, what: int, inp, out):
+        self._check(load_test_hooks().plfem_debug_lane_ops(self._h, int(what), self._dev(inp), self._dev(out)),
+                    "plfem_debug_lane_ops")
+
     def debug_level_plan(self):
         nl = self.sym.info["levels"] + 1
         out = np.zeros(len(PLAN_FIELDS) * nl, dtype=np.int64)
diff --git a/pl_fem_vectoriel_amd/csrc/api_debug.hip b/pl_fem_vectoriel_amd/csrc/api_debug.hip
--- a/pl_fem_vectoriel_amd/csrc/api_debug.hip
+++ b/pl_fem_vectoriel_amd/csrc/api_debug.hip
@@ -52,6 +52,10 @@
   else if (n == "V") src = c->d_V;
   else if (n == "BV") src = c->d_BV;
   else if (n == "Hcols") src = c->d_Hcols;
+  else if (n == "partial") {
+    if ((size_t)offset + (size_t)count > c->partial_doubles) return PLFEM_EINVAL;
+    src = c->d_partial;
+  }
   else if (n == "counters") {
     if (offset + count > 4) return PLFEM_EINVAL;
     int32_t tmp[4];
@@ -223,6 +227,82 @@
   return lanczos_hook_done(c, "debug rotate");
 } catch (...) { return host_failure(c); }
 
+namespace {
+template <int H, int BIT, bool DESC, int V>
+__device__ __forceinline__ void shfl_reduce_step(double (&a)[V], int lane) {
+  if constexpr (H >= 1) {
+    const bool up = (lane & BIT) != 0;
+#pragma unroll
+    for (int k = 0; k < H; ++k) {
+      const double send = up ? a[k] : a[k + H];
+      const double keep = up ? a[k + H] : a[k];
+      a[k] = keep + __shfl_xor(send, BIT);
+    }
+    shfl_reduce_step<H / 2, DESC ? BIT / 2 : 2 * BIT, DESC>(a, lane);
+  }
+}
+template <int V, bool DESC>
+__device__ __forceinline__ void shfl_reduce(double (&a)[V], int lane) {
+  shfl_reduce_step<V / 2, DESC ? 32 : 1, DESC>(a, lane);
+  if constexpr (DESC) {
+#pragma unroll
+    for (int off = 32 / V; off >= 1; off >>= 1) a[0] += __shfl_xor(a[0], off);
+  } else {
+#pragma unroll
+    for (int off = V; off < 64; off <<= 1) a[0] += __shfl_xor(a[0], off);
+  }
+}
+
+template <int OFF>
+__global__ __launch_bounds__(64) void k_debug_lane_xor(const double* __restrict__ in, double* __restrict__ out) {
+  out[threadIdx.x] = plfem::lane_xor<OFF>(in[threadIdx.x]);
+}
+__global__ __launch_bounds__(64) void k_debug_lane_sum(const double* __restrict__ in, double* __restrict__ out) {
+  const double x = in[threadIdx.x];
+  double v = x;
+  for (int off = 32; off >= 1; off >>= 1) v += __shfl_xor(v, off);
+  out[threadIdx.x] = plfem::wave_sum_desc(x);
+  out[64 + threadIdx.x] = v;
+}
+template <int V, bool DESC>
+__global__ __launch_bounds__(64) void k_debug_lane_reduce(const double* __restrict__ in, double* __restrict__ out) {
+  const int lane = threadIdx.x;
+  double a[V], b[V];
+#pragma unroll
+  for (int v = 0; v < V; ++v) a[v] = b[v] = in[v * 64 + lane];
+  plfem::multi_reduce<V, DESC>(a, lane);
+  shfl_reduce<V, DESC>(b, lane);
+  out[lane] = a[0];
+  out[64 + lane] = b[0];
+  out[128 + lane] = (double)plfem::multi_reduce_index<V, DESC>(lane);
+}
+}
+
+extern "C" int plfem_debug_lane_ops(plfem_ctx* c, int32_t what, const double* in, double* out) try {
+  if (!c || !in || !out) return PLFEM_EINVAL;
+  HIP_TRY(c, hipSetDevice(c->device));
+  hipStream_t st = c->stream;
+  if (what >= PLFEM_DEBUG_LANE_XOR && what < PLFEM_DEBUG_LANE_XOR + 6) {
+    plfem::with_constant<0, 1, 2, 3, 4, 5>(what - PLFEM_DEBUG_LANE_XOR, [&](auto s) {
+      hipLaunchKernelGGL(k_debug_lane_xor<(1 << decltype(s)::value)>, dim3(1), dim3(64), 0, st, in, out);
+    });
+  } else if (what == PLFEM_DEBUG_LANE_SUM) {
+    hipLaunchKernelGGL(k_debug_lane_sum, dim3(1), dim3(64), 0, st, in, out);
+  } else if (what >= PLFEM_DEBUG_LANE_REDUCE + 4 && what < PLFEM_DEBUG_LANE_REDUCE + 12) {
+    const int lv = (what - PLFEM_DEBUG_LANE_REDUCE) >> 1;
+    const bool desc = (what & 1) != 0;
+    plfem::with_constant<2, 3, 4, 5>(lv, [&](auto s) {
+      constexpr int V = 1 << decltype(s)::value;
+      if (desc) hipLaunchKernelGGL((k_debug_lane_reduce<V, true>), dim3(1), dim3(64), 0, st, in, out);
+      else hipLaunchKernelGGL((k_debug_lane_reduce<V, false>), dim3(1), dim3(64), 0, st, in, out);
+    });
+  } else {
+    c->err = "debug lane ops: unknown operation";
+    return PLFEM_EINVAL;
+  }
+  return lanczos_hook_done(c, "debug lane ops");
+} catch (...) { return host_failure(c); }
+
 extern "C" int plfem_debug_start_field(plfem_ctx* c, int32_t nvec, double* out) try {
   if (!c || !out || nvec < 1 || nvec > plfem::BLOCK_P) return PLFEM_EINVAL;
   HIP_TRY(c, hipSetDevice(c->device));
diff --git a/pl_fem_vectoriel_amd/csrc/device.h b/pl_fem_vectoriel_amd/csrc/device.h
--- a/pl_fem_vectoriel_amd/csrc/device.h
+++ b/pl_fem_vectoriel_amd/csrc/device.h
@@ -204,6 +204,76 @@
   else with_constant<Rest...>(v, f);
 }
 
+namespace lane_detail {
+template <int CTRL, int BANKS>
+__device__ __forceinline__ int dpp(int old, int src) {
+  return __builtin_amdgcn_update_dpp(old, src, CTRL, 0xf, BANKS, false);
+}
+template <int OFF>
+__device__ __forceinline__ int xor_dpp(int x) {
+  static_assert(OFF == 1 || OFF == 2 || OFF == 4 || OFF == 8, "DPP reaches inside a row of 16 lanes");
+  if constexpr (OFF == 1) return dpp<0xB1, 0xf>(x, x);
+  else if constexpr (OFF == 2) return dpp<0x4E, 0xf>(x, x);
+  else if constexpr (OFF == 8) return dpp<0x128, 0xf>(x, x);
+  else return dpp<0x114, 0xa>(dpp<0x104, 0x5>(x, x), x);
+}
+}
+
+template <int OFF>
+__device__ __forceinline__ double lane_xor(double v, bool upper) {
+  static_assert(OFF == 1 || OFF == 2 || OFF == 4 || OFF == 8 || OFF == 16 || OFF == 32, "one butterfly distance of a wave");
+  const int lo = __double2loint(v), hi = __double2hiint(v);
+  if constexpr (OFF == 32) {
+    const auto a = __builtin_amdgcn_permlane32_swap(lo, lo, false, false);
+    const auto b = __builtin_amdgcn_permlane32_swap(hi, hi, false, false);
+    return __hiloint2double(upper ? b[0] : b[1], upper ? a[0] : a[1]);
+  } else if constexpr (OFF == 16) {
+    const auto a = __builtin_amdgcn_permlane16_swap(lo, lo, false, false);
+    const auto b = __builtin_amdgcn_permlane16_swap(hi, hi, false, false);
+    return __hiloint2double(upper ? b[0] : b[1], upper ? a[0] : a[1]);
+  } else {
+    return __hiloint2double(lane_detail::xor_dpp<OFF>(hi), lane_detail::xor_dpp<OFF>(lo));
+  }
+}
+template <int OFF>
+__device__ __forceinline__ double lane_xor(double v) {
+  return lane_xor<OFF>(v, OFF >= 16 && (__lane_id() & OFF) != 0);
+}
+
+template <int OFF>
+__device__ __forceinline__ double lane_xor_pair_sum(double x, double y, bool upper) {
+  if constexpr (OFF == 32 || OFF == 16) {
+    const int xl = __double2loint(x), xh = __double2hiint(x), yl = __double2loint(y), yh = __double2hiint(y);
+    if constexpr (OFF == 32) {
+      const auto a = __builtin_amdgcn_permlane32_swap(xl, yl, false, false);
+      const auto b = __builtin_amdgcn_permlane32_swap(xh, yh, false, false);
+      return __hiloint2double(b[0], a[0]) + __hiloint2double(b[1], a[1]);
+    } else {
+      const auto a = __builtin_amdgcn_permlane16_swap(xl, yl, false, false);
+      const auto b = __builtin_amdgcn_permlane16_swap(xh, yh, false, false);
+      return __hiloint2double(b[0], a[0]) + __hiloint2double(b[1], a[1]);
+    }
+  } else {
+    return (upper ? y : x) + lane_xor<OFF>(upper ? x : y, upper);
+  }
+}
+
+__device__ __forceinline__ double wave_sum_desc(double v) {
+  v += lane_xor<32>(v);
+  v += lane_xor<16>(v);
+  v += lane_xor<8>(v);
+  v += lane_xor<4>(v);
+  v += lane_xor<2>(v);
+  v += lane_xor<1>(v);
+  return v;
+}
+__device__ __forceinline__ double group8_sum_desc(double v) {
+  v += lane_xor<4>(v);
+  v += lane_xor<2>(v);
+  v += lane_xor<1>(v);
+  return v;
+}
+
 template <int V, bool DESC = false>
 __device__ __forceinline__ int multi_reduce_index(int lane) {
   int idx = 0;
@@ -217,25 +287,23 @@
   if constexpr (H >= 1) {
     const bool up = (lane & BIT) != 0;
 #pragma unroll
-    for (int k = 0; k < H; ++k) {
-      const double send = up ? a[k] : a[k + H];
-      const double keep = up ? a[k + H] : a[k];
-      a[k] = keep + __shfl_xor(send, BIT);
-    }
+    for (int k = 0; k < H; ++k) a[k] = lane_xor_pair_sum<BIT>(a[k], a[k + H], up);
     multi_reduce_step<H / 2, DESC ? BIT / 2 : 2 * BIT, DESC>(a, lane);
+  }
+}
+
+template <int OFF, bool DESC>
+__device__ __forceinline__ void multi_reduce_tail(double& v) {
+  if constexpr (OFF >= 1 && OFF <= 32) {
+    v += lane_xor<OFF>(v);
+    multi_reduce_tail<DESC ? OFF / 2 : 2 * OFF, DESC>(v);
   }
 }
 
 template <int V, bool DESC = false>
 __device__ __forceinline__ void multi_reduce(double (&a)[V], int lane) {
   multi_reduce_step<V / 2, DESC ? 32 : 1, DESC>(a, lane);
-  if constexpr (DESC) {
-#pragma unroll
-    for (int off = 32 / V; off >= 1; off >>= 1) a[0] += __shfl_xor(a[0], off);
-  } else {
-#pragma unroll
-    for (int off = V; off < 64; off <<= 1) a[0] += __shfl_xor(a[0], off);
-  }
+  multi_reduce_tail<DESC ? 32 / V : V, DESC>(a[0]);
 }
 
 inline int ceil_div(int64_t a, int64_t b) { return (int)((a + b - 1) / b); }
diff --git a/pl_fem_vectoriel_amd/csrc/kernels_assembly.hip b/pl_fem_vectoriel_amd/csrc/kernels_assembly.hip
--- a/pl_fem_vectoriel_amd/csrc/kernels_assembly.hip
+++ b/pl_fem_vectoriel_amd/csrc/kernels_assembly.hip
@@ -252,11 +252,8 @@
   }
 #pragma unroll
   for (int q = 0; q < P; ++q) {
-#pragma unroll
-    for (int off = 4; off >= 1; off >>= 1) {
-      sx[q] += __shfl_xor(sx[q], off, 8);
-      sy[q] += __shfl_xor(sy[q], off, 8);
-    }
+    sx[q] = group8_sum_desc(sx[q]);
+    sy[q] = group8_sum_desc(sy[q]);
   }
   if (row < N && sub == 0) {
 #pragma unroll
@@ -289,10 +286,7 @@
     }
   }
 #pragma unroll
-  for (int q = 0; q < DPN * P; ++q) {
-#pragma unroll
-    for (int off = 4; off >= 1; off >>= 1) s[q] += __shfl_xor(s[q], off, 8);
-  }
+  for (int q = 0; q < DPN * P; ++q) s[q] = group8_sum_desc(s[q]);
   if (row < N && sub == 0) {
 #pragma unroll
     for (int comp = 0; comp < DPN; ++comp)
@@ -322,9 +316,9 @@
     }
 #pragma unroll
     for (int t = 0; t < GE; ++t) {
-      g[t] += __shfl_xor(g[t], 8);
-      g[t] += __shfl_xor(g[t], 16);
-      g[t] += __shfl_xor(g[t], 32);
+      g[t] += lane_xor<8>(g[t]);
+      g[t] += lane_xor<16>(g[t]);
+      g[t] += lane_xor<32>(g[t]);
     }
     const int wave = threadIdx.x >> 6, lane = threadIdx.x & 63;
     if (lane < 8) {
@@ -363,11 +357,8 @@
   }
 #pragma unroll
   for (int q = 0; q < P; ++q) {
-#pragma unroll
-    for (int off = 4; off >= 1; off >>= 1) {
-      sx[q] += __shfl_xor(sx[q], off, 8);
-      sy[q] += __shfl_xor(sy[q], off, 8);
-    }
+    sx[q] = group8_sum_desc(sx[q]);
+    sy[q] = group8_sum_desc(sy[q]);
   }
   if (row < N && sub == 0) {
 #pragma unroll
diff --git a/pl_fem_vectoriel_amd/csrc/kernels_front.hip b/pl_fem_vectoriel_amd/csrc/kernels_front.hip
--- a/pl_fem_vectoriel_amd/csrc/kernels_front.hip
+++ b/pl_fem_vectoriel_amd/csrc/kernels_front.hip
@@ -135,13 +135,6 @@
   return fma(fma(-d, r, 1.0), r, r);
 }
 
-__device__ __forceinline__ double lane_xor16(double v, bool odd_row) {
-  const int lo = __double2loint(v), hi = __double2hiint(v);
-  const auto a = __builtin_amdgcn_permlane16_swap(lo, lo, false, false);
-  const auto b = __builtin_amdgcn_permlane16_swap(hi, hi, false, false);
-  return __hiloint2double(odd_row ? b[0] : b[1], odd_row ? a[0] : a[1]);
-}
-
 __device__ __forceinline__ void pair_step(double a, double b, double c, double thr, double rep, bool past_first, bool past_second,
                                           double y0, double y1, const double (&ra)[4], const double (&rb)[4],
                                           double (&v)[4], double& d0, double& d1, double& od, int& nper) {
@@ -305,7 +298,7 @@
       for (int r = 0; r < 4; ++r) {
         const int c = 16 * tc + lk + 4 * r;
         const double y = tc == 0 ? y0[r] : y1[r];
-        const double w = fma(y, rdd[tc][r], lane_xor16(y, lk & 1) * rdo[tc][r]);
+        const double w = fma(y, rdd[tc][r], lane_xor<16>(y, lk & 1) * rdo[tc][r]);
         W[(int64_t)c * m + i] = w;
         Y[(int64_t)c * m + i] = y;
         if (c < nbk) F[(int64_t)(kcol + c) * m + i] = w;
diff --git a/pl_fem_vectoriel_amd/csrc/kernels_lanczos.hip b/pl_fem_vectoriel_amd/csrc/kernels_lanczos.hip
--- a/pl_fem_vectoriel_amd/csrc/kernels_lanczos.hip
+++ b/pl_fem_vectoriel_amd/csrc/kernels_lanczos.hip
@@ -43,11 +43,11 @@
   const double* col[CW];
 #pragma unroll
   for (int t = 0; t < CW; ++t) col[t] = Pm + (int64_t)min(c0 + t, ncols - 1) * n;
-  double acc[CW][P];
-#pragma unroll
-  for (int t = 0; t < CW; ++t)
-#pragma unroll
-    for (int q = 0; q < P; ++q) acc[t][q] = 0.0;
+  constexpr int V = CW * P;
+  static_assert((V & (V - 1)) == 0 && V <= 64, "multi_reduce<V>");
+  double acc[V];
+#pragma unroll
+  for (int v = 0; v < V; ++v) acc[v] = 0.0;
   int64_t i = i0 + lane;
   for (; i + 64 < i1; i += 128) {
     double a[2][CW], w[2][P];
@@ -63,7 +63,7 @@
 #pragma unroll
       for (int t = 0; t < CW; ++t)
 #pragma unroll
-        for (int q = 0; q < P; ++q) acc[t][q] += a[h][t] * w[h][q];
+        for (int q = 0; q < P; ++q) acc[t * P + q] += a[h][t] * w[h][q];
   }
   for (; i < i1; i += 64) {
     double w[P];
@@ -73,17 +73,16 @@
     for (int t = 0; t < CW; ++t) {
       const double a = col[t][i];
 #pragma unroll
-      for (int q = 0; q < P; ++q) acc[t][q] += a * w[q];
-    }
-  }
-#pragma unroll
-  for (int t = 0; t < CW; ++t) {
-#pragma unroll
-    for (int q = 0; q < P; ++q) {
-      double v = acc[t][q];
-      for (int off = 32; off >= 1; off >>= 1) v += __shfl_xor(v, off);
-      if (lane == 0 && c0 + t < ncols) partial[((int64_t)(c0 + t) * P + q) * nchunks + blockIdx.x] = v;
-    }
+      for (int q = 0; q < P; ++q) acc[t * P + q] += a * w[q];
+    }
+  }
+  if constexpr (V == 1) {
+    const double v = wave_sum_desc(acc[0]);
+    if (lane == 0) partial[(int64_t)c0 * nchunks + blockIdx.x] = v;
+  } else {
+    multi_reduce<V, true>(acc, lane);
+    const int v = multi_reduce_index<V, true>(lane), t = v / P, q = v % P;
+    if ((lane & (64 / V - 1)) == 0 && c0 + t < ncols) partial[((int64_t)(c0 + t) * P + q) * nchunks + blockIdx.x] = acc[0];
   }
 }
 
@@ -94,7 +93,7 @@
   const int c = cq / P, q = cq % P;
   double acc = 0.0;
   for (int t = threadIdx.x; t < nchunks; t += 64) acc += partial[(int64_t)cq * nchunks + t];
-  for (int off = 32; off >= 1; off >>= 1) acc += __shfl_xor(acc, off);
+  acc = wave_sum_desc(acc);
   if (threadIdx.x == 0) {
     h[c + (int64_t)q * ldh] = acc;
     if (hacc) hacc[c + (int64_t)q * ldacc] += acc;
@@ -207,9 +206,9 @@
       }
       for (; k < nseg; k += 8) x += pp[k];
     }
-    x += __shfl_xor(x, 1, 8);
-    x += __shfl_xor(x, 2, 8);
-    x += __shfl_xor(x, 4, 8);
+    x += lane_xor<1>(x);
+    x += lane_xor<2>(x);
+    x += lane_xor<4>(x);
     if (part == 0) {
       sh[v] = x;
       if (blockIdx.x == 0 && v / P < ncols) Hout[(v / P) + (int64_t)(v % P) * ldh] = x;
@@ -255,7 +254,7 @@
         for (int u = 0; u < 8; ++u) acc += v[u];
       }
       for (; t < nchunks; t += 64) acc += pp[t];
-      for (int off = 32; off >= 1; off >>= 1) acc += __shfl_xor(acc, off);
+      acc = wave_sum_desc(acc);
       if (lane == 0) sG[(cq / P) + (cq % P) * P] = acc;
     }
   }
@@ -435,8 +434,7 @@
   for (int j = 0; j < MB; ++j)
 #pragma unroll
     for (int t = 0; t < 5; ++t) {
-      double v = acc[j][t];
-      for (int off = 32; off >= 1; off >>= 1) v += __shfl_xor(v, off);
+      const double v = wave_sum_desc(acc[j][t]);
       if ((threadIdx.x & 63) == 0) red[threadIdx.x >> 6][j][t] = v;
     }
   __syncthreads();
@@ -452,7 +450,7 @@
   const int mode = t / 5, q = t % 5;
   double acc = 0.0;
   for (int b = threadIdx.x; b < nblocks; b += 64) acc += partial[((int64_t)mode * nblocks + b) * 5 + q];
-  for (int off = 32; off >= 1; off >>= 1) acc += __shfl_xor(acc, off);
+  acc = wave_sum_desc(acc);
   if (threadIdx.x == 0) out[t] = acc;
 }
 
@@ -502,14 +500,14 @@
   for (int j = 0; j < MB; ++j) { r2[j] = 0.0; a2[j] = 0.0; }
   const int sub = threadIdx.x & 7;
   for (int rr = threadIdx.x >> 3; rr < POST_ROWS; rr += 32) {
+    static_assert(POST_ROWS % 32 == 0, "k_resid_sums: whole trips");
     const int row = blockIdx.x * POST_ROWS + rr;
-    if (row >= N) break;
-    if (bmask[row]) continue;
+    const bool on = row < N && !bmask[row];
     double ax[MB], ay[MB], bx[MB], by[MB];
 #pragma unroll
     for (int j = 0; j < MB; ++j) { ax[j] = 0; ay[j] = 0; bx[j] = 0; by[j] = 0; }
-    const int q1 = rowptr[row + 1];
-    for (int q = rowptr[row] + sub; q < q1; q += 8) {
+    const int q1 = on ? rowptr[row + 1] : 0;
+    for (int q = on ? rowptr[row] + sub : 0; q < q1; q += 8) {
       const int c = colind[q];
       const double axx = vxx[q], m = vm[q];
       if (DPN == 1) {
@@ -534,7 +532,7 @@
         ax[j] += __shfl_xor(ax[j], off, 8); ay[j] += __shfl_xor(ay[j], off, 8);
         bx[j] += __shfl_xor(bx[j], off, 8); by[j] += __shfl_xor(by[j], off, 8);
       }
-      if (sub == 0) {
+      if (sub == 0 && on) {
         const double rx = ax[j] - l[j] * bx[j], ry = ay[j] - l[j] * by[j];
         r2[j] += rx * rx + ry * ry;
         a2[j] += ax[j] * ax[j] + ay[j] * ay[j];
@@ -543,7 +541,8 @@
   }
 #pragma unroll
   for (int j = 0; j < MB; ++j) {
-    for (int off = 32; off >= 1; off >>= 1) { r2[j] += __shfl_xor(r2[j], off); a2[j] += __shfl_xor(a2[j], off); }
+    r2[j] = wave_sum_desc(r2[j]);
+    a2[j] = wave_sum_desc(a2[j]);
     if ((threadIdx.x & 63) == 0) { red[threadIdx.x >> 6][j][0] = r2[j]; red[threadIdx.x >> 6][j][1] = a2[j]; }
   }
   __syncthreads();
@@ -558,7 +557,7 @@
   const int mode = t >> 1, q = t & 1;
   double acc = 0.0;
   for (int b = threadIdx.x; b < nblocks; b += 64) acc += partial[((int64_t)mode * nblocks + b) * 2 + q];
-  for (int off = 32; off >= 1; off >>= 1) acc += __shfl_xor(acc, off);
+  acc = wave_sum_desc(acc);
   if (threadIdx.x == 0) out[t] = acc;
 }
 
diff --git a/pl_fem_vectoriel_amd/csrc/kernels_sweep.hip b/pl_fem_vectoriel_amd/csrc/kernels_sweep.hip
--- a/pl_fem_vectoriel_amd/csrc/kernels_sweep.hip
+++ b/pl_fem_vectoriel_amd/csrc/kernels_sweep.hip
@@ -146,8 +146,8 @@
   }
 #pragma unroll
   for (int u = 0; u < P; ++u) {
-    acc[0][u] += __shfl_xor(acc[0][u], 32);
-    acc[1][u] += __shfl_xor(acc[1][u], 32);
+    acc[0][u] += lane_xor<32>(acc[0][u], h != 0);
+    acc[1][u] += lane_xor<32>(acc[1][u], h != 0);
   }
   if (h == 0) {
 #pragma unroll
@@ -361,8 +361,8 @@
   }
 #pragma unroll
   for (int u = 0; u < P; ++u) {
-    acc[0][u] += __shfl_xor(acc[0][u], 32);
-    acc[1][u] += __shfl_xor(acc[1][u], 32);
+    acc[0][u] += lane_xor<32>(acc[0][u], h != 0);
+    acc[1][u] += lane_xor<32>(acc[1][u], h != 0);
   }
   if (h == 0) {
 #pragma unroll
```

Result: no change. 553.0, median of 6 (+2.0%).
